# MarineRoboticsGroup/mac

Hardware: AMD Instinct MI355X
Metric: frank_wolfe_iters_per_sec (higher is better)
Workload: dtype f64; 1 GPU; configs[3]: ER N=100000 ~2M candidates, chain fixed, K=10%; N=100000, m_candidates=2001737, K=200173, fixed_edges=99999, fw_iters=209, parallelism=single GPU

## Files before the change

### include/machip.h

```cpp
#ifndef MACHIP_H
#define MACHIP_H

#include <stdint.h>

#ifdef __cplusplus
extern "C" {
#endif

#define MACHIP_ABI_VERSION 11

typedef enum machip_status {
    MACHIP_OK = 0,
    MACHIP_NOT_CONVERGED = 1,
    MACHIP_DISCONNECTED = 2,
    MACHIP_BAD_ARG = 3,
    MACHIP_HIP_ERROR = 4,
    MACHIP_RCCL_ERROR = 5,
    MACHIP_NO_DEVICE = 6
} machip_status;

typedef struct machip_problem machip_problem;

typedef struct machip_solve_stats {
    int64_t lanczos_steps;
    int64_t spmv_total;
    int64_t vec_passes;
    int64_t restarts;
    int64_t nnz;
    int64_t support;
    double residual;
    double lnorm;
    double gpu_ms;
    double step_ms;
    int64_t steps_timed;
    int64_t steps_lowp;
    double drift;
} machip_solve_stats;

int machip_version(void);
int machip_sizeof_stats(void);
int machip_device_count(void);
const char* machip_last_error(void);

int machip_create(int device, int64_t n,
                  int64_t n_fixed, const int32_t* fi, const int32_t* fj, const double* fw,
                  int64_t m, const int32_t* ci, const int32_t* cj, const double* cw,
                  double min_selection_weight_tol, machip_problem** out);
void machip_destroy(machip_problem* p);

int machip_set_x(machip_problem* p, const double* x);
int machip_get_x(machip_problem* p, double* x);

int machip_assemble(machip_problem* p, int64_t* nnz_out);
int machip_get_laplacian(machip_problem* p, int32_t* indptr, int32_t* indices, double* data);

int machip_fiedler(machip_problem* p, double tol, int max_steps, const double* x0, int warm_start,
                   double* lambda2, double* v_out, double* X_out, int q,
                   machip_solve_stats* stats);

int machip_set_start(machip_problem* p, const double* x0);

int machip_gradient(machip_problem* p, double* g_out);

int machip_lp_topk(machip_problem* p, int64_t k, double* s_out);

int machip_fw_step(machip_problem* p, int64_t k, int iter, double tol, int max_steps, int warm_start,
                   double* f, double* dual, double* gnorm, machip_solve_stats* stats);
int machip_fw_commit(machip_problem* p);
int machip_fw_run(machip_problem* p, int64_t k, int first_iter, int max_iters, double gap_tol, double grad_tol, double tol,
                  int max_steps, int warm_start, double* upper_inout, double* f_traj, double* dual_traj, double* gnorm_traj,
                  machip_solve_stats* stats, int* modes, int* iters_done);

int machip_round_nearest(machip_problem* p, int64_t k, int decimals, double* rounded_out);

int machip_fiedler_csr(int device, int64_t n, const int32_t* indptr, const int32_t* indices,
                       const double* data, double tol, int max_steps, const double* x0,
                       double* lambda2, double* v_out, double* X_out, int q,
                       machip_solve_stats* stats);

int machip_spmv(machip_problem* p, const double* v, double* y, int variant);

int machip_landscape(machip_problem* p, int sweeps, double* u_out);

int machip_profile_spmv(machip_problem* p, int reps, double* avg_us, double* bytes_per_launch);

int machip_comm_unique_id(void* id128);
int machip_comm_init(machip_problem* p, int rank, int nranks, const void* id128);
int machip_comm_init_local(machip_problem** handles, int nranks);
int machip_selftest_watchdog(int work_ms, int limit_ms);
int machip_peer_access(int device_a, int device_b);
int machip_ipc_blob_bytes(void);
int machip_ipc_export(machip_problem* p, void* blob, int blob_bytes);
int machip_comm_init_ipc(machip_problem* p, int rank, int nranks, const void* blobs, double timeout_s);
int machip_comm_close_ipc(machip_problem* p);
int machip_comm_drop_ipc(machip_problem* p);
int machip_comm_drop(machip_problem* p);
int machip_comm_timing(machip_problem* p, double* grad_us, double* exchange_us);
int machip_solve_mode(machip_problem* p, int64_t* closures);
int machip_comm_mode(machip_problem* p);
int machip_shard_plan(int64_t m, int nranks, int rank, int64_t* lo, int64_t* hi, int64_t* shard);

int machip_eval_batch(machip_problem* p, int B, const double* X, double tol, int max_steps, double* lambda2,
                      int* status);

int machip_fw_sweep(machip_problem* p, int B, const int64_t* ks, const double* X0, int max_iters, double gap_tol,
                    double grad_tol, double tol, int max_steps, int warm_start, int round_decimals, double* X_out,
                    double* R_out, double* upper, double* f_traj, int* iters, int* status);

int machip_set_solver(machip_problem* p, int mode);

int machip_set_precision(machip_problem* p, int precision);

#define MACHIP_OPTION_AUTO INT64_MIN
int machip_set_option(machip_problem* p, const char* name, int64_t value);
int machip_get_option(machip_problem* p, const char* name, int64_t* value);
const char* machip_option_name(int i);

int machip_synchronize(machip_problem* p);

int machip_membench(int device, int64_t bytes, int reps, double* read_gbs, double* triad_gbs);
int machip_panel_plan(int64_t n, int64_t nnz, int maxlen, int* out12);
void machip_release_cache(void);
int machip_host_tridiag_smallest(const double* a, const double* b, int J, double* theta, double* s);
int machip_host_follow_records(const double* tri3, int J, int n, double e_target, double tiny_l, int jcap, int* points, int cap,
                               int* npoints, int* jeff, double* est);

typedef struct machip_esp machip_esp;
#define MACHIP_ESP_DENSE_INVERSE 1
#define MACHIP_ESP_MATRIX_FREE 2
#define MACHIP_ESP_SPANNING_TREE 8
int machip_esp_create(int device, int64_t n, int64_t n_fixed, const int32_t* fi, const int32_t* fj, const double* fw,
                      int64_t m, const int32_t* ci, const int32_t* cj, const double* cw, int fold, int flags, machip_esp** out);
void machip_esp_destroy(machip_esp* h);
int machip_esp_select(machip_esp* h, int nb, const int64_t* ks, int32_t* order_out, double* gain_out, double* t_ms_out);
int machip_esp_weighted_resistances(machip_esp* h, double* r_out);
int machip_esp_info(machip_esp* h, int32_t* info4, double* beta);
int machip_esp_tree_plan(int64_t n, int64_t n_fixed, const int32_t* fi, const int32_t* fj, const double* fw, int32_t* parent,
                         double* R, int32_t* pre, int32_t* end, int64_t* n_seeds, int32_t* su, int32_t* sv, double* sw);
int machip_esp_seeds(machip_esp* h, int64_t* seeds_out);

int machip_esp_relax_eval(machip_esp* h, const double* x, double* F_out, double* grad_out);
int machip_esp_relax_run(machip_esp* h, int64_t k, int max_iters, double gap_tol, double grad_tol, double* x_inout,
                         double* f_traj, double* dual_traj, double* gnorm_traj, int* iters_out, double* upper_out);
int machip_esp_relax_inner(machip_esp* h, const double* a, const double* b, double* out);

typedef struct machip_eig machip_eig;
int machip_eig_create(int device, int64_t n, int64_t n_fixed, const int32_t* fi, const int32_t* fj, const double* fw,
                      int64_t m, const int32_t* ci, const int32_t* cj, const double* cw, int fold, int batch, int flags, machip_eig** out);
void machip_eig_destroy(machip_eig* h);
int machip_eig_select(machip_eig* h, int64_t k, int32_t* order_out, double* lambda2_out, double* t_ms_out);
int machip_eig_candidate_lambda2(machip_eig* h, double* out);
int machip_eig_candidate_bounds(machip_eig* h, double* out);
int machip_eig_info(machip_eig* h, int32_t* info6, double* beta_lambda2, int64_t cap, int32_t* solved_out, int32_t* applies_out);

#ifdef __cplusplus
}
#endif
#endif
```

### mac_amd/_lib.py

```python
from __future__ import annotations

import ctypes as C
import os

import numpy as np

_HERE = os.path.dirname(os.path.abspath(__file__))
LIB_PATH = os.environ.get("MACHIP_LIB") or os.path.join(_HERE, "libmachip.so")

OK, NOT_CONVERGED, DISCONNECTED, BAD_ARG, HIP_ERROR, RCCL_ERROR, NO_DEVICE = range(7)
STATUS_NAMES = ["OK", "NOT_CONVERGED", "DISCONNECTED", "BAD_ARG", "HIP_ERROR", "RCCL_ERROR", "NO_DEVICE"]


class MachipError(RuntimeError):
    def __init__(self, status, msg):
        super().__init__(f"libmachip: {STATUS_NAMES[status] if 0 <= status < 7 else status}: {msg}")
        self.status = status


class NotConverged(MachipError):
    pass


class Disconnected(MachipError):
    """lambda_2 ~ 0 (the reference fails with SuperLU 'Factor is exactly singular')."""


class SolveStats(C.Structure):
    _fields_ = [("lanczos_steps", C.c_int64), ("spmv_total", C.c_int64), ("vec_passes", C.c_int64),
                ("restarts", C.c_int64), ("nnz", C.c_int64), ("support", C.c_int64),
                ("residual", C.c_double), ("lnorm", C.c_double), ("gpu_ms", C.c_double),
                ("step_ms", C.c_double), ("steps_timed", C.c_int64), ("steps_lowp", C.c_int64), ("drift", C.c_double)]

    def asdict(self):
        return {k: getattr(self, k) for k, _ in self._fields_}


_i32p = C.POINTER(C.c_int32)
_f64p = C.POINTER(C.c_double)
_lib = None

SIGNATURES = {
    "machip_version": (C.c_int, []),
    "machip_sizeof_stats": (C.c_int, []),
    "machip_device_count": (C.c_int, []),
    "machip_last_error": (C.c_char_p, []),
    "machip_create": (C.c_int, [C.c_int, C.c_int64, C.c_int64, _i32p, _i32p, _f64p, C.c_int64, _i32p, _i32p,
                                _f64p, C.c_double, C.POINTER(C.c_void_p)]),
    "machip_destroy": (None, [C.c_void_p]),
    "machip_set_x": (C.c_int, [C.c_void_p, _f64p]),
    "machip_get_x": (C.c_int, [C.c_void_p, _f64p]),
    "machip_assemble": (C.c_int, [C.c_void_p, C.POINTER(C.c_int64)]),
    "machip_get_laplacian": (C.c_int, [C.c_void_p, _i32p, _i32p, _f64p]),
    "machip_fiedler": (C.c_int, [C.c_void_p, C.c_double, C.c_int, _f64p, C.c_int, _f64p, _f64p, _f64p, C.c_int,
                                 C.POINTER(SolveStats)]),
    "machip_set_start": (C.c_int, [C.c_void_p, _f64p]),
    "machip_gradient": (C.c_int, [C.c_void_p, _f64p]),
    "machip_lp_topk": (C.c_int, [C.c_void_p, C.c_int64, _f64p]),
    "machip_fw_step": (C.c_int, [C.c_void_p, C.c_int64, C.c_int, C.c_double, C.c_int, C.c_int, _f64p, _f64p,
                                 _f64p, C.POINTER(SolveStats)]),
    "machip_fw_commit": (C.c_int, [C.c_void_p]),
    "machip_fw_run": (C.c_int, [C.c_void_p, C.c_int64, C.c_int, C.c_int, C.c_double, C.c_double, C.c_double, C.c_int, C.c_int, _f64p, _f64p,
                                _f64p, _f64p, C.POINTER(SolveStats), C.POINTER(C.c_int), C.POINTER(C.c_int)]),
    "machip_round_nearest": (C.c_int, [C.c_void_p, C.c_int64, C.c_int, _f64p]),
    "machip_fiedler_csr": (C.c_int, [C.c_int, C.c_int64, _i32p, _i32p, _f64p, C.c_double, C.c_int, _f64p, _f64p,
                                     _f64p, _f64p, C.c_int, C.POINTER(SolveStats)]),
    "machip_spmv": (C.c_int, [C.c_void_p, _f64p, _f64p, C.c_int]),
    "machip_landscape": (C.c_int, [C.c_void_p, C.c_int, _f64p]),
    "machip_profile_spmv": (C.c_int, [C.c_void_p, C.c_int, _f64p, _f64p]),
    "machip_comm_unique_id": (C.c_int, [C.c_void_p]),
    "machip_comm_init": (C.c_int, [C.c_void_p, C.c_int, C.c_int, C.c_void_p]),
    "machip_comm_init_local": (C.c_int, [C.POINTER(C.c_void_p), C.c_int]),
    "machip_selftest_watchdog": (C.c_int, [C.c_int, C.c_int]),
    "machip_peer_access": (C.c_int, [C.c_int, C.c_int]),
    "machip_ipc_blob_bytes": (C.c_int, []),
    "machip_ipc_export": (C.c_int, [C.c_void_p, C.c_void_p, C.c_int]),
    "machip_comm_init_ipc": (C.c_int, [C.c_void_p, C.c_int, C.c_int, C.c_void_p, C.c_double]),
    "machip_comm_close_ipc": (C.c_int, [C.c_void_p]),
    "machip_comm_mode": (C.c_int, [C.c_void_p]),
    "machip_shard_plan": (C.c_int, [C.c_int64, C.c_int, C.c_int, C.POINTER(C.c_int64), C.POINTER(C.c_int64), C.POINTER(C.c_int64)]),
    "machip_eval_batch": (C.c_int, [C.c_void_p, C.c_int, _f64p, C.c_double, C.c_int, _f64p, C.POINTER(C.c_int)]),
    "machip_fw_sweep": (C.c_int, [C.c_void_p, C.c_int, C.POINTER(C.c_int64), _f64p, C.c_int, C.c_double, C.c_double, C.c_double,
                                  C.c_int, C.c_int, C.c_int, _f64p, _f64p, _f64p, _f64p, C.POINTER(C.c_int), C.POINTER(C.c_int)]),
    "machip_set_solver": (C.c_int, [C.c_void_p, C.c_int]),
    "machip_set_option": (C.c_int, [C.c_void_p, C.c_char_p, C.c_int64]),
    "machip_get_option": (C.c_int, [C.c_void_p, C.c_char_p, C.POINTER(C.c_int64)]),
    "machip_option_name": (C.c_char_p, [C.c_int]),
    "machip_comm_drop_ipc": (C.c_int, [C.c_void_p]),
    "machip_comm_drop": (C.c_int, [C.c_void_p]),
    "machip_comm_timing": (C.c_int, [C.c_void_p, _f64p, _f64p]),
    "machip_solve_mode": (C.c_int, [C.c_void_p, C.POINTER(C.c_int64)]),
    "machip_set_precision": (C.c_int, [C.c_void_p, C.c_int]),
    "machip_synchronize": (C.c_int, [C.c_void_p]),
    "machip_membench": (C.c_int, [C.c_int, C.c_int64, C.c_int, _f64p, _f64p]),
    "machip_host_tridiag_smallest": (C.c_int, [_f64p, _f64p, C.c_int, _f64p, _f64p]),
    "machip_host_follow_records": (C.c_int, [_f64p, C.c_int, C.c_int, C.c_double, C.c_double, C.c_int, C.POINTER(C.c_int), C.c_int,
                                             C.POINTER(C.c_int), C.POINTER(C.c_int), C.POINTER(C.c_double)]),
    "machip_release_cache": (None, []),
    "machip_panel_plan": (C.c_int, [C.c_int64, C.c_int64, C.c_int, C.POINTER(C.c_int)]),
    "machip_esp_create": (C.c_int, [C.c_int, C.c_int64, C.c_int64, _i32p, _i32p, _f64p, C.c_int64, _i32p, _i32p, _f64p,
                                    C.c_int, C.c_int, C.POINTER(C.c_void_p)]),
    "machip_esp_destroy": (None, [C.c_void_p]),
    "machip_esp_select": (C.c_int, [C.c_void_p, C.c_int, C.POINTER(C.c_int64), _i32p, _f64p, _f64p]),
    "machip_esp_weighted_resistances": (C.c_int, [C.c_void_p, _f64p]),
    "machip_esp_info": (C.c_int, [C.c_void_p, _i32p, C.POINTER(C.c_double)]),
    "machip_esp_tree_plan": (C.c_int, [C.c_int64, C.c_int64, _i32p, _i32p, _f64p, _i32p, _f64p, _i32p, _i32p, C.POINTER(C.c_int64),
                                       _i32p, _i32p, _f64p]),
    "machip_esp_seeds": (C.c_int, [C.c_void_p, C.POINTER(C.c_int64)]),
    "machip_esp_relax_eval": (C.c_int, [C.c_void_p, _f64p, C.POINTER(C.c_double), _f64p]),
    "machip_esp_relax_run": (C.c_int, [C.c_void_p, C.c_int64, C.c_int, C.c_double, C.c_double, _f64p, _f64p, _f64p, _f64p,
                                       C.POINTER(C.c_int), C.POINTER(C.c_double)]),
    "machip_esp_relax_inner": (C.c_int, [C.c_void_p, _f64p, _f64p, C.POINTER(C.c_double)]),
    "machip_eig_create": (C.c_int, [C.c_int, C.c_int64, C.c_int64, _i32p, _i32p, _f64p, C.c_int64, _i32p, _i32p, _f64p,
                                    C.c_int, C.c_int, C.c_int, C.POINTER(C.c_void_p)]),
    "machip_eig_destroy": (None, [C.c_void_p]),
    "machip_eig_select": (C.c_int, [C.c_void_p, C.c_int64, _i32p, _f64p, _f64p]),
    "machip_eig_candidate_lambda2": (C.c_int, [C.c_void_p, _f64p]),
    "machip_eig_candidate_bounds": (C.c_int, [C.c_void_p, _f64p]),
    "machip_eig_info": (C.c_int, [C.c_void_p, _i32p, _f64p, C.c_int64, _i32p, _i32p]),
}


def load():
    global _lib
    if _lib is not None:
        return _lib
    if not os.path.exists(LIB_PATH):
        raise ImportError(f"{LIB_PATH} is missing: build it with `python __graft_entry__.py` "
                          "(hipcc --offload-arch=gfx950); mac_amd has no CPU fallback")
    lib = C.CDLL(LIB_PATH, mode=C.RTLD_GLOBAL)
    for name, (res, args) in SIGNATURES.items():
        fn = getattr(lib, name)
        fn.restype = res
        fn.argtypes = args
    _lib = lib
    import atexit
    atexit.register(lib.machip_release_cache)
    return lib


OPTION_AUTO = -(1 << 63)
CREATION_OPTIONS = frozenset({"asm_g", "asm_maxgrid", "vbudget_mb", "vcap"})


def option_names():
    lib, out, i = load(), [], 0
    while True:
        nm = lib.machip_option_name(i)
        if nm is None:
            return out
        out.append(nm.decode())
        i += 1


def set_default_option(name, value=None):
    check(load().machip_set_option(None, name.encode(), OPTION_AUTO if value is None else int(value)))


class default_options:

    def __init__(self, **opts):
        self.opts = opts

    def __enter__(self):
        lib = load()
        self.old = {}
        for k, v in self.opts.items():
            cur = C.c_int64(0)
            check(lib.machip_get_option(None, k.encode(), C.byref(cur)))
            self.old[k] = cur.value
            set_default_option(k, v)
        return self

    def __exit__(self, *exc):
# ... 130 lines not shown

    def gradient(self, want=True):
        g = np.empty(self.m) if want else None
        check(self._lib.machip_gradient(self._h, p_f64(g)))
        return g

    def lp_topk(self, k, want=True):
        s = np.empty(self.m) if want else None
        check(self._lib.machip_lp_topk(self._h, int(k), p_f64(s)))
        return s

    def fw_step(self, k, it, tol=1e-8, max_steps=0, warm_start=False):
        f, d, gn = C.c_double(), C.c_double(), C.c_double()
        check(self._lib.machip_fw_step(self._h, int(k), int(it), float(tol), int(max_steps),
                                       int(bool(warm_start)), C.byref(f), C.byref(d), C.byref(gn),
                                       C.byref(self.stats)))
        return f.value, d.value, gn.value

    def fw_commit(self):
        check(self._lib.machip_fw_commit(self._h))

    def fw_run(self, k, max_iters, first_iter=0, gap_tol=0.0, grad_tol=0.0, tol=1e-8, max_steps=0, warm_start=False, upper=float("inf")):
        n = max(1, int(max_iters))
        f = np.zeros(n); d = np.zeros(n); gn = np.zeros(n)
        st = (SolveStats * n)()
        modes = (C.c_int * (2 * n))()
        up = C.c_double(float(upper)); done = C.c_int(0)
        status = self._lib.machip_fw_run(self._h, int(k), int(first_iter), int(max_iters), float(gap_tol), float(grad_tol), float(tol),
                                         int(max_steps), int(bool(warm_start)), C.byref(up), p_f64(f), p_f64(d), p_f64(gn), st, modes, C.byref(done))
        it = int(done.value)
        if it:
            C.memmove(C.byref(self.stats), C.byref(st[it - 1]), C.sizeof(SolveStats))
        check(status)
        return dict(f=f[:it], dual=d[:it], gnorm=gn[:it], upper=up.value, iters=it, stats=[st[i] for i in range(it)],
                    modes=[(int(modes[2 * i]), int(modes[2 * i + 1])) for i in range(it)])

    def round_nearest(self, k, decimals=10):
        out = np.empty(self.m)
        check(self._lib.machip_round_nearest(self._h, int(k), -1 if decimals is None else int(decimals), p_f64(out)))
        return out

    def profile_spmv(self, reps=200):
        us, by = C.c_double(), C.c_double()
        check(self._lib.machip_profile_spmv(self._h, int(reps), C.byref(us), C.byref(by)))
        return us.value, by.value

    def comm_init(self, rank, nranks, unique_id: bytes):
        _single_node_bootstrap()
        buf = C.create_string_buffer(unique_id, 128)
        with _stdout_to_stderr():
            st = self._lib.machip_comm_init(self._h, int(rank), int(nranks), buf)
        check(st)

    def ipc_export(self) -> bytes:
        nb = self._lib.machip_ipc_blob_bytes()
        buf = C.create_string_buffer(nb)
        check(self._lib.machip_ipc_export(self._h, buf, nb))
        return buf.raw

    def comm_init_ipc(self, rank, nranks, blobs, timeout_s=10.0):
        nb = self._lib.machip_ipc_blob_bytes()
        assert len(blobs) == nranks and all(len(b) == nb for b in blobs)
        buf = C.create_string_buffer(b"".join(blobs), nb * nranks)
        check(self._lib.machip_comm_init_ipc(self._h, int(rank), int(nranks), buf, float(timeout_s)))

    def comm_close_ipc(self):
        check(self._lib.machip_comm_close_ipc(self._h))

    def comm_drop_ipc(self):
        check(self._lib.machip_comm_drop_ipc(self._h))

    def comm_drop(self):
        check(self._lib.machip_comm_drop(self._h))

    def comm_timing(self):
        a, b = C.c_double(0.0), C.c_double(0.0)
        check(self._lib.machip_comm_timing(self._h, C.byref(a), C.byref(b)))
        return a.value, b.value

    def solve_mode(self):
        c = C.c_int64(0)
        return int(self._lib.machip_solve_mode(self._h, C.byref(c))), int(c.value)

    def set_option(self, name, value=None):
        if value is not None and name in CREATION_OPTIONS:
            raise ValueError(f"option {name!r} is read when the handle is created: set it with mac_amd._lib.default_options({name}=...) around the constructor")
        check(self._lib.machip_set_option(self._h, name.encode(), OPTION_AUTO if value is None else int(value)))

    def set_options(self, **opts):
        for k, v in opts.items():
            self.set_option(k, v)

    def get_option(self, name):
        v = C.c_int64(0)
        check(self._lib.machip_get_option(self._h, name.encode(), C.byref(v)))
        return None if v.value == OPTION_AUTO else v.value

    def set_solver(self, mode):
        check(self._lib.machip_set_solver(self._h, int(mode)))

    def eval_batch(self, X, tol=1e-8, max_steps=0):
        X = np.ascontiguousarray(X, dtype=np.float64)
        assert X.ndim == 2 and X.shape[1] == self.m
        B = X.shape[0]
        lam = np.zeros(B)
        st = np.zeros(B, dtype=np.int32)
        check(self._lib.machip_eval_batch(self._h, B, p_f64(X), float(tol), int(max_steps), p_f64(lam),
                                          st.ctypes.data_as(C.POINTER(C.c_int))))
        return lam, st

    def fw_sweep(self, ks, X0, max_iters=5, gap_tol=1e-4, grad_tol=1e-8, tol=1e-8, max_steps=0, warm_start=False,
                 round_decimals=10, want_rounded=True):
        X0 = np.ascontiguousarray(X0, dtype=np.float64)
        ks = np.ascontiguousarray(ks, dtype=np.int64)
        assert X0.ndim == 2 and X0.shape == (len(ks), self.m)
        B = len(ks)
        X = np.empty((B, self.m)); R = np.empty((B, self.m)) if want_rounded else None
        up = np.zeros(B); ft = np.full((B, max(1, max_iters)), np.nan)
        it = np.zeros(B, dtype=np.int32); st = np.zeros(B, dtype=np.int32)
        check(self._lib.machip_fw_sweep(self._h, B, ks.ctypes.data_as(C.POINTER(C.c_int64)), p_f64(X0), int(max_iters),
                                        float(gap_tol), float(grad_tol), float(tol), int(max_steps), int(bool(warm_start)),
                                        int(round_decimals), p_f64(X), p_f64(R), p_f64(up), p_f64(ft),
                                        it.ctypes.data_as(C.POINTER(C.c_int)), st.ctypes.data_as(C.POINTER(C.c_int))))
        return dict(x=X, rounded=R, upper=up, f_traj=ft[:, :max_iters], iters=it, status=st)

    def set_precision(self, precision):
        check(self._lib.machip_set_precision(self._h, int(precision)))

    def synchronize(self):
        check(self._lib.machip_synchronize(self._h))


ESP_DENSE_INVERSE = 1
ESP_MATRIX_FREE = 2
ESP_SPANNING_TREE = 8


def host_esp_tree(n, fi, fj, fw):
    fi, fj, fw = i32(fi), i32(fj), f64(fw)
    n, nf = int(n), len(fw)
    parent, pre, end = (np.zeros(max(n, 1), dtype=np.int32) for _ in range(3))
    R = np.zeros(max(n, 1))
    su, sv, sw = np.zeros(max(nf, 1), dtype=np.int32), np.zeros(max(nf, 1), dtype=np.int32), np.zeros(max(nf, 1))
    r = C.c_int64(0)
    check(load().machip_esp_tree_plan(n, nf, p_i32(fi), p_i32(fj), p_f64(fw), p_i32(parent), p_f64(R), p_i32(pre), p_i32(end),
                                      C.byref(r), p_i32(su), p_i32(sv), p_f64(sw)))
    r = r.value
    return dict(parent=parent[:n], R=R[:n], pre=pre[:n], end=end[:n], seeds=(su[:r].copy(), sv[:r].copy(), sw[:r].copy()))


class Esp:

    def __init__(self, n, fi, fj, fw, ci, cj, cw, fold=64, dense_inverse=False, device=0, *, matrix_free=False):
        if not isinstance(matrix_free, (bool, np.bool_)) and matrix_free != "tree":
            raise ValueError(f'matrix_free must be False, True or "tree", not {matrix_free!r}')
        lib = load()
        require_device()
        self.n = int(n)
        fi, fj, fw = i32(fi), i32(fj), f64(fw)
        ci, cj, cw = i32(ci), i32(cj), f64(cw)
        self.m = int(len(cw))
        h = C.c_void_p()
        flags = (ESP_DENSE_INVERSE if dense_inverse else 0) | (ESP_MATRIX_FREE if matrix_free else 0)
        if isinstance(matrix_free, str):
            flags |= ESP_SPANNING_TREE
        check(lib.machip_esp_create(int(device), self.n, len(fw), p_i32(fi), p_i32(fj), p_f64(fw), self.m,
# ... 198 lines not shown
```

### mac_amd/csrc/kernels.h

```cpp
#pragma once
#include "common.h"

namespace machip {

template <typename T>
struct CsrViewT {
    int n;
    const int* rowptr;
    const int* col;
    const T* val;
};
using CsrView = CsrViewT<double>;

struct PatternView {
    int n;
    const int* prow;
    const int* pcol;
    const int* pk;
    const double* pw;
};

struct LanState {
    int jA;
    int jB;
// ... 3 lines not shown

struct LanView {
    int n;
    LanState* st;
    double* u;
    double* w;
    double* V;
    double* alpha;
    double* beta;
    double* l1;
    double* part_u;
    int P_u;
    double* part_a;
    int P_a;
};

constexpr int kAsmGrid = 4096;
__global__ __launch_bounds__(kBlock) void k_x_bits(const double* __restrict__ x, long m, double tol, unsigned long long* __restrict__ bits) {
    for (long i = (long)blockIdx.x * kBlock + threadIdx.x; i < m; i += (long)gridDim.x * kBlock) {
        const unsigned long long bal = __ballot(x[i] > tol);
        if ((threadIdx.x & 63) == 0) bits[i >> 6] = bal;
    }
}
__device__ __forceinline__ bool x_bit(const unsigned int* __restrict__ bits32, int k) { return (bits32[k >> 5] >> (k & 31)) & 1u; }

template <int G>
__global__ __launch_bounds__(kBlock) void k_asm_count(PatternView P, const unsigned int* __restrict__ xbits,
                                                      int rows_per_block,
                                                      int* __restrict__ cnt, int* __restrict__ blk_sum,
                                                      int* __restrict__ hsum = nullptr) {
    __shared__ int sm[4];
    constexpr int GPB = kBlock / G;
    const int lane = threadIdx.x % G, g = threadIdx.x / G;
    const int r0 = blockIdx.x * rows_per_block;
    const int r1 = min(P.n, r0 + rows_per_block);
    int local = 0, supp = 0, mx = 0;
    for (int r = r0 + g; r < r1; r += GPB) {
        const int b = P.prow[r], e = P.prow[r + 1];
        int c = 0, sc = 0;
        for (int p = b + lane; p < e; p += G) {
            const int k = P.pk[p];
            const bool cand = k >= 0;
            const bool act = cand ? x_bit(xbits, k) : true;
            c += act;
            sc += (cand && act);
        }
        c = group_sum_i<G>(c);
        sc = group_sum_i<G>(sc);
        if (lane == 0) {
            cnt[r] = c + 1;
            local += c + 1;
            supp += sc;
            mx = max(mx, c + 1);
        }
    }
    const int tot = block_sum_i(local, sm);
    const int stot = block_sum_i(supp, sm);
#pragma unroll
    for (int o = 32; o > 0; o >>= 1) mx = max(mx, __shfl_xor(mx, o, kWave));
    __syncthreads();
    if ((threadIdx.x & 63) == 0) sm[threadIdx.x >> 6] = mx;
    __syncthreads();
    if (threadIdx.x == 0) {
        blk_sum[blockIdx.x] = tot;
        blk_sum[kAsmGrid + blockIdx.x] = stot;
        const int longest = max(max(sm[0], sm[1]), max(sm[2], sm[3]));
        blk_sum[2 * kAsmGrid + blockIdx.x] = longest;
        if (hsum) {
            hsum[blockIdx.x] = tot; hsum[kAsmGrid + blockIdx.x] = stot; hsum[2 * kAsmGrid + blockIdx.x] = longest;
        }
    }
}

struct PanSpec {
    int NP = 0;
    int C = 1;
    int band = 0;
    int* ps = nullptr;
    double* bd = nullptr;
    int* bpk = nullptr;
    int* ovf = nullptr;
};

template <int G>
__global__ __launch_bounds__(kBlock) void k_asm_fill(PatternView P, const unsigned int* __restrict__ xbits, const double* __restrict__ x,
                                                     int rows_per_block,
                                                     const int* __restrict__ cnt,
                                                     const int* __restrict__ blk_sum,
                                                     int* __restrict__ rowptr, int* __restrict__ col,
                                                     double* __restrict__ val,
                                                     double* __restrict__ blk_lnorm, PanSpec S = PanSpec()) {
    extern __shared__ __attribute__((aligned(16))) char smem_raw[];
    int* s_off = reinterpret_cast<int*>(smem_raw);
    __shared__ int sm_i[4];
    __shared__ double sm_d[4];
    __shared__ int s_chunk[kBlock];
    constexpr int GPB = kBlock / G;
    const int tid = threadIdx.x;
    const int lane = tid % G, g = tid / G;
    const int r0 = blockIdx.x * rows_per_block;
    const int r1 = min(P.n, r0 + rows_per_block);
    const int nr = max(0, r1 - r0);

    int acc = 0;
    for (int b = tid; b < (int)blockIdx.x; b += kBlock) acc += blk_sum[b];
    const int base = block_sum_i(acc, sm_i);

    const int per = (nr + kBlock - 1) / kBlock;
    int csum = 0;
    for (int i = 0; i < per; ++i) {
        const int idx = tid * per + i;
        if (idx < nr) csum += cnt[r0 + idx];
    }
    {
        const int ln = tid & 63, wv = tid >> 6;
        int x = csum;
        for (int o = 1; o < 64; o <<= 1) { const int y = __shfl_up(x, o, kWave); if (ln >= o) x += y; }
        if (ln == 63) s_chunk[wv] = x;
        __syncthreads();
        int before = 0;
        for (int q = 0; q < wv; ++q) before += s_chunk[q];
        int run = before + x - csum;
        if (tid == kBlock - 1) s_off[nr] = before + x;
        for (int i = 0; i < per; ++i) {
            const int idx = tid * per + i;
            if (idx < nr) { s_off[idx] = run; run += cnt[r0 + idx]; }
        }
    }
    __syncthreads();

    double lmax = 0.0;
    for (int r = r0 + g; r < r1; r += GPB) {
        const int b = P.prow[r], e = P.prow[r + 1];
        const int out = base + s_off[r - r0];
        int pos = out + 1;
        double dsum = 0.0, asum = 0.0;
        int lastpid = 0;
        int hb = 0x7fffffff, hn = 0;
        double vl = 0.0, vu = 0.0;
        const int gbase = ((tid & 63) / G) * G;
        for (int p0 = b; p0 < e; p0 += G) {
            const int p = p0 + lane;
            const bool in = p < e;
            const int kc = in ? P.pk[p] : -1;
            const double wgt = in ? P.pw[p] : 0.0;
            const double xk = kc >= 0 ? x[kc] : 1.0;
            const bool act = in && (kc < 0 || x_bit(xbits, kc));
            const double v = act ? xk * wgt : 0.0;
            const unsigned long long bal = __ballot(act);
            unsigned long long gm;
            if (G == 64) gm = bal;
            else gm = (bal >> gbase) & ((1ull << (G & 63)) - 1ull);
            const unsigned long long below = gm & ((1ull << lane) - 1ull);
            const int before = __popcll(below);
            const int c = act ? P.pcol[p] : 0;
            if (act) { col[pos + before] = c; val[pos + before] = -v; }
            if (S.NP) {
                const int pid = act ? c / S.C : 0;
                const int src = below ? 63 - __builtin_clzll(below) : 0;
                const int got = __shfl(pid, gbase + src, kWave);
                const int ppid = below ? got : lastpid;
                if (act) {
                    const int q = pos + before;
                    for (int pp = ppid + 1; pp <= pid; ++pp) S.ps[(size_t)r * (S.NP + 1) + pp] = q;
                    if (S.band && (c == r - 1 || c == r + 1)) {
                        hb = min(hb, q); hn += 1;
                        if (c == r - 1) vl += -v; else vu += -v;
                    }
                }
                if (gm) lastpid = __shfl(pid, gbase + 63 - __builtin_clzll(gm), kWave);
            }
            pos += __popcll(gm);
            dsum += v;
            asum += fabs(v);
        }
        dsum = group_sum<G>(dsum);
        asum = group_sum<G>(asum);
        if (S.NP) {
            if (lane == 0) S.ps[(size_t)r * (S.NP + 1)] = out + 1;
            for (int pp = lastpid + 1 + lane; pp <= S.NP; pp += G) S.ps[(size_t)r * (S.NP + 1) + pp] = pos;
            if (S.band) {
                hn = group_sum_i<G>(hn);
                vl = group_sum<G>(vl); vu = group_sum<G>(vu);
#pragma unroll
                for (int o = G / 2; o > 0; o >>= 1) hb = min(hb, __shfl_xor(hb, o, kWave));
                if (lane == 0) {
                    S.bpk[r] = ((hn ? hb : pos) << 3) | min(hn, 7);
                    if (hn > 7) *S.ovf = 1;
                    S.bd[r] = dsum; S.bd[(size_t)P.n + r] = vl; S.bd[2 * (size_t)P.n + r] = vu;
                }
            }
        }
        if (lane == 0) {
            rowptr[r] = out;
            col[out] = r;
            val[out] = dsum;
            lmax = fmax(lmax, fabs(dsum) + asum);
        }
    }
    lmax = block_max(lmax, sm_d);
    if (tid == 0) {
        blk_lnorm[blockIdx.x] = lmax;
        if (blockIdx.x == gridDim.x - 1) rowptr[P.n] = base + s_off[nr];
    }
}

template <int G, class Op>
__device__ __forceinline__ void spmv_rows_vec(const CsrView& A, const double* __restrict__ x, Op& op) {
    constexpr int GPB = kBlock / G;
    const int lane = threadIdx.x % G, g = threadIdx.x / G;
    const int stride = gridDim.x * GPB;
    for (int r = blockIdx.x * GPB + g; r < A.n; r += 2 * stride) {
        const int r2 = r + stride;
        const bool two = r2 < A.n;
        const int b = A.rowptr[r], e = A.rowptr[r + 1];
        const int b2 = two ? A.rowptr[r2] : 0, e2 = two ? A.rowptr[r2 + 1] : 0;
        double acc = 0.0, acc2 = 0.0;
        int p = b + lane, q = b2 + lane;
        while (p < e || q < e2) {
            double v1 = 0.0, x1 = 0.0, v2 = 0.0, x2 = 0.0;
            if (p < e) { v1 = A.val[p]; x1 = op.gather(x, A.col[p]); }
            if (q < e2) { v2 = A.val[q]; x2 = op.gather(x, A.col[q]); }
            if (p < e) acc += v1 * x1;
            if (q < e2) acc2 += v2 * x2;
            p += G; q += G;
        }
        acc = group_sum<G>(acc);
        acc2 = group_sum<G>(acc2);
        if (lane == 0) { op.row(r, acc); if (two) op.row(r2, acc2); }
    }
}

constexpr int kStreamTile = 2048;

template <int TPR, class Op>
__device__ __forceinline__ void spmv_rows_stream(const CsrView& A, const double* __restrict__ x, Op& op,
                                                 double* prod, int* sptr) {
    constexpr int R = kBlock / TPR;
    const int tid = threadIdx.x;
    const int row = tid / TPR, sub = tid % TPR;
    for (int tile = blockIdx.x; tile * R < A.n; tile += gridDim.x) {
        const int r0 = tile * R;
        const int nr = min(R, A.n - r0);
        for (int i = tid; i <= nr; i += kBlock) sptr[i] = A.rowptr[r0 + i];
        __syncthreads();
        const int p0 = sptr[0], p1 = sptr[nr];
        double acc = 0.0;
        for (int base = p0; base < p1; base += kStreamTile) {
            const int cnt = min(kStreamTile, p1 - base);
            for (int i = tid; i < cnt; i += kBlock) prod[i] = A.val[base + i] * op.gather(x, A.col[base + i]);
            __syncthreads();
            if (row < nr) {
                const int lo = max(sptr[row], base), hi = min(sptr[row + 1], base + cnt);
                for (int q = lo + sub; q < hi; q += TPR) acc += prod[q - base];
            }
            __syncthreads();
        }
        acc = group_sum<TPR>(acc);
        if (row < nr && sub == 0) op.row(r0 + row, acc);
        __syncthreads();
    }
}

struct OpPlain {
    double* y;
    __device__ __forceinline__ void begin(double*) {}
    __device__ __forceinline__ double gather(const double* __restrict__ x, int c) const { return x[c]; }
    __device__ __forceinline__ void row(int r, double acc) { y[r] = acc; }
    __device__ __forceinline__ void end(double*) {}
};

struct OpLanczos {
    LanView L;
    int j;
    double mu, beta, inv, ap;
    const double* vprev;
    double* vj;
    __device__ __forceinline__ void begin(double* sm) {
        j = L.st->jA;
        const double s1 = reduce_partials(L.part_u, L.P_u, sm);
        const double s2 = reduce_partials(L.part_u + kMaxGrid, L.P_u, sm);
        const double s3 = reduce_partials(L.part_u + 2 * kMaxGrid, L.P_u, sm);
        mu = s1 / (double)L.n;
        const double nrm2 = s2 - (double)L.n * mu * mu;
        beta = nrm2 > 0.0 ? sqrt(nrm2) : 0.0;
        inv = beta > 1e-290 ? 1.0 / beta : 0.0;
        ap = 0.0;
        vj = L.V + (size_t)j * (size_t)L.n;
        vprev = j > 0 ? vj - L.n : nullptr;
        if (blockIdx.x == 0 && threadIdx.x == 0) {
            L.beta[j] = beta;
            L.l1[j] = s3 * inv;
            L.st->jB = j;
        }
    }
    __device__ __forceinline__ double gather(const double* __restrict__ x, int c) const { return x[c]; }
    __device__ __forceinline__ void row(int r, double acc) {
        const double wr = acc * inv;
        const double v = (L.u[r] - mu) * inv;
        vj[r] = v;
        L.w[r] = wr;
        const double t = vprev ? wr - beta * vprev[r] : wr;
        ap += v * t;
    }
    __device__ __forceinline__ void end(double* sm) {
        const double tot = block_sum(ap, sm);
        if (threadIdx.x == 0) L.part_a[blockIdx.x] = tot;
    }
};

template <int G, class Op>
__global__ __launch_bounds__(kBlock) void k_spmv_vec(CsrView A, const double* __restrict__ x, Op op) {
    __shared__ double sm[4];
    op.begin(sm);
    spmv_rows_vec<G>(A, x, op);
    op.end(sm);
}

template <int TPR, class Op>
__global__ __launch_bounds__(kBlock) void k_spmv_stream(CsrView A, const double* __restrict__ x, Op op) {
    __shared__ double sm[4];
    __shared__ double prod[kStreamTile];
    __shared__ int sptr[kBlock / TPR + 1];
    op.begin(sm);
    spmv_rows_stream<TPR>(A, x, op, prod, sptr);
    op.end(sm);
}

__global__ __launch_bounds__(kBlock) void k_land_init(CsrView A, double* __restrict__ dg, double* __restrict__ u) {
    for (int r = blockIdx.x * kBlock + threadIdx.x; r < A.n; r += gridDim.x * kBlock) {
        double d = 0.0;
        for (int p = A.rowptr[r], e = A.rowptr[r + 1]; p < e; ++p)
            if (A.col[p] == r) { d = A.val[p]; break; }
        dg[r] = d;
        u[r] = d > 0.0 ? 1.0 / d : 0.0;
    }
}
struct OpLand {
    const double* uin;
    double* uout;
    const double* dg;
    double* pmax;
    double mx;
    __device__ __forceinline__ void begin(double*) { mx = 0.0; }
    __device__ __forceinline__ double gather(const double* __restrict__ x, int c) const { return x[c]; }
    __device__ __forceinline__ void row(int r, double acc) {
        const double d = dg[r];
        double v = d > 0.0 ? uin[r] + (1.0 - acc) / d : 0.0;
        v = v > 0.0 && v < 1e300 ? v : 0.0;
        uout[r] = v;
        mx = fmax(mx, v);
    }
    __device__ __forceinline__ void end(double* sm) {
        const double m = block_max(mx, sm);
        if (threadIdx.x == 0) pmax[blockIdx.x] = m;
    }
};
__global__ __launch_bounds__(kBlock) void k_land_weight(const double* __restrict__ u, const double* __restrict__ pmax, int npart,
                                                        double* __restrict__ z, int n, double p, double floor_w) {
    __shared__ double sm[4];
    double m = 0.0;
    for (int i = threadIdx.x; i < npart; i += kBlock) m = fmax(m, pmax[i]);
    m = block_max(m, sm);
    if (!(m > 0.0)) return;
    const double inv = 1.0 / m;
    for (int r = blockIdx.x * kBlock + threadIdx.x; r < n; r += gridDim.x * kBlock) {
        const double q = u[r] * inv;
        z[r] *= fmax(q > 0.0 ? exp(p * log(q)) : 0.0, floor_w);
    }
}

__global__ __launch_bounds__(kBlock) void k_lan_update(LanView L) {
    __shared__ double sm[4];
    const int j = L.st->jB;
    const double alpha = reduce_partials(L.part_a, L.P_a, sm);
    const double beta = L.beta[j];
    const double* vj = L.V + (size_t)j * (size_t)L.n;
    const double* vp = j > 0 ? vj - L.n : nullptr;
    double s1 = 0.0, s2 = 0.0, s3 = 0.0;
    for (int r = blockIdx.x * kBlock + threadIdx.x; r < L.n; r += gridDim.x * kBlock) {
        double t = L.w[r] - alpha * vj[r];
        if (vp) t -= beta * vp[r];
        L.u[r] = t;
        s1 += t;
        s2 += t * t;
        s3 += fabs(t);
    }
    s1 = block_sum(s1, sm);
    s2 = block_sum(s2, sm);
    s3 = block_sum(s3, sm);
    if (threadIdx.x == 0) {
        L.part_u[blockIdx.x] = s1;
        L.part_u[kMaxGrid + blockIdx.x] = s2;
        L.part_u[2 * kMaxGrid + blockIdx.x] = s3;
        if (blockIdx.x == 0) {
            L.alpha[j] = alpha;
            L.st->jA = j + 1;
        }
    }
}

__global__ __launch_bounds__(kBlock) void k_lan_tail(LanView L) {
    __shared__ double sm[4];
    const int j = L.st->jA;
    const double s1 = reduce_partials(L.part_u, L.P_u, sm);
    const double s2 = reduce_partials(L.part_u + kMaxGrid, L.P_u, sm);
    const double s3 = reduce_partials(L.part_u + 2 * kMaxGrid, L.P_u, sm);
    if (threadIdx.x == 0) {
        const double mu = s1 / (double)L.n;
        const double nrm2 = s2 - (double)L.n * mu * mu;
        const double beta = nrm2 > 0.0 ? sqrt(nrm2) : 0.0;
        L.beta[j] = beta;
        L.l1[j] = beta > 1e-290 ? s3 / beta : 0.0;
    }
}

// ... 965 lines not shown
```

### mac_amd/csrc/machip.hip

```cpp
#include <rccl/rccl.h>
#include <unistd.h>

#include <algorithm>
#include <atomic>
#include <cmath>
#include <chrono>
#include <condition_variable>
#include <functional>
#include <future>
#include <memory>
#include <mutex>
#include <numeric>
#include <thread>
#include <vector>

#include "solver.h"
#include "esp.h"
#include "esp_free.h"
#include "esp_tree.h"
#include "esp_relax.h"
#include "eig.h"

namespace machip {
thread_local std::string g_err;
}
using namespace machip;

#define NCCL_TRY(expr)                                                                       \
    do {                                                                                     \
        ncclResult_t r__ = (expr);                                                           \
        if (r__ != ncclSuccess)                                                              \
            return fail(MACHIP_RCCL_ERROR, std::string(#expr) + ": " + ncclGetErrorString(r__)); \
    } while (0)

static int run_with_watchdog(const std::function<int()>& fn, double limit_s, const std::string& what) {
    auto state = std::make_shared<std::promise<int>>();
    std::future<int> fut = state->get_future();
    std::thread([state, fn] { int r = MACHIP_HIP_ERROR; try { r = fn(); } catch (...) {} state->set_value(r); }).detach();
    if (fut.wait_for(std::chrono::duration<double>(limit_s)) != std::future_status::ready)
        return fail(MACHIP_RCCL_ERROR, what + " did not return within " + std::to_string((int)limit_s) + " s (a peer rank is missing, or the fabric / bootstrap interface is not reachable; MACHIP_RCCL_TIMEOUT_S raises the limit)");
    return fut.get();
}
static double rccl_timeout_s() { const Options& opt = default_options(); const int t = OPT(rccl_timeout_s, 600); return t > 0 ? (double)t : 600.0; }

struct machip_problem;
struct LocalGroup {
    int nranks = 0;
    std::vector<double*> g;
    std::vector<machip_problem*> members;
    ShardGroup sg;
    bool shard_eig = false;
    int lead_status = MACHIP_OK;
    double lead_lam = 0.0;
    machip_solve_stats lead_stats{};
    std::string lead_err;
    ~LocalGroup() {
        for (ShardRank& r : sg.rk) for (hipEvent_t e : r.ev) if (e) (void)hipEventDestroy(e);
        if (sg.fork) (void)hipEventDestroy(sg.fork);
    }
    std::mutex mu;
    std::condition_variable cv;
    int waiting = 0;
    unsigned long generation = 0;
    bool broken = false;
    bool barrier() {
        std::unique_lock<std::mutex> lk(mu);
        if (broken) return false;
        const unsigned long gen = generation;
        if (++waiting == nranks) { waiting = 0; ++generation; cv.notify_all(); return true; }
        cv.wait(lk, [&] { return generation != gen || broken; });
        return !broken;
    }
    void abort() {
        std::lock_guard<std::mutex> lk(mu);
        broken = true;
        cv.notify_all();
    }
};

struct machip_problem {
    int device = 0;
    hipStream_t stream = nullptr;
    int n = 0;
    long m = 0, m_pad = 0;
    double tol_sel = 1e-10;
    int *prow = nullptr, *pcol = nullptr, *pk = nullptr;
    double* pw = nullptr;
    long P = 0;
    int asm_G = 16, asm_rpb = 1, asm_grid = 1;
    int *ci = nullptr, *cj = nullptr;
    double* cw = nullptr;
    double *x = nullptr, *x_next = nullptr, *g = nullptr, *s = nullptr, *scratch_m = nullptr;
    int *cnt = nullptr, *blk_sum = nullptr, *rowptr = nullptr, *col = nullptr;
    double *val = nullptr, *blk_lnorm = nullptr;
    unsigned long long *xb = nullptr, *xb_next = nullptr;
    bool xb_valid = false, xb_next_valid = false;
    long nnz = 0, support = 0;
    int maxlen = 0;
    double lnorm = 0.0;
    bool assembled = false, have_vec = false, csr_only = false;
    bool band_dups_ok = true;
    unsigned int* hist = nullptr;
    SelState* sel = nullptr;
    double* part_fw = nullptr;
    int* h_int = nullptr;
    double* h_dbl = nullptr;
    int* d_hint = nullptr;
    double* d_hdbl = nullptr;
    Solver sol;
    ncclComm_t comm = nullptr;
    std::shared_ptr<LocalGroup> lgroup;
    bool first_collective_pending = false;
    hipEvent_t ev_g0 = nullptr, ev_g1 = nullptr, ev_g2 = nullptr;
    bool ev_g_valid = false;
    std::unique_ptr<IpcGroup> ipcg;
    int rank = 0, nranks = 1;
    bool is_lane = false, lane_fw_ready = false;
    std::vector<machip_problem*> lanes;
    unsigned long start_version = 0;
    unsigned long seen_start_version = ~0ul;

    CsrView csr() const { return CsrView{n, rowptr, col, val}; }
    PatternView pattern() const { return PatternView{n, prow, pcol, pk, pw}; }
};

static int create_lane_stream(const Options& opt, int device, hipStream_t* out) {
    if (OPT(lane_queues, 0) == 0) {
        hipDeviceProp_t prop;
        if (hipGetDeviceProperties(&prop, device) == hipSuccess && prop.multiProcessorCount > 0) {
            const int words = (prop.multiProcessorCount + 31) / 32;
            std::vector<uint32_t> mask((size_t)words, 0xffffffffu);
            if (prop.multiProcessorCount % 32) mask.back() = (1u << (prop.multiProcessorCount % 32)) - 1u;
            if (hipExtStreamCreateWithCUMask(out, (uint32_t)words, mask.data()) == hipSuccess) return MACHIP_OK;
            (void)hipGetLastError();
        }
    }
    HIP_TRY(hipStreamCreateWithFlags(out, hipStreamNonBlocking));
    return MACHIP_OK;
}

namespace {

std::mutex g_csr_mu;
machip_problem* g_csr_cache = nullptr;

struct Slot {
    int col;
    int k;
    double w;
};

int build_pattern(machip_problem* p, int64_t nf, const int32_t* fi, const int32_t* fj, const double* fw,
                  int64_t m, const int32_t* ci, const int32_t* cj, const double* cw) {
    const Options& opt = p->sol.opt;
    const int n = p->n;
    std::vector<long> deg((size_t)n + 1, 0);
    auto chk = [&](int a, int b) { return a >= 0 && a < n && b >= 0 && b < n; };
    for (int64_t e = 0; e < nf; ++e) {
        if (!chk(fi[e], fj[e])) return fail(MACHIP_BAD_ARG, "fixed edge endpoint out of range");
        if (fi[e] != fj[e]) { deg[(size_t)fi[e]]++; deg[(size_t)fj[e]]++; }
    }
    for (int64_t e = 0; e < m; ++e) {
        if (!chk(ci[e], cj[e])) return fail(MACHIP_BAD_ARG, "candidate edge endpoint out of range");
        if (ci[e] != cj[e]) { deg[(size_t)ci[e]]++; deg[(size_t)cj[e]]++; }
    }
    std::vector<long> off((size_t)n + 1, 0);
    for (int r = 0; r < n; ++r) off[(size_t)r + 1] = off[(size_t)r] + deg[(size_t)r];
    std::vector<Slot> slots((size_t)off[(size_t)n]);
    std::vector<long> cur(off.begin(), off.end() - 1);
    for (int64_t e = 0; e < nf; ++e) {
        const int a = fi[e], b = fj[e];
        if (a == b) continue;
        slots[(size_t)cur[(size_t)a]++] = Slot{b, -1, fw[e]};
        slots[(size_t)cur[(size_t)b]++] = Slot{a, -1, fw[e]};
    }
    for (int64_t e = 0; e < m; ++e) {
        const int a = ci[e], b = cj[e];
        if (a == b) continue;
        slots[(size_t)cur[(size_t)a]++] = Slot{b, (int)e, cw[e]};
        slots[(size_t)cur[(size_t)b]++] = Slot{a, (int)e, cw[e]};
    }
    std::vector<int> prow((size_t)n + 1, 0);
    std::vector<int> pcol, pk;
    std::vector<double> pw;
    pcol.reserve(slots.size()); pk.reserve(slots.size()); pw.reserve(slots.size());
    for (int r = 0; r < n; ++r) {
        Slot* b = slots.data() + off[(size_t)r];
        Slot* e = slots.data() + off[(size_t)r + 1];
        std::sort(b, e, [](const Slot& x, const Slot& y) {
            if (x.col != y.col) return x.col < y.col;
            return x.k < y.k;
        });
        for (Slot* q = b; q < e; ++q) {
            if (q->k < 0 && !pcol.empty() && (long)pcol.size() > prow[(size_t)r] && pcol.back() == q->col &&
                pk.back() < 0) {
                pw.back() += q->w;
            } else {
                pcol.push_back(q->col); pk.push_back(q->k); pw.push_back(q->w);
            }
        }
        if (pcol.size() > 2000000000ull) return fail(MACHIP_BAD_ARG, "pattern exceeds int32 indexing");
        {
            int band_slots = 0;
            for (size_t q = (size_t)prow[(size_t)r]; q < pcol.size(); ++q) band_slots += (pcol[q] == r - 1 || pcol[q] == r + 1);
            if (band_slots > 7) p->band_dups_ok = false;
        }
        prow[(size_t)r + 1] = (int)pcol.size();
    }
    p->P = (long)pcol.size();
    ST_TRY(dev_alloc(&p->prow, (size_t)n + 1));
    ST_TRY(dev_alloc(&p->pcol, (size_t)p->P)); ST_TRY(dev_alloc(&p->pk, (size_t)p->P)); ST_TRY(dev_alloc(&p->pw, (size_t)p->P));
    HIP_TRY(hipMemcpyAsync(p->prow, prow.data(), sizeof(int) * ((size_t)n + 1), hipMemcpyHostToDevice, p->stream));
    if (p->P) {
        HIP_TRY(hipMemcpyAsync(p->pcol, pcol.data(), sizeof(int) * (size_t)p->P, hipMemcpyHostToDevice, p->stream));
        HIP_TRY(hipMemcpyAsync(p->pk, pk.data(), sizeof(int) * (size_t)p->P, hipMemcpyHostToDevice, p->stream));
        HIP_TRY(hipMemcpyAsync(p->pw, pw.data(), sizeof(double) * (size_t)p->P, hipMemcpyHostToDevice, p->stream));
    }
    HIP_TRY(hipStreamSynchronize(p->stream));
    const double mean = n ? (double)p->P / n : 1.0;
    int G = 4;
    while (G < 64 && G < mean * 0.75) G <<= 1;
    p->asm_G = OPT(asm_g, G);
    const int gpb = kBlock / p->asm_G;
    long nblk = std::min<long>(std::min(kAsmGrid, std::max(1, OPT(asm_maxgrid, kAsmGrid))), ((long)n + gpb - 1) / gpb);
    if (nblk < 1) nblk = 1;
    long rpb = ((long)n + nblk - 1) / nblk;
    rpb = (rpb + gpb - 1) / gpb * gpb;
    p->asm_rpb = (int)rpb;
    p->asm_grid = (int)(((long)n + rpb - 1) / rpb);
    if (p->asm_grid < 1) p->asm_grid = 1;
    if ((rpb + 1) * (long)sizeof(int) > 64 * 1024)
        return fail(MACHIP_BAD_ARG, "num_nodes above the supported 16.7 million (row-offset scan of the assembly kernel)");
    return MACHIP_OK;
}

template <int G>
void launch_asm(machip_problem* p, const PanSpec& S) {
    const PatternView P = p->pattern();
    const unsigned int* xb32 = reinterpret_cast<const unsigned int*>(p->xb);
    k_asm_count<G><<<p->asm_grid, kBlock, 0, p->stream>>>(P, xb32, p->asm_rpb, p->cnt, p->blk_sum, p->d_hint);
    const size_t lds = sizeof(int) * ((size_t)p->asm_rpb + 1);
    k_asm_fill<G><<<p->asm_grid, kBlock, lds, p->stream>>>(P, xb32, p->x, p->asm_rpb, p->cnt, p->blk_sum,
                                                           p->rowptr, p->col, p->val, p->d_hdbl, S);
}

int assemble(machip_problem* p) {
    if (p->csr_only) return fail(MACHIP_BAD_ARG, "handle wraps a caller CSR; nothing to assemble");
    PanSpec S;
    ST_TRY(p->sol.pan_spec_prepare(&S));
    if (!p->xb_valid) {
        const int grid = std::max(1, (int)std::min<long>(kMaxGrid, (p->m + kBlock - 1) / kBlock));
        k_x_bits<<<grid, kBlock, 0, p->stream>>>(p->x, p->m, p->tol_sel, p->xb);
        p->xb_valid = true;
    }
    switch (p->asm_G) {
        case 4: launch_asm<4>(p, S); break;
        case 8: launch_asm<8>(p, S); break;
        case 16: launch_asm<16>(p, S); break;
        case 32: launch_asm<32>(p, S); break;
        default: launch_asm<64>(p, S); break;
    }
    HIP_TRY(hipGetLastError());
    const int gb = p->asm_grid;
    HIP_TRY(hipStreamSynchronize(p->stream));
    long nnz = 0, supp = 0;
    int maxlen = 0;
    double ln = 0.0;
    for (int b = 0; b < gb; ++b) {
        nnz += p->h_int[b]; supp += p->h_int[kAsmGrid + b]; maxlen = std::max(maxlen, p->h_int[2 * kAsmGrid + b]);
        ln = std::max(ln, p->h_dbl[b]);
    }
    p->nnz = nnz; p->support = supp / 2; p->lnorm = ln; p->maxlen = maxlen;
    p->assembled = true;
    return MACHIP_OK;
}

int alloc_common(machip_problem* p, int vbudget_mb = 0) {
    ST_TRY(p->sol.init(p->n, p->stream, vbudget_mb));
    HIP_TRY(hipHostMalloc((void**)&p->h_int, sizeof(int) * 3 * kAsmGrid, hipHostMallocMapped));
    HIP_TRY(hipHostMalloc((void**)&p->h_dbl, sizeof(double) * std::max(4 * kMaxGrid, kAsmGrid), hipHostMallocMapped));
    HIP_TRY(hipHostGetDevicePointer((void**)&p->d_hint, p->h_int, 0));
    HIP_TRY(hipHostGetDevicePointer((void**)&p->d_hdbl, p->h_dbl, 0));
    return MACHIP_OK;
}

int select_on(machip_problem* p, const double* keys, long k, SelState* st, int prefer_high, bool hist0_done = false) {
    const Options& opt = p->sol.opt;
    const long m = p->m;
    if (k < 0) k = 0;
    if (k > m) k = m;
    if (m <= kSelSmallMax && OPT(sel_small, 1)) {
        k_sel_small<<<1, 1024, 0, p->stream>>>(keys, m, (long long)k, st, prefer_high);
        HIP_TRY(hipGetLastError());
        return MACHIP_OK;
    }
    if (!hist0_done) k_sel_init<<<1, 1024, 0, p->stream>>>(st, (long long)k, p->hist, 6 * kBins);
    if (k > 0) {
        constexpr int B = 1024, U = 4;
        const int grid = (int)std::max<long>(1, std::min<long>(128, (m + (long)B * U - 1) / ((long)B * U)));
        if (hist0_done) k_sel_close0<<<1, 1024, 0, p->stream>>>(p->hist, st);
        for (int pass = hist0_done ? 1 : 0; pass < 6; ++pass) k_sel_pass<U, B><<<grid, B, 0, p->stream>>>(keys, m, pass, p->hist, st);
    }
    k_sel_ties<<<1, 1024, 0, p->stream>>>(keys, m, st, prefer_high);
    HIP_TRY(hipGetLastError());
    return MACHIP_OK;
}

int select_topk(machip_problem* p, long k, bool hist0_done = false) { return select_on(p, p->g, k, p->sel, 0, hist0_done); }

void shard_plan(long m, int nranks, int rank, long* lo, long* hi, long* shard) {
    const long sh = nranks > 0 ? (m + nranks - 1) / nranks : m;
    *shard = sh;
    *lo = std::min(m, sh * rank);
    *hi = std::min(m, *lo + sh);
}

int local_allgather(machip_problem* p, long shard) {
    LocalGroup& G = *p->lgroup;
    HIP_TRY(hipStreamSynchronize(p->stream));
    if (!G.barrier()) return fail(MACHIP_RCCL_ERROR, "in-process communicator was shut down by another rank");
    for (int r = 0; r < G.nranks; ++r)
        if (r != p->rank)
            HIP_TRY(hipMemcpyAsync(p->g + shard * r, G.g[(size_t)r] + shard * r, sizeof(double) * (size_t)shard,
                                   hipMemcpyDeviceToDevice, p->stream));
    HIP_TRY(hipStreamSynchronize(p->stream));
    if (!G.barrier()) return fail(MACHIP_RCCL_ERROR, "in-process communicator was shut down by another rank");
    return MACHIP_OK;
}

int compute_gradient(machip_problem* p, bool have_vec_now = false, long fuse_k = -1, bool* fused = nullptr) {
    const Options& opt = p->sol.opt;
    if (!p->have_vec && !have_vec_now) return fail(MACHIP_BAD_ARG, "no Fiedler vector on the device: call machip_fiedler first");
    const long m = p->m;
    long lo = 0, hi = m, shard = m;
    if (p->nranks > 1) shard_plan(m, p->nranks, p->rank, &lo, &hi, &shard);
    const bool ipc_gather = p->nranks > 1 && !p->comm && p->ipcg;
    if (ipc_gather) {
        k_ipc_pubwait<<<1, 64, 0, p->stream>>>(p->ipcg->view, 3);
    }
    const bool timed = p->nranks > 1;
    if (timed) {
        if (!p->ev_g0) { HIP_TRY(hipEventCreate(&p->ev_g0)); HIP_TRY(hipEventCreate(&p->ev_g1)); HIP_TRY(hipEventCreate(&p->ev_g2)); }
        p->ev_g_valid = false;
        HIP_TRY(hipEventRecord(p->ev_g0, p->stream));
    }
    if (hi > lo) {
        const int grid = (int)std::min<long>(kMaxGrid * 4, (hi - lo + kBlock - 1) / kBlock);
        PeerVecs all;
        if (ipc_gather) { all.n = p->ipcg->nranks; for (int q = 0; q < all.n; ++q) all.v[q] = p->ipcg->g[q]; }
        const bool fuse = fuse_k > 0 && p->nranks <= 1 && m > kSelSmallMax && OPT(sel_fuse, 1) != 0;
        if (fused) *fused = fuse;
        if (fuse) {
            k_sel_init<<<1, 1024, 0, p->stream>>>(p->sel, (long long)std::min(fuse_k, m), p->hist, (6 + kSelRep) * kBins);
            k_grad<true><<<grid, kBlock, 0, p->stream>>>(p->ci, p->cj, p->cw, p->sol.yvec, lo, hi, p->g, all, p->hist + 6 * kBins);
        } else k_grad<false><<<grid, kBlock, 0, p->stream>>>(p->ci, p->cj, p->cw, p->sol.yvec, lo, hi, p->g, all);
        HIP_TRY(hipGetLastError());
    }
    if (timed) HIP_TRY(hipEventRecord(p->ev_g1, p->stream));
    if (ipc_gather) {
        k_ipc_pubwait<<<1, 64, 0, p->stream>>>(p->ipcg->view, 2);
        HIP_TRY(hipGetLastError());
        HIP_TRY(hipEventRecord(p->ev_g2, p->stream));
        p->ev_g_valid = true;
        return MACHIP_OK;
    }
    if (p->nranks > 1) {
        if (p->comm) {
            NCCL_TRY(ncclAllGather(p->g + shard * p->rank, p->g, (size_t)shard, ncclDouble, p->comm, p->stream));
            if (p->first_collective_pending) {
                p->first_collective_pending = false;
                const auto t0 = std::chrono::steady_clock::now();
                const double lim = rccl_timeout_s();
                for (;;) {
                    const hipError_t q = hipStreamQuery(p->stream);
                    if (q == hipSuccess) break;
                    if (q != hipErrorNotReady) return fail(MACHIP_HIP_ERROR, std::string("first ncclAllGather: ") + hipGetErrorString(q));
                    ncclResult_t ar = ncclSuccess;
                    if (ncclCommGetAsyncError(p->comm, &ar) == ncclSuccess && ar != ncclSuccess && ar != ncclInProgress)
                        return fail(MACHIP_RCCL_ERROR, std::string("first ncclAllGather failed asynchronously: ") + ncclGetErrorString(ar));
                    if (std::chrono::duration<double>(std::chrono::steady_clock::now() - t0).count() > lim) {
                        (void)ncclCommAbort(p->comm);
                        p->comm = nullptr;
                        return fail(MACHIP_RCCL_ERROR, "first ncclAllGather of rank " + std::to_string(p->rank) + " of " + std::to_string(p->nranks) +
                                    " did not complete within " + std::to_string((int)lim) + " s: communicator aborted");
                    }
                    std::this_thread::sleep_for(std::chrono::microseconds(200));
                }
            }
        }
        else if (p->lgroup) { const int st = local_allgather(p, shard); if (st != MACHIP_OK) { p->lgroup->abort(); return st; } }
        else return fail(MACHIP_BAD_ARG, "nranks > 1 without a communicator");
        HIP_TRY(hipEventRecord(p->ev_g2, p->stream));
        p->ev_g_valid = true;
    }
    return MACHIP_OK;
}

int run_fiedler(machip_problem* p, double tol, int max_steps, const double* x0, int warm_start,
                double* lambda2, machip_solve_stats* stats) {
    if (!p->assembled) ST_TRY(assemble(p));
    if (x0) {
        HIP_TRY(hipMemcpyAsync(p->sol.start, x0, sizeof(double) * (size_t)p->n, hipMemcpyHostToDevice, p->stream));
        HIP_TRY(hipStreamSynchronize(p->stream));
        p->sol.have_start = true;
        ++p->start_version;
    }
    machip_solve_stats local;
    memset(&local, 0, sizeof(local));
    p->sol.maxlen_hint = p->maxlen;
    p->sol.support_hint = (p->csr_only && !p->sol.chain_like) ? -1 : p->support;
    p->sol.start_guess = x0 != nullptr;
    const int st = p->sol.solve(p->csr(), p->nnz, p->lnorm, tol, max_steps, (x0 == nullptr && warm_start) ? 1 : 0,
                                kAuto, lambda2, &local);
    p->sol.start_guess = false;
    local.support = p->support;
    if (stats) *stats = local;
    p->have_vec = (st == MACHIP_OK || st == MACHIP_NOT_CONVERGED || st == MACHIP_DISCONNECTED);
    return st;
}

int group_fiedler(machip_problem* p, double tol, int max_steps, int warm_start, double* lambda2, machip_solve_stats* stats) {
    LocalGroup& G = *p->lgroup;
    if (!G.barrier()) return fail(MACHIP_RCCL_ERROR, "in-process communicator was shut down by another rank");
    if (p->rank == 0) {
        for (int r = 0; r < G.nranks; ++r) {
            machip_problem* q = G.members[(size_t)r];
            ShardRank& k = G.sg.rk[(size_t)r];
            k.device = q->device; k.stream = q->stream; k.Z0 = q->sol.Z0; k.Z1 = q->sol.Z1; k.part = q->sol.part; k.V = q->sol.V;
            k.ypart = q->sol.ypart; k.sdev = q->sol.sdev; k.yvec = q->sol.yvec; k.A = q->csr();
        }
        machip_solve_stats local;
        memset(&local, 0, sizeof(local));
        p->sol.shard = &G.sg;
        int st = run_fiedler(p, tol, max_steps, nullptr, warm_start, &G.lead_lam, &local);
        p->sol.shard = nullptr;
        if (st == MACHIP_OK || st == MACHIP_NOT_CONVERGED || st == MACHIP_DISCONNECTED) {
            const std::string keep = g_err;
            for (int r = 1; r < G.nranks && (st == MACHIP_OK || st == MACHIP_NOT_CONVERGED || st == MACHIP_DISCONNECTED); ++r)
                if (hipMemcpyAsync(G.sg.rk[(size_t)r].yvec, p->sol.yvec, sizeof(double) * (size_t)p->n, hipMemcpyDeviceToDevice, p->stream) != hipSuccess)
                    st = fail(MACHIP_HIP_ERROR, "copy of the Fiedler vector to a peer failed");
            if (hipStreamSynchronize(p->stream) != hipSuccess) st = fail(MACHIP_HIP_ERROR, "stream error after the row-partitioned solve");
            else g_err = keep;
        }
        G.lead_status = st; G.lead_stats = local; G.lead_err = g_err;
    }
    if (!G.barrier()) return fail(MACHIP_RCCL_ERROR, "in-process communicator was shut down by another rank");
    const int st = G.lead_status;
    *lambda2 = G.lead_lam;
    if (stats) { *stats = G.lead_stats; stats->support = p->support; }
    if (p->rank != 0) {
        g_err = G.lead_err;
        p->have_vec = (st == MACHIP_OK || st == MACHIP_NOT_CONVERGED || st == MACHIP_DISCONNECTED);
    }
    return st;
}

}

extern "C" {

int machip_version(void) { return MACHIP_ABI_VERSION; }
int machip_sizeof_stats(void) { return (int)sizeof(machip_solve_stats); }

int machip_device_count(void) {
    int c = 0;
    if (hipGetDeviceCount(&c) != hipSuccess) return 0;
    return c;
}

const char* machip_last_error(void) { return g_err.c_str(); }

int machip_create(int device, int64_t n, int64_t n_fixed, const int32_t* fi, const int32_t* fj, const double* fw,
                  int64_t m, const int32_t* ci, const int32_t* cj, const double* cw, double min_sel_tol,
                  machip_problem** out) {
    if (!out) return fail(MACHIP_BAD_ARG, "out is NULL");
    *out = nullptr;
    if (n < 2 || n > 2000000000ll) return fail(MACHIP_BAD_ARG, "num_nodes must be in [2, 2e9]");
    if (n_fixed < 0 || m < 0 || m > 2000000000ll) return fail(MACHIP_BAD_ARG, "bad edge counts");
    if ((n_fixed && (!fi || !fj || !fw)) || (m && (!ci || !cj || !cw))) return fail(MACHIP_BAD_ARG, "NULL edge array");
    if (n_fixed + m < n - 1) return fail(MACHIP_BAD_ARG, "fewer than n-1 edges: no spanning tree possible");
    if ((double)(n_fixed + m) > 0.5 * (double)n * (double)(n - 1)) return fail(MACHIP_BAD_ARG, "more edges than the complete graph");
    if (machip_device_count() <= 0) return fail(MACHIP_NO_DEVICE, "no HIP device visible");
    HIP_TRY(hipSetDevice(device));
// ... 22 lines not shown
        ST_TRY(dev_alloc(&p->cnt, (size_t)n + 1)); ST_TRY(dev_alloc(&p->blk_sum, 3 * kAsmGrid));
        ST_TRY(dev_alloc(&p->rowptr, (size_t)n + 1)); ST_TRY(dev_alloc(&p->col, cap)); ST_TRY(dev_alloc(&p->val, cap));
        ST_TRY(dev_alloc(&p->blk_lnorm, kAsmGrid));
        ST_TRY(dev_alloc(&p->xb, (size_t)m / 64 + 2)); ST_TRY(dev_alloc(&p->xb_next, (size_t)m / 64 + 2));
        ST_TRY(dev_alloc(&p->hist, (6 + kSelRep) * kBins)); ST_TRY(dev_alloc(&p->sel, 2)); ST_TRY(dev_alloc(&p->part_fw, 2 * kMaxGrid));
        ST_TRY(alloc_common(p));
        p->sol.csr_cap = cap;
        p->sol.pat = p->pattern();
        p->sol.pan_allowed = p->band_dups_ok;
        {
            std::vector<char> has((size_t)n, 0);
            for (int64_t e = 0; e < n_fixed; ++e) {
                const int a = std::min(fi[e], fj[e]), b = std::max(fi[e], fj[e]);
                if (a >= 0 && b < n && b == a + 1 && fw[e] > 0.0) has[(size_t)a] = 1;
            }
            long cnt = 0;
            for (int64_t i = 0; i + 1 < n; ++i) cnt += has[(size_t)i];
            p->sol.chain_like = cnt >= (long)(0.98 * (double)(n - 1));
            p->sol.chain_edges = cnt;
        }
        return MACHIP_OK;
    };
    st = body();
    if (st != MACHIP_OK) { machip_destroy(p); return st; }
    *out = p;
    return MACHIP_OK;
}

void machip_destroy(machip_problem* p) {
    if (!p) return;
    for (machip_problem* q : p->lanes) machip_destroy(q);
    p->lanes.clear();
    (void)hipSetDevice(p->device);
    if (p->stream) (void)hipStreamSynchronize(p->stream);
    if (p->is_lane) { p->prow = p->pcol = p->pk = nullptr; p->pw = nullptr; p->ci = p->cj = nullptr; p->cw = nullptr; }
    if (p->comm) (void)ncclCommDestroy(p->comm);
    if (p->lgroup) p->lgroup->abort();
    if (p->ipcg) {
        IpcGroup& G = *p->ipcg;
        if (!G.clean_exit) { k_ipc_abort<<<1, 64, 0, p->stream>>>(G.view); (void)hipStreamSynchronize(p->stream); }
        p->sol.ipc = nullptr;
        p->ipcg.reset();
    }
    p->sol.destroy();
    void* ptrs[] = {p->prow, p->pcol, p->pk, p->pw, p->ci, p->cj, p->cw, p->x, p->x_next, p->g, p->s, p->scratch_m, p->cnt,
                    p->blk_sum, p->rowptr, p->col, p->val, p->blk_lnorm, p->xb, p->xb_next, p->hist, p->sel, p->part_fw};
    for (void* q : ptrs) if (q) (void)hipFree(q);
    for (hipEvent_t e : {p->ev_g0, p->ev_g1, p->ev_g2}) if (e) (void)hipEventDestroy(e);
    if (p->h_int) (void)hipHostFree(p->h_int);
    if (p->h_dbl) (void)hipHostFree(p->h_dbl);
    if (p->stream) (void)hipStreamDestroy(p->stream);
    delete p;
}

int machip_set_x(machip_problem* p, const double* x) {
    if (!p || !x || p->csr_only) return fail(MACHIP_BAD_ARG, "machip_set_x: bad handle or NULL x");
    HIP_TRY(hipSetDevice(p->device));
    HIP_TRY(hipMemcpyAsync(p->x, x, sizeof(double) * (size_t)p->m, hipMemcpyHostToDevice, p->stream));
    HIP_TRY(hipStreamSynchronize(p->stream));
    p->assembled = false; p->xb_valid = false;
    return MACHIP_OK;
}

int machip_get_x(machip_problem* p, double* x) {
    if (!p || !x || p->csr_only) return fail(MACHIP_BAD_ARG, "machip_get_x: bad handle or NULL x");
    HIP_TRY(hipSetDevice(p->device));
    HIP_TRY(hipMemcpyAsync(x, p->x, sizeof(double) * (size_t)p->m, hipMemcpyDeviceToHost, p->stream));
    HIP_TRY(hipStreamSynchronize(p->stream));
    return MACHIP_OK;
}

int machip_assemble(machip_problem* p, int64_t* nnz_out) {
    if (!p) return fail(MACHIP_BAD_ARG, "NULL handle");
    HIP_TRY(hipSetDevice(p->device));
    ST_TRY(assemble(p));
    if (nnz_out) *nnz_out = p->nnz;
    return MACHIP_OK;
}

int machip_get_laplacian(machip_problem* p, int32_t* indptr, int32_t* indices, double* data) {
    if (!p || !indptr || !indices || !data) return fail(MACHIP_BAD_ARG, "NULL argument");
    HIP_TRY(hipSetDevice(p->device));
    if (!p->assembled) ST_TRY(assemble(p));
    HIP_TRY(hipMemcpyAsync(indptr, p->rowptr, sizeof(int) * ((size_t)p->n + 1), hipMemcpyDeviceToHost, p->stream));
    HIP_TRY(hipMemcpyAsync(indices, p->col, sizeof(int) * (size_t)p->nnz, hipMemcpyDeviceToHost, p->stream));
    HIP_TRY(hipMemcpyAsync(data, p->val, sizeof(double) * (size_t)p->nnz, hipMemcpyDeviceToHost, p->stream));
    HIP_TRY(hipStreamSynchronize(p->stream));
    return MACHIP_OK;
}

int machip_fiedler(machip_problem* p, double tol, int max_steps, const double* x0, int warm_start,
                   double* lambda2, double* v_out, double* X_out, int q, machip_solve_stats* stats) {
    if (!p || !lambda2) return fail(MACHIP_BAD_ARG, "NULL argument");
    if (X_out && (q < 1 || q > 4)) return fail(MACHIP_BAD_ARG, "q must be in [1,4]");
    HIP_TRY(hipSetDevice(p->device));
    const int st = run_fiedler(p, tol, max_steps, x0, warm_start, lambda2, stats);
    if (st != MACHIP_OK && st != MACHIP_NOT_CONVERGED && st != MACHIP_DISCONNECTED) return st;
    const std::string keep = g_err;
    if (v_out) {
        HIP_TRY(hipMemcpyAsync(v_out, p->sol.yvec, sizeof(double) * (size_t)p->n, hipMemcpyDeviceToHost, p->stream));
        HIP_TRY(hipStreamSynchronize(p->stream));
    }
    if (X_out) ST_TRY(p->sol.ritz_block(q, X_out));
    g_err = keep;
    return st;
}

int machip_set_start(machip_problem* p, const double* x0) {
    if (!p || !x0) return fail(MACHIP_BAD_ARG, "NULL argument");
    HIP_TRY(hipSetDevice(p->device));
    HIP_TRY(hipMemcpyAsync(p->sol.start, x0, sizeof(double) * (size_t)p->n, hipMemcpyHostToDevice, p->stream));
    HIP_TRY(hipStreamSynchronize(p->stream));
    p->sol.have_start = true;
    ++p->start_version;
    return MACHIP_OK;
}

namespace {
struct GroupGuard {
    machip_problem* p;
    bool ok = false;
    ~GroupGuard() {
        if (!ok && p && p->lgroup) p->lgroup->abort();
        if (!ok && p && p->ipcg) { k_ipc_abort<<<1, 64, 0, p->stream>>>(p->ipcg->view); (void)hipStreamSynchronize(p->stream); }
    }
};
}

int machip_gradient(machip_problem* p, double* g_out) {
    if (!p || p->csr_only) return fail(MACHIP_BAD_ARG, "bad handle");
    GroupGuard guard{p};
    HIP_TRY(hipSetDevice(p->device));
    if (!p->have_vec) { guard.ok = true; return fail(MACHIP_BAD_ARG, "no Fiedler vector on the device: call machip_fiedler first"); }
    ST_TRY(compute_gradient(p));
    if (g_out) HIP_TRY(hipMemcpyAsync(g_out, p->g, sizeof(double) * (size_t)p->m, hipMemcpyDeviceToHost, p->stream));
    HIP_TRY(hipStreamSynchronize(p->stream));
    guard.ok = true;
    return MACHIP_OK;
}

int machip_lp_topk(machip_problem* p, int64_t k, double* s_out) {
    if (!p || p->csr_only) return fail(MACHIP_BAD_ARG, "bad handle");
    HIP_TRY(hipSetDevice(p->device));
    ST_TRY(select_topk(p, (long)k));
    const int grid = (int)std::min<long>(kMaxGrid, (p->m + kBlock - 1) / kBlock);
    k_fw_final<<<std::max(grid, 1), kBlock, 0, p->stream>>>(p->g, nullptr, p->m, p->sel, 0.0, nullptr, p->s, p->part_fw);
    if (s_out) HIP_TRY(hipMemcpyAsync(s_out, p->s, sizeof(double) * (size_t)p->m, hipMemcpyDeviceToHost, p->stream));
    HIP_TRY(hipStreamSynchronize(p->stream));
    return MACHIP_OK;
}

int machip_fw_step(machip_problem* p, int64_t k, int iter, double tol, int max_steps, int warm_start,
                   double* f, double* dual, double* gnorm, machip_solve_stats* stats) {
    if (!p || p->csr_only || !f || !dual || !gnorm) return fail(MACHIP_BAD_ARG, "bad argument");
    GroupGuard guard{p};
    HIP_TRY(hipSetDevice(p->device));
    ST_TRY(assemble(p));
    double lam = 0.0;
    const int grid = std::max(1, (int)std::min<long>(kMaxGrid, (p->m + kBlock - 1) / kBlock));
    const double gamma = 2.0 / ((double)iter + 2.0);
    int epi_status = MACHIP_OK;
    auto epilogue = [&](bool speculative) {
        bool fused = false;
        int st = compute_gradient(p, speculative, (long)k, &fused);
        if (st == MACHIP_OK) st = select_topk(p, (long)k, fused);
        if (st == MACHIP_OK) {
            k_fw_final<<<grid, kBlock, 0, p->stream>>>(p->g, p->x, p->m, p->sel, gamma, p->x_next, nullptr, p->d_hdbl, p->tol_sel, p->xb_next);
            p->xb_next_valid = true;
            if (hipGetLastError() != hipSuccess) st = fail(MACHIP_HIP_ERROR, "k_fw_final launch failed");
        }
        epi_status = st;
    };
    bool done = false;
    auto soft = [](int st) { return st == MACHIP_NOT_CONVERGED || st == MACHIP_DISCONNECTED; };
    if (p->lgroup && p->lgroup->shard_eig) {
        const int st = group_fiedler(p, tol, max_steps, warm_start, &lam, stats);
        if (st != MACHIP_OK) { guard.ok = soft(st); return st; }
    } else {
        const bool spec = p->nranks <= 1 && p->sol.opt.get(kOpt_spec_epilogue, 1) != 0;
        if (spec) p->sol.after_check = [&] { epilogue(true); };
        const int st = run_fiedler(p, tol, max_steps, nullptr, warm_start, &lam, stats);
        p->sol.after_check = nullptr;
        if (st != MACHIP_OK) { guard.ok = soft(st); return st; }
        done = spec && p->sol.hook_seq == p->sol.final_check_seq && epi_status == MACHIP_OK;
    }
    if (!done) {
        epilogue(false);
        if (epi_status != MACHIP_OK) return epi_status;
        HIP_TRY(hipStreamSynchronize(p->stream));
    }
    if (p->ipcg) ST_TRY(p->sol.ipc_check_err("gradient exchange"));
    double d = 0.0, q2 = 0.0;
    for (int b = 0; b < grid; ++b) { d += p->h_dbl[b]; q2 += p->h_dbl[kMaxGrid + b]; }
    *f = lam;
    *dual = lam + d;
    *gnorm = std::sqrt(q2);
    guard.ok = true;
    return MACHIP_OK;
}

int machip_fw_run(machip_problem* p, int64_t k, int first_iter, int max_iters, double gap_tol, double grad_tol, double tol, int max_steps,
                  int warm_start, double* upper_inout, double* f_traj, double* dual_traj, double* gnorm_traj, machip_solve_stats* stats,
                  int* modes, int* iters_done) {
    if (!p || p->csr_only || max_iters < 0 || first_iter < 0 || !upper_inout || !iters_done) return fail(MACHIP_BAD_ARG, "machip_fw_run: bad argument");
    double u = *upper_inout;
    int done = 0;
    *iters_done = 0;
    for (int i = 0; i < max_iters; ++i) {
        double f = 0.0, dual = 0.0, gn = 0.0;
        machip_solve_stats st;
        memset(&st, 0, sizeof(st));
        const int rc = machip_fw_step(p, k, first_iter + i, tol, max_steps, (warm_start && (first_iter + i) > 0) ? 1 : 0, &f, &dual, &gn, &st);
        if (rc != MACHIP_OK) { *upper_inout = u; *iters_done = done; return rc; }
        u = std::min(u, dual);
        if (f_traj) f_traj[i] = f;
        if (dual_traj) dual_traj[i] = dual;
        if (gnorm_traj) gnorm_traj[i] = gn;
        if (stats) stats[i] = st;
        if (modes) { modes[2 * i] = p->sol.last_mode; modes[2 * i + 1] = (int)p->sol.last_wb_s; }
        done = i + 1;
        if (gn < grad_tol) break;
        if ((u - f) < gap_tol * std::fabs(f)) break;
        ST_TRY(machip_fw_commit(p));
    }
    *upper_inout = u; *iters_done = done;
    return MACHIP_OK;
}

int machip_round_nearest(machip_problem* p, int64_t k, int decimals, double* rounded_out) {
    if (!p || p->csr_only || !rounded_out) return fail(MACHIP_BAD_ARG, "bad argument");
    if (decimals > 15) return fail(MACHIP_BAD_ARG, "decimals must be <= 15");
    HIP_TRY(hipSetDevice(p->device));
    const long m = p->m;
    if (m == 0) return MACHIP_OK;
    if (!p->scratch_m) ST_TRY(dev_alloc(&p->scratch_m, (size_t)m + 64));
    const int grid = std::max(1, (int)std::min<long>(kMaxGrid, (m + kBlock - 1) / kBlock));
    double* r = p->s;
    const bool tb = decimals >= 0;
    if (tb) k_round_keys<<<grid, kBlock, 0, p->stream>>>(p->x, m, std::pow(10.0, decimals), r);
    else HIP_TRY(hipMemcpyAsync(r, p->x, sizeof(double) * (size_t)m, hipMemcpyDeviceToDevice, p->stream));
// ... 26 lines not shown

int machip_fiedler_csr(int device, int64_t n, const int32_t* indptr, const int32_t* indices, const double* data,
                       double tol, int max_steps, const double* x0, double* lambda2, double* v_out, double* X_out,
                       int q, machip_solve_stats* stats) {
    if (!indptr || !indices || !data || !lambda2) return fail(MACHIP_BAD_ARG, "NULL argument");
    if (n < 2 || n > 2000000000ll) return fail(MACHIP_BAD_ARG, "n must be in [2, 2e9]");
    if (X_out && (q < 1 || q > 4)) return fail(MACHIP_BAD_ARG, "q must be in [1,4]");
    const long nnz = indptr[n];
    if (indptr[0] != 0 || nnz < 0) return fail(MACHIP_BAD_ARG, "bad indptr: indptr[0] must be 0 and indptr[n] >= 0 (int32 row pointers: nnz < 2^31)");
    for (int64_t r = 0; r < n; ++r)
        if (indptr[r + 1] < indptr[r]) return fail(MACHIP_BAD_ARG, "indptr not monotone");
    double lnorm = 0.0;
    int maxlen_csr = 0;
    long chain_cnt = 0;
    for (int64_t r = 0; r < n; ++r) {
        double s = 0.0;
        for (long pp = indptr[r]; pp < (long)indptr[r + 1]; ++pp) {
            if (indices[pp] < 0 || indices[pp] >= n) return fail(MACHIP_BAD_ARG, "column index out of range");
            s += std::fabs(data[pp]);
            if (indices[pp] == r + 1 && data[pp] != 0.0) ++chain_cnt;
        }
        lnorm = std::max(lnorm, s);
        maxlen_csr = std::max(maxlen_csr, (int)(indptr[r + 1] - indptr[r]));
    }
    if (machip_device_count() <= 0) return fail(MACHIP_NO_DEVICE, "no HIP device visible");
    HIP_TRY(hipSetDevice(device));
    std::unique_lock<std::mutex> lk(g_csr_mu, std::try_to_lock);
    machip_problem* p = nullptr;
    bool cached = false;
    if (lk.owns_lock() && g_csr_cache && g_csr_cache->device == device && g_csr_cache->n == (int)n && (long)g_csr_cache->sol.csr_cap >= nnz) {
        p = g_csr_cache;
        cached = true;
    } else {
        if (lk.owns_lock() && g_csr_cache) { machip_destroy(g_csr_cache); g_csr_cache = nullptr; }
        p = new machip_problem();
        p->device = device; p->n = (int)n; p->csr_only = true;
    }
    auto body = [&]() -> int {
        if (!cached) {
            const size_t cap = (size_t)nnz + (size_t)nnz / 4 + 64;
            HIP_TRY(hipStreamCreateWithFlags(&p->stream, hipStreamNonBlocking));
            ST_TRY(dev_alloc(&p->rowptr, (size_t)n + 1)); ST_TRY(dev_alloc(&p->col, cap)); ST_TRY(dev_alloc(&p->val, cap));
            ST_TRY(alloc_common(p));
            p->sol.csr_cap = cap;
        }
        HIP_TRY(hipMemcpyAsync(p->rowptr, indptr, sizeof(int) * ((size_t)n + 1), hipMemcpyHostToDevice, p->stream));
        if (nnz) {
            HIP_TRY(hipMemcpyAsync(p->col, indices, sizeof(int) * (size_t)nnz, hipMemcpyHostToDevice, p->stream));
            HIP_TRY(hipMemcpyAsync(p->val, data, sizeof(double) * (size_t)nnz, hipMemcpyHostToDevice, p->stream));
        }
        HIP_TRY(hipStreamSynchronize(p->stream));
        p->nnz = nnz; p->lnorm = lnorm; p->maxlen = maxlen_csr; p->assembled = true; p->have_vec = false;
        Solver& S = p->sol;
        S.have_prev = false; S.warm_skip = 0; S.warm_fails = 0; S.last_pr = 0.0; S.have_start = false; S.hist_lan_steps = -1; S.hist_lob_iters = -1; S.hist_exact_iters = -1; S.last_steps = 0;
        S.last_steps_lowp = 0; S.J_last = 0; S.last_was_lob = false; S.last_seq_f32 = false; S.solver_mode = 0; S.precision = 0;
        S.opt = default_options();
        p->sol.chain_like = chain_cnt >= (long)(0.98 * (double)(n - 1));
        p->sol.chain_edges = chain_cnt;
        p->support = std::max<long>(0, (nnz - n) / 2 - chain_cnt);
        return MACHIP_OK;
    };
    int st = body();
    if (st == MACHIP_OK) st = machip_fiedler(p, tol, max_steps, x0, 0, lambda2, v_out, X_out, q, stats);
    const std::string keep = g_err;
    const bool hard = st != MACHIP_OK && st != MACHIP_NOT_CONVERGED && st != MACHIP_DISCONNECTED;
    if (lk.owns_lock() && !hard) g_csr_cache = p;
    else {
        if (cached) g_csr_cache = nullptr;
        machip_destroy(p);
    }
    g_err = keep;
    return st;
}

void machip_release_cache(void) {
    std::lock_guard<std::mutex> lk(g_csr_mu);
    if (g_csr_cache) { machip_destroy(g_csr_cache); g_csr_cache = nullptr; }
}

int machip_spmv(machip_problem* p, const double* v, double* y, int variant) {
    if (!p || !v || !y) return fail(MACHIP_BAD_ARG, "NULL argument");
    HIP_TRY(hipSetDevice(p->device));
    if (!p->assembled) ST_TRY(assemble(p));
    HIP_TRY(hipMemcpyAsync(p->sol.y_raw, v, sizeof(double) * (size_t)p->n, hipMemcpyHostToDevice, p->stream));
    const SpmvPlan pl = plan_spmv(p->sol.opt, p->n, p->nnz, variant);
    OpPlain op{p->sol.w2};
    launch_spmv(pl, p->stream, p->csr(), p->sol.y_raw, op);
    HIP_TRY(hipMemcpyAsync(y, p->sol.w2, sizeof(double) * (size_t)p->n, hipMemcpyDeviceToHost, p->stream));
    HIP_TRY(hipStreamSynchronize(p->stream));
    return MACHIP_OK;
}

int machip_landscape(machip_problem* p, int sweeps, double* u_out) {
    if (!p || !u_out || sweeps < 0 || sweeps > 16) return fail(MACHIP_BAD_ARG, "bad argument (0 <= sweeps <= 16)");
    HIP_TRY(hipSetDevice(p->device));
    if (!p->assembled) ST_TRY(assemble(p));
    const SpmvPlan pl = p->sol.landscape_plan(p->nnz);
    const double* f = p->sol.landscape_field(p->csr(), pl, sweeps);
    HIP_TRY(hipGetLastError());
    HIP_TRY(hipMemcpyAsync(u_out, f, sizeof(double) * (size_t)p->n, hipMemcpyDeviceToHost, p->stream));
    HIP_TRY(hipStreamSynchronize(p->stream));
    return MACHIP_OK;
}

int machip_profile_spmv(machip_problem* p, int reps, double* avg_us, double* bytes_per_launch) {
    if (!p || !avg_us || reps < 1) return fail(MACHIP_BAD_ARG, "bad argument");
    HIP_TRY(hipSetDevice(p->device));
    if (!p->assembled) ST_TRY(assemble(p));
    Solver& S = p->sol;
    const SpmvPlan pl = plan_pipe(p->sol.opt, p->n, p->nnz, p->maxlen);
    k_fill_start<<<S.vgrid(), kBlock, 0, p->stream>>>(S.u, p->n, 77ull);
    const PipeView L = S.pview(pl);
    k_pipe_init<<<pl.grid, kBlock, 0, p->stream>>>(L, S.u, (int)(++S.epoch));
    launch_pipe(pl, p->stream, p->csr(), L, 0);
    launch_pipe(pl, p->stream, p->csr(), L, 1);
    k_pipe_tail<<<1, 64, 0, p->stream>>>(L, 2);
    for (int i = 0; i < 3; ++i) launch_pipe(pl, p->stream, p->csr(), L, 0);
    HIP_TRY(hipEventRecord(S.ev0, p->stream));
    for (int i = 0; i < reps; ++i) launch_pipe(pl, p->stream, p->csr(), L, 0);
    HIP_TRY(hipEventRecord(S.ev1, p->stream));
    HIP_TRY(hipEventSynchronize(S.ev1));
    float ms = 0.f;
    HIP_TRY(hipEventElapsedTime(&ms, S.ev0, S.ev1));
    *avg_us = 1e3 * (double)ms / reps;
    if (bytes_per_launch) {
        *bytes_per_launch = (double)p->nnz * 12.0 + ((double)p->n + 1.0) * 4.0 + (double)p->n * 56.0;
    }
    return MACHIP_OK;
}

int machip_comm_unique_id(void* id128) {
    if (!id128) return fail(MACHIP_BAD_ARG, "NULL id buffer");
    static_assert(sizeof(ncclUniqueId) == 128, "ncclUniqueId is expected to be 128 bytes");
    ncclUniqueId id;
    NCCL_TRY(ncclGetUniqueId(&id));
    memcpy(id128, &id, sizeof(id));
    return MACHIP_OK;
}

int machip_comm_init(machip_problem* p, int rank, int nranks, const void* id128) {
    if (!p || p->csr_only || !id128 || nranks < 1 || rank < 0 || rank >= nranks) return fail(MACHIP_BAD_ARG, "bad argument");
    if (nranks > 64) return fail(MACHIP_BAD_ARG, "at most 64 ranks");
    if (p->comm || p->lgroup) return fail(MACHIP_BAD_ARG, "machip_comm_init: handle already belongs to a communicator");
    HIP_TRY(hipSetDevice(p->device));
    ncclUniqueId id;
    memcpy(&id, id128, sizeof(id));
    {
        const int dev = p->device;
        auto comm_out = std::make_shared<ncclComm_t>(nullptr);
        auto err_out = std::make_shared<std::string>();
        const int st = run_with_watchdog([=]() -> int {
            if (hipSetDevice(dev) != hipSuccess) { *err_out = "hipSetDevice failed"; return MACHIP_HIP_ERROR; }
            const ncclResult_t r = ncclCommInitRank(comm_out.get(), nranks, id, rank);
            if (r != ncclSuccess) { *err_out = std::string("ncclCommInitRank: ") + ncclGetErrorString(r); return MACHIP_RCCL_ERROR; }
            return MACHIP_OK;
        }, rccl_timeout_s(), "ncclCommInitRank (rank " + std::to_string(rank) + " of " + std::to_string(nranks) + ")");
        if (st != MACHIP_OK) return err_out->empty() ? st : fail((machip_status)st, *err_out);
        p->comm = *comm_out;
    }
    p->rank = rank; p->nranks = nranks;
    p->first_collective_pending = true;
    long lo, hi, shard;
    shard_plan(p->m, nranks, rank, &lo, &hi, &shard);
    p->m_pad = shard * nranks;
    return MACHIP_OK;
}

namespace {
struct IpcBlob {
    unsigned long long magic;
    int n; long m; int pid; int device;
    hipIpcMemHandle_t Z0, Z1, part, yraw, g, flags;
};
constexpr unsigned long long kIpcMagic = 0x6d61636869706331ull;
constexpr size_t kIpcFlagWords = (size_t)kIpcChannels * kMaxPeers + kIpcChannels + 8;
}

int machip_ipc_blob_bytes(void) { return (int)sizeof(IpcBlob); }

int machip_ipc_export(machip_problem* p, void* blob, int blob_bytes) {
    if (!p || p->csr_only || !blob || blob_bytes < (int)sizeof(IpcBlob)) return fail(MACHIP_BAD_ARG, "machip_ipc_export: bad argument");
    if (p->lgroup || p->ipcg) return fail(MACHIP_BAD_ARG, "machip_ipc_export: handle already belongs to a communicator");
    HIP_TRY(hipSetDevice(p->device));
    auto G = std::make_unique<IpcGroup>();
    ST_TRY(dev_alloc(&G->flags_mem, kIpcFlagWords));
    HIP_TRY(hipMemsetAsync(G->flags_mem, 0, sizeof(unsigned long long) * kIpcFlagWords, p->stream));
    HIP_TRY(hipStreamSynchronize(p->stream));
    HIP_TRY(hipHostMalloc((void**)&G->h_err, 64, hipHostMallocMapped));
    *G->h_err = 0;
    IpcBlob b;
    memset(&b, 0, sizeof(b));
// ... 173 lines not shown
        q->sol.opt = opt;
        ST_TRY(alloc_common(q, std::max(16, OPT(lane_vbudget_mb, std::max(16, OPT(vbudget_mb, 4096) / 8)))));
        q->sol.csr_cap = cap;
        q->sol.pat = q->pattern();
        q->sol.pan_allowed = p->sol.pan_allowed;
        q->sol.chain_like = p->sol.chain_like; q->sol.chain_edges = p->sol.chain_edges;
        return MACHIP_OK;
    };
    const int st = body();
    if (st != MACHIP_OK) { machip_destroy(q); return st; }
    *out = q;
    return MACHIP_OK;
}

int ensure_lane_fw(machip_problem* q) {
    if (q->lane_fw_ready) return MACHIP_OK;
    const size_t mp = (size_t)q->m + 64 * 8;
    if (!q->x_next) ST_TRY(dev_alloc(&q->x_next, mp));
    if (!q->g) ST_TRY(dev_alloc(&q->g, mp));
    if (!q->s) ST_TRY(dev_alloc(&q->s, mp));
    if (!q->hist) ST_TRY(dev_alloc(&q->hist, (6 + kSelRep) * kBins));
    if (!q->sel) ST_TRY(dev_alloc(&q->sel, 2));
    if (!q->part_fw) ST_TRY(dev_alloc(&q->part_fw, 2 * kMaxGrid));
    HIP_TRY(hipMemsetAsync(q->g, 0, sizeof(double) * mp, q->stream));
    HIP_TRY(hipStreamSynchronize(q->stream));
    q->lane_fw_ready = true;
    return MACHIP_OK;
}

int prepare_lanes(machip_problem* p, int B, bool fw, int* nl_out) {
    const bool small = p->sol.chain_like && persist_fits(p->n, std::max(0l, (long)p->P - 2 * p->sol.chain_edges));
    const Options& opt = p->sol.opt;
    int nl = std::max(1, std::min(B, std::min(16, OPT(lanes, small ? 16 : 4))));
    while ((int)p->lanes.size() < nl) {
        machip_problem* q = nullptr;
        const int st = make_lane(p, &q);
        if (st != MACHIP_OK) {
            if (p->lanes.empty()) return st;
            (void)hipGetLastError();
            nl = (int)p->lanes.size();
            break;
        }
        p->lanes.push_back(q);
    }
    HIP_TRY(hipStreamSynchronize(p->stream));
    for (int l = 0; l < nl; ++l) {
        machip_problem* q = p->lanes[(size_t)l];
        q->sol.solver_mode = p->sol.solver_mode; q->sol.precision = p->sol.precision;
        q->sol.opt = p->sol.opt;
        q->sol.throughput_lane = true;
        if (p->sol.have_start && q->seen_start_version != p->start_version) {
            HIP_TRY(hipMemcpyAsync(q->sol.start, p->sol.start, sizeof(double) * (size_t)p->n, hipMemcpyDeviceToDevice, q->stream));
            HIP_TRY(hipStreamSynchronize(q->stream));
            q->sol.have_start = true;
            q->seen_start_version = p->start_version;
        }
    }
    if (fw) for (int l = 0; l < nl; ++l) ST_TRY(ensure_lane_fw(p->lanes[(size_t)l]));
    *nl_out = nl;
    return MACHIP_OK;
}
}

int machip_eval_batch(machip_problem* p, int B, const double* X, double tol, int max_steps, double* lambda2, int* status) {
    if (!p || p->csr_only || p->is_lane || B < 0 || (B && (!X || !lambda2))) return fail(MACHIP_BAD_ARG, "machip_eval_batch: bad argument");
    if (B == 0) return MACHIP_OK;
    HIP_TRY(hipSetDevice(p->device));
    int nl = 0;
    ST_TRY(prepare_lanes(p, B, false, &nl));
    std::atomic<int> next{0};
    std::vector<int> lane_status((size_t)nl, MACHIP_OK);
    std::vector<std::string> lane_err((size_t)nl);
    auto work = [&](int l) {
        machip_problem* q = p->lanes[(size_t)l];
        if (hipSetDevice(q->device) != hipSuccess) { lane_status[(size_t)l] = MACHIP_HIP_ERROR; lane_err[(size_t)l] = "hipSetDevice failed"; return; }
        for (int b = next.fetch_add(1); b < B; b = next.fetch_add(1)) {
            int st = MACHIP_OK;
            double lam = 0.0;
            if (hipMemcpyAsync(q->x, X + (size_t)b * (size_t)q->m, sizeof(double) * (size_t)q->m, hipMemcpyHostToDevice, q->stream) != hipSuccess ||
                hipStreamSynchronize(q->stream) != hipSuccess) {
                st = fail(MACHIP_HIP_ERROR, "machip_eval_batch: copy of x failed");
            } else {
                q->assembled = false; q->xb_valid = false;
                st = assemble(q);
                q->sol.have_prev = false; q->sol.warm_skip = 0; q->sol.warm_fails = 0; q->sol.last_pr = 0.0; q->sol.hist_lan_steps = -1; q->sol.hist_lob_iters = -1; q->sol.hist_exact_iters = -1; q->sol.last_steps = 0; q->sol.last_steps_lowp = 0;
                if (st == MACHIP_OK) st = run_fiedler(q, tol, max_steps, nullptr, 0, &lam, nullptr);
            }
            lambda2[b] = lam;
            if (status) status[b] = st;
            if (st != MACHIP_OK && st != MACHIP_NOT_CONVERGED && st != MACHIP_DISCONNECTED) {
                lane_status[(size_t)l] = st; lane_err[(size_t)l] = g_err;
                return;
            }
        }
    };
    std::vector<std::thread> th;
    for (int l = 1; l < nl; ++l) th.emplace_back(work, l);
    work(0);
    for (auto& t : th) t.join();
    for (int l = 0; l < nl; ++l)
        if (lane_status[(size_t)l] != MACHIP_OK) return fail((machip_status)lane_status[(size_t)l], lane_err[(size_t)l]);
    return MACHIP_OK;
}

int machip_fw_sweep(machip_problem* p, int B, const int64_t* ks, const double* X0, int max_iters, double gap_tol,
                    double grad_tol, double tol, int max_steps, int warm_start, int round_decimals, double* X_out,
                    double* R_out, double* upper, double* f_traj, int* iters, int* status) {
    if (!p || p->csr_only || p->is_lane || B < 0 || max_iters < 0 || (B && (!ks || !X0 || !X_out || !upper || !iters || !status)))
        return fail(MACHIP_BAD_ARG, "machip_fw_sweep: bad argument");
    if (p->nranks > 1) return fail(MACHIP_BAD_ARG, "machip_fw_sweep: not on a handle that belongs to a communicator");
    if (B == 0) return MACHIP_OK;
    HIP_TRY(hipSetDevice(p->device));
    int nl = 0;
    ST_TRY(prepare_lanes(p, B, true, &nl));
    const size_t m = (size_t)p->m;
    std::atomic<int> next{0};
    std::vector<int> lane_status((size_t)nl, MACHIP_OK);
    std::vector<std::string> lane_err((size_t)nl);
    auto work = [&](int l) {
        machip_problem* q = p->lanes[(size_t)l];
        for (int b = next.fetch_add(1); b < B; b = next.fetch_add(1)) {
            Solver& S = q->sol;
            S.have_prev = false; S.warm_skip = 0; S.warm_fails = 0; S.last_pr = 0.0; S.hist_lan_steps = -1; S.hist_lob_iters = -1; S.hist_exact_iters = -1; S.last_steps = 0; S.last_steps_lowp = 0;
            int st = machip_set_x(q, X0 + (size_t)b * m);
            double u = std::numeric_limits<double>::infinity();
            int done = 0;
            for (int i = 0; i < max_iters && st == MACHIP_OK; ++i) {
                double f = 0.0, dual = 0.0, gn = 0.0;
                st = machip_fw_step(q, ks[b], i, tol, max_steps, warm_start && i > 0, &f, &dual, &gn, nullptr);
                if (st != MACHIP_OK) break;
                u = std::min(u, dual);
                if (f_traj) f_traj[(size_t)b * (size_t)max_iters + (size_t)i] = f;
                done = i + 1;
                if (gn < grad_tol) break;
                if ((u - f) < gap_tol * std::fabs(f)) break;
                st = machip_fw_commit(q);
            }
            if (st == MACHIP_OK) st = machip_get_x(q, X_out + (size_t)b * m);
            if (st == MACHIP_OK && R_out) st = machip_round_nearest(q, ks[b], round_decimals, R_out + (size_t)b * m);
            upper[b] = u; iters[b] = done; status[b] = st;
            if (st != MACHIP_OK && st != MACHIP_NOT_CONVERGED && st != MACHIP_DISCONNECTED) {
                lane_status[(size_t)l] = st; lane_err[(size_t)l] = g_err;
                return;
            }
        }
    };
    std::vector<std::thread> th;
    for (int l = 1; l < nl; ++l) th.emplace_back(work, l);
    work(0);
    for (auto& t : th) t.join();
    for (int l = 0; l < nl; ++l)
        if (lane_status[(size_t)l] != MACHIP_OK) return fail((machip_status)lane_status[(size_t)l], lane_err[(size_t)l]);
    return MACHIP_OK;
}

int machip_set_option(machip_problem* p, const char* name, int64_t value) {
    const int id = option_id(name);
    if (id < 0) return fail(MACHIP_BAD_ARG, std::string("machip_set_option: unknown option '") + (name ? name : "(null)") + "'");
    const long v = value == INT64_MIN ? kOptAuto : (long)value;
    if (!p) { default_options().v[id] = v; return MACHIP_OK; }
    p->sol.opt.v[id] = v;
    for (machip_problem* q : p->lanes) q->sol.opt.v[id] = v;
    return MACHIP_OK;
}

int machip_get_option(machip_problem* p, const char* name, int64_t* value) {
    const int id = option_id(name);
    if (id < 0 || !value) return fail(MACHIP_BAD_ARG, "machip_get_option: unknown option or NULL output");
    const long v = p ? p->sol.opt.v[id] : default_options().v[id];
    *value = v == kOptAuto ? INT64_MIN : (int64_t)v;
    return MACHIP_OK;
}

const char* machip_option_name(int i) { return (i >= 0 && i < kNumOpts) ? option_names()[i] : nullptr; }

int machip_comm_timing(machip_problem* p, double* grad_us, double* exchange_us) {
    if (!p || !grad_us || !exchange_us) return fail(MACHIP_BAD_ARG, "machip_comm_timing: NULL argument");
    *grad_us = 0.0; *exchange_us = 0.0;
    if (!p->ev_g_valid) return fail(MACHIP_BAD_ARG, "machip_comm_timing: no sharded gradient has been computed on this handle");
    HIP_TRY(hipSetDevice(p->device));
    HIP_TRY(hipEventSynchronize(p->ev_g2));
    float a = 0.f, b = 0.f;
    HIP_TRY(hipEventElapsedTime(&a, p->ev_g0, p->ev_g1));
    HIP_TRY(hipEventElapsedTime(&b, p->ev_g1, p->ev_g2));
    *grad_us = 1e3 * (double)a; *exchange_us = 1e3 * (double)b;
    return MACHIP_OK;
}

int machip_solve_mode(machip_problem* p, int64_t* closures) {
    if (!p) return -1;
    if (closures) *closures = p->sol.last_wb_s;
    return p->sol.last_mode;
}

int machip_comm_drop(machip_problem* p) {
    if (!p) return fail(MACHIP_BAD_ARG, "machip_comm_drop: NULL handle");
    if (p->lgroup) return fail(MACHIP_BAD_ARG, "machip_comm_drop: in-process communicators end with their handles");
    HIP_TRY(hipSetDevice(p->device));
    (void)hipStreamSynchronize(p->stream);
    if (p->ipcg) { p->sol.ipc = nullptr; p->ipcg.reset(); }
    if (p->comm) { (void)ncclCommAbort(p->comm); p->comm = nullptr; }
    p->first_collective_pending = false; p->ev_g_valid = false;
    p->rank = 0; p->nranks = 1; p->m_pad = p->m;
    return MACHIP_OK;
}

int machip_comm_drop_ipc(machip_problem* p) {
    if (!p || !p->ipcg) return fail(MACHIP_BAD_ARG, "machip_comm_drop_ipc: no inter-process communicator");
    HIP_TRY(hipSetDevice(p->device));
    HIP_TRY(hipStreamSynchronize(p->stream));
    p->sol.ipc = nullptr;
    p->ipcg.reset();
    if (!p->comm) { p->rank = 0; p->nranks = 1; p->m_pad = p->m; }
    return MACHIP_OK;
}

int machip_set_solver(machip_problem* p, int mode) {
    if (!p || mode < 0 || mode > 2) return fail(MACHIP_BAD_ARG, "machip_set_solver: mode must be 0 (auto), 1 (Lanczos) or 2 (preconditioned)");
    p->sol.solver_mode = mode;
    return MACHIP_OK;
}

int machip_set_precision(machip_problem* p, int precision) {
    if (!p || precision < 0 || precision > 1) return fail(MACHIP_BAD_ARG, "machip_set_precision: 0 (f64) or 1 (f32 iterate + f64 refinement)");
    p->sol.precision = precision;
    return MACHIP_OK;
}

int machip_synchronize(machip_problem* p) {
    if (!p) return fail(MACHIP_BAD_ARG, "NULL handle");
    HIP_TRY(hipSetDevice(p->device));
    HIP_TRY(hipStreamSynchronize(p->stream));
    return MACHIP_OK;
}

int machip_membench(int device, int64_t bytes, int reps, double* read_gbs, double* triad_gbs) {
    if (bytes < (1 << 20) || reps < 1 || !read_gbs || !triad_gbs) return fail(MACHIP_BAD_ARG, "machip_membench: bytes >= 1 MiB, reps >= 1, non-NULL outputs");
    if (machip_device_count() <= 0) return fail(MACHIP_NO_DEVICE, "no HIP device visible");
    HIP_TRY(hipSetDevice(device));
    const long cnt2 = (long)(bytes / 16);
    double2 *a = nullptr, *b = nullptr, *c = nullptr;
    double* out = nullptr;
    hipEvent_t e0 = nullptr, e1 = nullptr;
    hipStream_t ms_ = nullptr;
    auto body = [&]() -> int {
        HIP_TRY(hipStreamCreateWithFlags(&ms_, hipStreamNonBlocking));
        ST_TRY(dev_alloc(&a, (size_t)cnt2)); ST_TRY(dev_alloc(&b, (size_t)cnt2)); ST_TRY(dev_alloc(&c, (size_t)cnt2)); ST_TRY(dev_alloc(&out, 8));
        HIP_TRY(hipMemsetAsync(a, 0, (size_t)cnt2 * 16, ms_)); HIP_TRY(hipMemsetAsync(b, 0, (size_t)cnt2 * 16, ms_)); HIP_TRY(hipMemsetAsync(c, 0, (size_t)cnt2 * 16, ms_));
        HIP_TRY(hipEventCreate(&e0)); HIP_TRY(hipEventCreate(&e1));
        const int grid = 256 * 16;
        float ms = 0.f;
        k_mb_read<<<grid, kBlock, 0, ms_>>>(a, cnt2, out);
        HIP_TRY(hipEventRecord(e0, ms_));
        for (int r = 0; r < reps; ++r) k_mb_read<<<grid, kBlock, 0, ms_>>>(r & 1 ? b : a, cnt2, out);
        HIP_TRY(hipEventRecord(e1, ms_)); HIP_TRY(hipEventSynchronize(e1));
        HIP_TRY(hipEventElapsedTime(&ms, e0, e1));
        *read_gbs = (double)cnt2 * 16.0 * reps / (ms * 1e-3) / 1e9;
        k_mb_triad<<<grid, kBlock, 0, ms_>>>(a, b, c, 3.0, cnt2);
        HIP_TRY(hipEventRecord(e0, ms_));
        for (int r = 0; r < reps; ++r) k_mb_triad<<<grid, kBlock, 0, ms_>>>(a, b, c, 3.0, cnt2);
        HIP_TRY(hipEventRecord(e1, ms_)); HIP_TRY(hipEventSynchronize(e1));
        HIP_TRY(hipEventElapsedTime(&ms, e0, e1));
        *triad_gbs = (double)cnt2 * 48.0 * reps / (ms * 1e-3) / 1e9;
        HIP_TRY(hipGetLastError());
        return MACHIP_OK;
    };
    const int st = body();
    const std::string keep = g_err;
// ... 484 lines not shown
```

### mac_amd/csrc/options.h

```cpp
#pragma once
#include <climits>
#include <cstdlib>
#include <cstring>
#include <mutex>
#include <string>

namespace machip {

#define MACHIP_OPTION_LIST(X)                                                                                                      \
                                                                                                          \
    X(solver) X(graph) X(debug) X(chunk) X(chunk_near) X(sched) X(near_x10) X(trigger_pct) X(classic_n) X(persist) X(pchunk)      \
    X(spec_epilogue) X(spec_slack_pct) X(f32_switch_e9) X(tailless) X(stream) X(stream_trigger_pct) X(stream_retry_pct) X(stream_look) X(stream_margin) X(stream_window) X(stream_far) X(start_land) X(start_pow) X(start_floor_e6) X(start_land_pr_permille) X(start_land_min_mean10)                                                                \
                                                                        \
    X(spmv) X(g) X(unroll) X(block) X(maxgrid) X(defer) X(tpr) X(ell)                                                              \
                                                                                                            \
    X(panel) X(panel_min_n) X(panel_min_mean10) X(panel_multi_min_mean10) X(panel_np) X(panel_nb) X(panel_b2) X(panel_g2)         \
    X(panel_cells) X(panel_maxcells) X(panel_band) X(panel_u) X(panel_u_amp) X(pan32) X(pan32_switch_e9) X(panel_ops) X(panel_rev)                                                                               \
                                                                                                 \
    X(woodbury) X(wb_max) X(wb_hard) X(wb_lane_max) X(exact_big) X(exact_switch) X(gj_look_min) X(lob_density_pct) X(lob_chunk)   \
    X(lob_patience) X(lob_small_s) X(lob_fuse)                                                                                     \
     \
    X(sel_small) X(sel_fuse) X(asm_g) X(asm_maxgrid) X(vbudget_mb) X(vcap) X(lanes) X(lane_vbudget_mb) X(lane_queues) X(shard_eig) X(ipc_panel) \
    X(rccl_timeout_s)                                                                                                              \
               \
    X(esp_free_split)

enum OptId {
#define X(n) kOpt_##n,
    MACHIP_OPTION_LIST(X)
#undef X
    kNumOpts
};

constexpr long kOptAuto = LONG_MIN;

inline const char* const* option_names() {
    static const char* const names[] = {
#define X(n) #n,
        MACHIP_OPTION_LIST(X)
#undef X
        nullptr};
    return names;
}
inline int option_id(const char* name) {
    if (!name) return -1;
    const char* const* nm = option_names();
    for (int i = 0; i < kNumOpts; ++i) if (!strcmp(nm[i], name)) return i;
    return -1;
}

struct Options {
    long v[kNumOpts];
    int get(OptId id, int dflt) const { return v[id] == kOptAuto ? dflt : (int)v[id]; }
    bool is_set(OptId id) const { return v[id] != kOptAuto; }
};

inline long option_parse(int id, const char* s) {
    if (id == kOpt_solver) {
        if (!strcmp(s, "auto")) return 0;
        if (!strcmp(s, "lanczos")) return 1;
        if (!strcmp(s, "lobpcg")) return 2;
    }
    if (id == kOpt_spmv) {
        if (!strcmp(s, "stream")) return 1;
        if (!strcmp(s, "vec")) return 2;
    }
    if (id == kOpt_lane_queues) {
        if (!strcmp(s, "shared")) return 1;
        if (!strcmp(s, "cumask")) return 0;
    }
    return atol(s);
}

inline Options& default_options() {
    static Options D;
    static std::once_flag once;
    std::call_once(once, [] {
        const char* const* nm = option_names();
        for (int i = 0; i < kNumOpts; ++i) {
            D.v[i] = kOptAuto;
            std::string e = "MACHIP_";
            for (const char* c = nm[i]; *c; ++c) e += (char)(*c >= 'a' && *c <= 'z' ? *c - 32 : *c);
            const char* s = getenv(e.c_str());
            if (s && *s) D.v[i] = option_parse(i, s);
        }
    });
    return D;
}

#define OPT(name, dflt) (opt.get(kOpt_##name, (dflt)))

}
```

### mac_amd/csrc/solver.h

```cpp
#pragma once
#include <functional>
#include <dlfcn.h>

#include <array>
#include <deque>
#include <limits>
#include <map>
#include <mutex>
#include <tuple>
#include <vector>

#include "kernels.h"
#include "persist.h"
#include "precond.h"
#include "woodbury.h"
#include "panel.h"
#include "plan.h"
#include "tridiag.h"
#include "follow.h"

namespace machip {


struct IpcGroup {
    int nranks = 0, rank = 0;
    IpcView view;
    void* Z0[kMaxPeers] = {};
    void* Z1[kMaxPeers] = {};
    double* part[kMaxPeers] = {};
    double* yraw[kMaxPeers] = {};
    double* g[kMaxPeers] = {};
    std::vector<void*> opened;
    unsigned long long* flags_mem = nullptr;
    int* h_err = nullptr;
    int g0 = 0, g1 = 0;
    bool clean_exit = false;
    ~IpcGroup() {
        for (void* q : opened) (void)hipIpcCloseMemHandle(q);
        if (flags_mem) (void)hipFree(flags_mem);
        if (h_err) (void)hipHostFree(h_err);
    }
};

struct Solver {
    Options opt = default_options();
    int n = 0;
    hipStream_t stream = nullptr;
    size_t vcap = 0;
    double *u = nullptr, *V = nullptr, *tri = nullptr, *part = nullptr;
    Z2 *Z0 = nullptr, *Z1 = nullptr;
    LanState* st = nullptr;
    double *y_raw = nullptr, *w2 = nullptr, *yvec = nullptr, *ypart = nullptr, *sdev = nullptr;
    double *part_c = nullptr, *part_a2 = nullptr, *part_r = nullptr, *scratch3 = nullptr, *rq_dev = nullptr;
    LanState* st2 = nullptr;
    double *wc = nullptr, *ctri = nullptr, *part_u = nullptr, *part_a = nullptr;
    LanState* stc = nullptr;
    float* valf = nullptr;
    size_t valf_cap = 0, csr_cap = 0;
    bool last_seq_f32 = false;
    long last_steps_lowp = 0;
    double* start = nullptr;
    bool have_start = false, have_prev = false;
    int ks_max = 16;
    double* h_tri = nullptr;
    double* d_htri = nullptr;
    double* d_hpin = nullptr;
    unsigned long long* h_flag = nullptr;
    unsigned long long* d_hflag = nullptr;
    unsigned int epoch = 0;
    double* h_pin = nullptr;
    hipEvent_t ev0 = nullptr, ev1 = nullptr, evs0 = nullptr, evs1 = nullptr;
    bool ev1_at_check = false;
    std::function<void()> after_check;
    long check_seq = 0, hook_seq = -1, final_check_seq = -2;
    bool spec_likely = true;
    std::vector<hipEvent_t> ev_pool;
    std::map<std::tuple<int, int, int, int, int>, std::array<hipGraphExec_t, 2>> graphs;
    unsigned graph_flip = 0;
    const void* graph_csr_key = nullptr;
    bool profiled = false;
    double launch_us_hist[8] = {0, 0, 0, 0, 0, 0, 0, 0};
    double cur_launch_us = 0.0;
    bool use_graph(double launch_us = 0.0) const {
        if (opt.is_set(kOpt_graph)) return OPT(graph, 1) != 0;
        if (profiled) return false;
        if (throughput_lane) return false;
        return launch_us > 0.0 && launch_us < 5.2;
    }
    std::vector<double> ha, hb, hl1;
    std::vector<double> wk, guess;
    tri::Smallest sm;
    int J_last = 0;
    long last_steps = 0;
    int maxlen_hint = 0;
    double *lx_x = nullptr, *lx_Lx = nullptr, *lx_p = nullptr, *lx_Lp = nullptr, *lx_Lw = nullptr;
    double *lx_rT = nullptr, *lx_wT = nullptr, *lx_tl = nullptr, *lx_tdinv = nullptr, *lx_tcu = nullptr;
    double *lx_ys = nullptr, *lx_pas = nullptr, *lx_as = nullptr, *lx_bs = nullptr;
    double* lx_maps = nullptr;
    double *lx_ba = nullptr, *lx_bd = nullptr, *lx_bu = nullptr;
    int *wb_ui = nullptr, *wb_uj = nullptr, *wb_counts = nullptr;
    double *wb_uc = nullptr, *wb_g = nullptr, *wb_h = nullptr, *wb_Zt = nullptr, *wb_Cm = nullptr;
    size_t wb_Zt_cap = 0, wb_pas_cap = 0;
    double *wb_pas = nullptr, *wb_maps = nullptr;
    double* wb_Cm2 = nullptr;
    double* wb_piv = nullptr;
    WbView wb_active{};
    double *lx_part = nullptr, *lx_partR = nullptr;
    int *lx_colT = nullptr, *lx_bad = nullptr;
    PersistPack ppack{};
    int* ell_col = nullptr;
    double* ell_val = nullptr;
    CsrView ell_view{};
    size_t lx_colT_cap = 0;
    LobState* lx_st = nullptr;
    double *h_lrec = nullptr, *d_hlrec = nullptr;
    bool lob_ready = false, last_was_lob = false;
    int last_mode = 0;
    long last_wb_s = 0;
    int solver_mode = 0;
    bool throughput_lane = false;
    int precision = 0;
    bool chain_like = false;
    long chain_edges = 0;
    long support_hint = -1;
    long hist_lan_steps = -1, hist_lob_iters = -1;
    long hist_exact_iters = -1;
    static constexpr int kSwitchToExact = 1000;
    double switch_est_us = 0.0;
    double switch_to_go = 0.0;
    static constexpr int kLobCap = 100000;
    bool seq_sharded = false;
    bool seq_ipc = false;
    SpmvPlan seq_plan;
    ShardGroup* shard = nullptr;
    IpcGroup* ipc = nullptr;
    bool last_seq_sharded = false;
    bool pan_allowed = false;
    PanPlan pan;
    PanView panv{};
    bool pan_live = false;
    bool pan_u = false;
    PanU pu{};
    PeerSet* d_ps = nullptr; PeerSet h_ps{};
    double *pu_sig = nullptr, *pu_U0 = nullptr, *pu_U1 = nullptr;
    double last_amp = 0.0;
    bool pan32 = false;
    int pan32_from = INT_MAX;
    float* pan_bv32 = nullptr;
    size_t pan_bv32_cap = 0;
    size_t pan_cap = 0, pan_nt_cap = 0, pan_y_cap = 0, pan_band_cap = 0;
    std::array<int, 5> pan_shape_key{0, 0, 0, 0, 0};
    PatternView pat{};
    bool pan_rows_ready = false;
    int pan_rows_NP = 0, pan_rows_C = 0; bool pan_rows_band = false;

    int init(int n_, hipStream_t s, int budget_mb = 0) {
        n = n_;
        stream = s;
        size_t budget = (size_t)(budget_mb > 0 ? budget_mb : OPT(vbudget_mb, 4096)) * (size_t)(1 << 20);
        vcap = budget / (sizeof(double) * (size_t)std::max(n, 1));
        vcap = std::max<size_t>(std::min<size_t>(vcap, 16384), 64);
        vcap = std::min<size_t>(vcap, (size_t)n + 10);
        vcap = std::max<size_t>(vcap, 64);
        vcap = (size_t)OPT(vcap, (int)vcap);
        profiled = dlopen("librocprofiler-sdk.so", RTLD_NOLOAD | RTLD_LAZY) != nullptr ||
                   dlopen("librocprofiler-sdk.so.1", RTLD_NOLOAD | RTLD_LAZY) != nullptr;
        ST_TRY(dev_alloc(&u, n));
        ST_TRY(dev_alloc(&V, (size_t)n * vcap));
        ST_TRY(dev_alloc(&tri, 3 * (vcap + 2)));
        ST_TRY(dev_alloc(&part, 2 * kNP * kMaxGrid));
        ST_TRY(dev_alloc(&Z0, n)); ST_TRY(dev_alloc(&Z1, n));
        ST_TRY(dev_alloc(&st, 1)); ST_TRY(dev_alloc(&st2, 1));
        HIP_TRY(hipMemsetAsync(st2, 0, sizeof(LanState), stream));
        ST_TRY(dev_alloc(&y_raw, (size_t)n + 2)); ST_TRY(dev_alloc(&w2, (size_t)n + 2)); ST_TRY(dev_alloc(&yvec, n));
        ST_TRY(dev_alloc(&ypart, (size_t)n * ks_max)); ST_TRY(dev_alloc(&sdev, vcap + 2));
        ST_TRY(dev_alloc(&part_c, 3 * kMaxGrid)); ST_TRY(dev_alloc(&part_a2, kMaxGrid));
        ST_TRY(dev_alloc(&part_r, kMaxGrid)); ST_TRY(dev_alloc(&scratch3, 8)); ST_TRY(dev_alloc(&rq_dev, 1));
        ST_TRY(dev_alloc(&start, n));
        ST_TRY(dev_alloc(&wc, n)); ST_TRY(dev_alloc(&ctri, 3 * (vcap + 2)));
        ST_TRY(dev_alloc(&part_u, 3 * kMaxGrid)); ST_TRY(dev_alloc(&part_a, kMaxGrid)); ST_TRY(dev_alloc(&stc, 1));
        HIP_TRY(hipHostMalloc((void**)&h_tri, 3 * (vcap + 2) * sizeof(double), hipHostMallocMapped));
        HIP_TRY(hipHostGetDevicePointer((void**)&d_htri, h_tri, 0));
        HIP_TRY(hipHostMalloc((void**)&h_flag, 64, hipHostMallocMapped));
        HIP_TRY(hipHostGetDevicePointer((void**)&d_hflag, h_flag, 0));
        *h_flag = 0;
        HIP_TRY(hipHostMalloc((void**)&h_pin, (4 * (vcap + 2) + 2 * kMaxGrid + 64) * sizeof(double), hipHostMallocMapped));
        HIP_TRY(hipHostGetDevicePointer((void**)&d_hpin, h_pin, 0));
        HIP_TRY(hipEventCreate(&ev0)); HIP_TRY(hipEventCreate(&ev1));
        HIP_TRY(hipEventCreate(&evs0)); HIP_TRY(hipEventCreate(&evs1));
        return MACHIP_OK;
    }
    void destroy() {
        for (auto& kv : graphs) for (hipGraphExec_t ge : kv.second) if (ge) (void)hipGraphExecDestroy(ge);
        graphs.clear();
        void* ptrs[] = {u, V, tri, part, Z0, Z1, st, st2, y_raw, w2, yvec, ypart, sdev,
                        part_c, part_a2, part_r, scratch3, rq_dev, start, wc, ctri, part_u, part_a, stc,
                        lx_x, lx_Lx, lx_p, lx_Lp, lx_Lw, lx_rT, lx_wT, lx_tl, lx_tdinv, lx_tcu, lx_part, lx_partR,
                        lx_ys, lx_pas, lx_as, lx_bs, lx_maps, lx_ba, lx_bd, lx_bu, wb_ui, wb_uj, wb_counts, wb_uc, wb_g, wb_h, wb_Zt, wb_Cm, wb_Cm2, wb_piv, wb_pas, wb_maps,
                        lx_colT, lx_bad, lx_st, valf};
        {
            void* pb[] = {panv.tptr, panv.thead, panv.bval, panv.bcol, panv.ypart, panv.coef, panv.cbase, panv.ps, panv.tick, panv.claim, panv.ovf, panv.bd, panv.bpk};
            for (void* q : pb) if (q) (void)hipFree(q);
            void* pu_[] = {pu_U0, pu_U1, pu.W, pu_sig, pan_bv32, d_ps};
            for (void* q : pu_) if (q) (void)hipFree(q);
            void* pk[] = {ppack.band, ppack.cc, ppack.crow, ppack.ccol, ppack.cval, ell_col, ell_val};
            for (void* q : pk) if (q) (void)hipFree(q);
        }
        if (h_lrec) (void)hipHostFree(h_lrec);
        for (void* p : ptrs) if (p) (void)hipFree(p);
        if (h_tri) (void)hipHostFree(h_tri);
        if (h_flag) (void)hipHostFree(h_flag);
        if (h_pin) (void)hipHostFree(h_pin);
        if (ev0) (void)hipEventDestroy(ev0);
        if (ev1) (void)hipEventDestroy(ev1);
        if (evs0) (void)hipEventDestroy(evs0);
        if (evs1) (void)hipEventDestroy(evs1);
        for (hipEvent_t e : ev_pool) (void)hipEventDestroy(e);
    }

    bool start_guess = false;
    static constexpr int kWarmSkip = 7;
    int warm_skip = 0, warm_fails = 0;
    double last_pr = 0.0;
    SpmvPlan landscape_plan(long nnz) const { return plan_spmv(opt, n, nnz, kAuto, 3 * kMaxGrid); }
    const double* landscape_field(const CsrView& A, const SpmvPlan& pl, int sweeps, int* grid_out = nullptr) {
        k_land_init<<<vgrid(), kBlock, 0, stream>>>(A, wc, y_raw);
        double *src = y_raw, *dst = w2;
        const bool via_panel = pan_live && OPT(panel_ops, 1) != 0;
        for (int s = 0; s < sweeps; ++s) {
            OpLand op{src, dst, wc, part_c, 0.0};
            if (via_panel) panel_spmv(src, op, vgrid());
            else launch_spmv(pl, stream, A, src, op);
            std::swap(src, dst);
        }
        if (grid_out) *grid_out = via_panel ? vgrid() : pl.grid;
        return src;
    }
    template <class Op>
    void panel_spmv(const double* x, const Op& op, int grid) {
        const int g1 = pan.NB * pan.NP;
        const PipeView L = pview(SpmvPlan());
        switch (pan.LPT * 10 + pan.TWT) {
#define MACHIP_PANU_CASE(LP, TW) case LP * 10 + TW: k_pan_mul8<LP, TW, double><<<g1, kPanThreads, 0, stream>>>(x, panv.tptr, panv.thead, panv.bval, panv.bcol, panv.n, panv.C, panv.NP | (panv.TWW << 16), panv.NTB << 16, panv, L, -1); break;
#define MACHIP_PANU_ROW(LP) MACHIP_PANU_CASE(LP, 3) MACHIP_PANU_CASE(LP, 5) MACHIP_PANU_CASE(LP, 8)
            MACHIP_PANU_ROW(1) MACHIP_PANU_ROW(2) MACHIP_PANU_ROW(3) MACHIP_PANU_ROW(4) MACHIP_PANU_ROW(5) MACHIP_PANU_ROW(6)
            MACHIP_PANU_ROW(7) MACHIP_PANU_ROW(8) MACHIP_PANU_CASE(9, 3)
#undef MACHIP_PANU_ROW
#undef MACHIP_PANU_CASE
            default: break;
        }
        k_pan_rowop<Op><<<grid, kBlock, 0, stream>>>(panv, x, op);
    }
    int landscape_start(const CsrView& A, const SpmvPlan& pl) {
        const int sweeps = std::min(16, OPT(start_land, 3));
        if (sweeps <= 0) return MACHIP_OK;
        const double pw = (double)std::max(1, OPT(start_pow, 128));
        int gmax = pl.grid;
        const double* f = landscape_field(A, pl, sweeps, &gmax);
        const double floor_w = 1e-6 * (double)std::max(0, OPT(start_floor_e6, 1000));
        k_land_weight<<<vgrid(), kBlock, 0, stream>>>(f, part_c, gmax, u, n, pw, floor_w);
        HIP_TRY(hipGetLastError());
        return MACHIP_OK;
    }
    int vgrid() const { return (int)std::min<long>(kMaxGrid, ((long)n + kBlock - 1) / kBlock); }

    template <typename T = double>
    PipeViewT<T> pview(const SpmvPlan& pl) const {
        PipeViewT<T> L;
        L.n = n; L.st = st; L.Z0 = reinterpret_cast<ZRec<T>*>(Z0); L.Z1 = reinterpret_cast<ZRec<T>*>(Z1); L.V = reinterpret_cast<T*>(V); L.tri = tri; L.htri = d_htri; L.hflag = d_hflag; L.part = part; L.P = pl.grid; L.chunk = 0; L.pub = 0; L.pubstep = 0;
        L.sig = (pl.variant == kPanel && pan_u) ? pu_sig : nullptr;
        return L;
    }
    LanView check_view(const SpmvPlan& pl) const {
        LanView L;
        L.n = n; L.st = st2; L.u = y_raw; L.w = w2; L.V = yvec; L.alpha = scratch3; L.beta = scratch3 + 2;
        L.l1 = scratch3 + 4; L.part_u = part_c; L.P_u = vgrid(); L.part_a = part_a2; L.P_a = pl.grid;
        return L;
    }

    LanView classic_view(const SpmvPlan& pl) const {
        LanView L;
        L.n = n; L.st = stc; L.u = u; L.w = wc; L.V = V; L.alpha = ctri; L.beta = ctri + (vcap + 2);
        L.l1 = ctri + 2 * (vcap + 2); L.part_u = part_u; L.P_u = vgrid(); L.part_a = part_a; L.P_a = pl.grid;
        return L;
    }
    void enqueue_classic(const CsrView& A, const SpmvPlan& pl, int steps) {
        OpLanczos op;
        op.L = classic_view(pl);
        const int g2 = vgrid();
        for (int s = 0; s < steps; ++s) {
            launch_spmv(pl, stream, A, op.L.u, op);
            k_lan_update<<<g2, kBlock, 0, stream>>>(op.L);
        }
        k_lan_tail<<<1, kBlock, 0, stream>>>(op.L);
    }

    template <typename T = double>
    PersistViewT<T> persist_view() const {
        PersistViewT<T> L;
        L.n = n; L.st = st; L.u = u; L.vprev = wc; L.V = reinterpret_cast<T*>(V); L.tri = tri; L.htri = d_htri; L.hflag = d_hflag;
        return L;
    }
    int pack_persist(const CsrView& A) {
        if (!ppack.band) {
            ST_TRY(dev_alloc(&ppack.band, 5 * (size_t)kPersistPad)); ST_TRY(dev_alloc(&ppack.cc, 2 * (size_t)kPersistPad));
            ST_TRY(dev_alloc(&ppack.crow, (size_t)kPersistPad + 1));
            ST_TRY(dev_alloc(&ppack.ccol, kPersistPackEntries)); ST_TRY(dev_alloc(&ppack.cval, kPersistPackEntries));
        }
        k_persist_pack<<<1, 1024, 0, stream>>>(A, ppack);
        HIP_TRY(hipGetLastError());
        return MACHIP_OK;
    }
    template <typename T>
    void launch_persist_t(const CsrView& A, int steps) {
        const PersistViewT<T> L = persist_view<T>();
        switch ((n + kPersistThreads - 1) / kPersistThreads) {
            case 1: case 2: k_lan_persist<2, T><<<1, kPersistThreads, 0, stream>>>(ppack, L, steps); break;
            case 3: k_lan_persist<3, T><<<1, kPersistThreads, 0, stream>>>(ppack, L, steps); break;
            case 4: k_lan_persist<4, T><<<1, kPersistThreads, 0, stream>>>(ppack, L, steps); break;
            case 5: k_lan_persist<5, T><<<1, kPersistThreads, 0, stream>>>(ppack, L, steps); break;
            default: k_lan_persist<6, T><<<1, kPersistThreads, 0, stream>>>(ppack, L, steps); break;
        }
    }
    void launch_persist(const CsrView& A, int steps, bool f32 = false) {
        if (f32) launch_persist_t<float>(A, steps); else launch_persist_t<double>(A, steps);
    }

    int pan_spec_prepare(PanSpec* out) {
        *out = PanSpec();
        pan_rows_ready = false;
        if (!pan_allowed || !pat.prow) return MACHIP_OK;
        const PanPlan sh = plan_panel(opt, n, 0, 1, true, (long)csr_cap, true, OPT(stream, 1) != 0);
        if (!sh.on) return MACHIP_OK;
        ST_TRY(pan_row_buffers(sh, sh.band));
        HIP_TRY(hipMemsetAsync(panv.ovf, 0, sizeof(int), stream));
        out->NP = sh.NP; out->C = sh.C; out->band = sh.band ? 1 : 0;
        out->ps = panv.ps; out->bd = panv.bd; out->bpk = panv.bpk; out->ovf = panv.ovf;
        pan_rows_ready = true; pan_rows_NP = sh.NP; pan_rows_C = sh.C; pan_rows_band = sh.band;
        return MACHIP_OK;
    }
    template <class T>
    int pan_regrow(T** ptr, size_t count, bool* dropped) {
        if (*ptr) { if (!*dropped) { HIP_TRY(hipStreamSynchronize(stream)); drop_graphs(); *dropped = true; } (void)hipFree(*ptr); *ptr = nullptr; }
        return dev_alloc(ptr, count);
    }
    int pan_row_buffers(const PanPlan& pn, bool band) {
        bool dropped = false;
        if ((size_t)pn.NP * (size_t)n > pan_y_cap) {
            ST_TRY(pan_regrow(&panv.ypart, (size_t)pn.NP * ((size_t)n + 2), &dropped));
            ST_TRY(pan_regrow(&panv.ps, ((size_t)pn.NP + 1) * (size_t)n, &dropped));
            pan_y_cap = (size_t)pn.NP * (size_t)n;
            pan_rows_ready = false;
        }
        if (!panv.ovf) ST_TRY(dev_alloc(&panv.ovf, 1));
        if (band && (size_t)n > pan_band_cap) {
            ST_TRY(pan_regrow(&panv.bd, 3 * (size_t)n, &dropped)); ST_TRY(pan_regrow(&panv.bpk, (size_t)n, &dropped));
            pan_band_cap = (size_t)n;
            pan_rows_ready = false;
        }
        return MACHIP_OK;
    }
    int ensure_panel(const CsrView& A, long nnz, const PanPlan& pn, bool band, bool rows_ready) {
        const size_t cells = (size_t)pn.NB * pn.NP, NTP = (size_t)kPanWork * pn.TWW;
        const size_t NT = cells * NTP;
        bool dropped = false;
        if (NT > pan_nt_cap) {
            ST_TRY(pan_regrow(&panv.tptr, cells * (NTP + 1) + 1, &dropped)); ST_TRY(pan_regrow(&panv.thead, NT * 64, &dropped));
            pan_nt_cap = NT;
        }
        ST_TRY(pan_row_buffers(pn, band));
        if (!panv.coef) ST_TRY(dev_alloc(&panv.coef, 8));
        panv.band = band ? 1 : 0;
        panv.rev = OPT(panel_rev, 1) != 0 ? 1 : 0;
#ifdef PAN_CLOCKS
        if (!panv.clk) { ST_TRY(dev_alloc(&panv.clk, (size_t)16 * kMaxGrid)); HIP_TRY(hipMemsetAsync(panv.clk, 0, sizeof(long long) * 16 * kMaxGrid, stream)); }
#endif
        panv.n = n; panv.NP = pn.NP; panv.C = pn.C; panv.NB = pn.NB; panv.NTB = pn.NTB; panv.TWW = pn.TWW; panv.CELLS = pn.cells;
        const std::array<int, 5> key{pn.NP, pn.C, pn.NB, pn.NTB, pn.TWW};
        if (!panv.cbase || key != pan_shape_key) {
            HIP_TRY(hipStreamSynchronize(stream));
            if (!dropped) { drop_graphs(); dropped = true; }
            if (panv.cbase) { (void)hipFree(panv.cbase); panv.cbase = nullptr; }
            ST_TRY(dev_alloc(&panv.cbase, cells + 1));
            std::vector<int> cnt(cells + 1, 0);
            if (pat.prow) {
                HIP_TRY(hipMemsetAsync(panv.cbase, 0, sizeof(int) * (cells + 1), stream));
                k_pan_cellcap<<<(n + kBlock - 1) / kBlock, kBlock, 0, stream>>>(pat, 64 * pn.NTB, pn.C, pn.NP, panv.cbase);
                HIP_TRY(hipGetLastError());
                HIP_TRY(hipMemcpyAsync(cnt.data(), panv.cbase, sizeof(int) * cells, hipMemcpyDeviceToHost, stream));
                HIP_TRY(hipStreamSynchronize(stream));
            } else {
                return fail(MACHIP_BAD_ARG, "column-panel form without a pattern");
            }
            std::vector<int> base(cells + 1, 0);
            size_t run = 0;
            for (size_t c = 0; c < cells; ++c) {
                base[c] = (int)run;
                run += (((size_t)cnt[c] + (size_t)64 * pn.NTB + 63) / 64) * 64 + (size_t)64 * (kPanMaxLen + 1);
                if (run > 2000000000ull) return fail(MACHIP_BAD_ARG, "column-panel form exceeds int32 indexing");
            }
            base[cells] = (int)run;
            HIP_TRY(hipMemcpyAsync(panv.cbase, base.data(), sizeof(int) * (cells + 1), hipMemcpyHostToDevice, stream));
            HIP_TRY(hipStreamSynchronize(stream));
            if (run + kPanSlack > pan_cap) {
                ST_TRY(pan_regrow(&panv.bval, run + kPanSlack, &dropped)); ST_TRY(pan_regrow(&panv.bcol, run + kPanSlack, &dropped));
                pan_cap = run + kPanSlack;
            }
            pan_shape_key = key;
        }
        if (!rows_ready) {
            HIP_TRY(hipMemsetAsync(panv.ovf, 0, sizeof(int), stream));
            k_pan_rows<<<(n + kBlock - 1) / kBlock, kBlock, 0, stream>>>(A, panv);
            pan_rows_ready = true; pan_rows_NP = pn.NP; pan_rows_C = pn.C; pan_rows_band = band;
        }
        {
            const int g = pan_build_grid(pn.NB, pn.NP);
            switch ((64 * pn.NTB + kPanThreads - 1) / kPanThreads) {
                case 1: k_pan_build<1><<<g, kPanThreads, 0, stream>>>(A, panv); break;
                case 2: k_pan_build<2><<<g, kPanThreads, 0, stream>>>(A, panv); break;
                case 3: k_pan_build<3><<<g, kPanThreads, 0, stream>>>(A, panv); break;
                case 4: k_pan_build<4><<<g, kPanThreads, 0, stream>>>(A, panv); break;
                case 5: k_pan_build<5><<<g, kPanThreads, 0, stream>>>(A, panv); break;
                case 6: k_pan_build<6><<<g, kPanThreads, 0, stream>>>(A, panv); break;
                case 7: k_pan_build<7><<<g, kPanThreads, 0, stream>>>(A, panv); break;
                default: k_pan_build<8><<<g, kPanThreads, 0, stream>>>(A, panv); break;
            }
        }
        HIP_TRY(hipGetLastError());
        (void)nnz;
        return MACHIP_OK;
    }
#ifdef PAN_CLOCKS
#define MACHIP_FINU_CLK , (const PeerSet*)nullptr, 0, 0, panv.clk
#else
#define MACHIP_FINU_CLK
#endif
    void launch_pan_step(const PipeView& L, int s, int jhost = -1) {
        const int g1 = pan.NB * pan.NP;
        if (pan_u) {
            if (pan32 && jhost >= 0 && jhost >= pan32_from) {
                switch (pan.LPT) {
#define MACHIP_PANU32_CASE(LP) case LP: k_pan_mul8<LP, 3, float><<<g1, kPanThreads, 0, stream>>>(PAN_MUL8_ARGS(panv, pu, L, s), pan_bv32); break;
                    MACHIP_PANU32_CASE(1) MACHIP_PANU32_CASE(2) MACHIP_PANU32_CASE(3) MACHIP_PANU32_CASE(4) MACHIP_PANU32_CASE(5) MACHIP_PANU32_CASE(6)
                    MACHIP_PANU32_CASE(7) MACHIP_PANU32_CASE(8) MACHIP_PANU32_CASE(9)
#undef MACHIP_PANU32_CASE
                    default: break;
                }
            } else
            switch (pan.LPT * 10 + pan.TWT) {
#define MACHIP_PANU_CASE(LP, TW) case LP * 10 + TW: k_pan_mul8<LP, TW><<<g1, kPanThreads, 0, stream>>>(PAN_MUL8_ARGS(panv, pu, L, s)); break;
#define MACHIP_PANU_ROW(LP) MACHIP_PANU_CASE(LP, 3) MACHIP_PANU_CASE(LP, 5) MACHIP_PANU_CASE(LP, 8)
                MACHIP_PANU_ROW(1) MACHIP_PANU_ROW(2) MACHIP_PANU_ROW(3) MACHIP_PANU_ROW(4) MACHIP_PANU_ROW(5) MACHIP_PANU_ROW(6)
                MACHIP_PANU_ROW(7) MACHIP_PANU_ROW(8) MACHIP_PANU_CASE(9, 3)
#undef MACHIP_PANU_ROW
#undef MACHIP_PANU_CASE
                default: break;
            }
            const int npm = pan.NP <= 6 ? 6 : pan.NP <= 8 ? 8 : pan.NP <= 12 ? 12 : 16;
            switch (pan.block2 * 100 + npm) {
#define MACHIP_FINU_CASE(B, M) case B * 100 + M: k_pan_finu<B, M><<<pan.grid2, B, 0, stream>>>(PAN_FINU_ARGS(panv, pu, L, s, jhost) MACHIP_FINU_CLK); break;
#define MACHIP_FINU_ROW(B) MACHIP_FINU_CASE(B, 6) MACHIP_FINU_CASE(B, 8) MACHIP_FINU_CASE(B, 12) MACHIP_FINU_CASE(B, 16)
                MACHIP_FINU_ROW(256) MACHIP_FINU_ROW(512) MACHIP_FINU_ROW(1024)
#undef MACHIP_FINU_ROW
#undef MACHIP_FINU_CASE
                default: break;
            }
            return;
        }
        if (pan.cells > 1) {
            const int gm = pan.NP * ((pan.NB + pan.cells - 1) / pan.cells);
            switch (pan.RPT) {
#define MACHIP_PAN_CASE(R) case R: k_pan_mul_multi<R><<<gm, kPanThreads, 0, stream>>>(PAN_MUL_ARGS(panv, L, s)); break;
                MACHIP_PAN_CASE(1) MACHIP_PAN_CASE(2) MACHIP_PAN_CASE(3) MACHIP_PAN_CASE(4) MACHIP_PAN_CASE(5) MACHIP_PAN_CASE(6)
                MACHIP_PAN_CASE(7) MACHIP_PAN_CASE(8) MACHIP_PAN_CASE(9) MACHIP_PAN_CASE(10) MACHIP_PAN_CASE(11) MACHIP_PAN_CASE(12)
#undef MACHIP_PAN_CASE
                default: k_pan_mul_multi<13><<<gm, kPanThreads, 0, stream>>>(PAN_MUL_ARGS(panv, L, s)); break;
            }
        } else switch (pan.RPT) {
#define MACHIP_PAN_CASE(R) case R: k_pan_mul<R><<<g1, kPanThreads, 0, stream>>>(PAN_MUL_ARGS(panv, L, s)); break;
            MACHIP_PAN_CASE(1) MACHIP_PAN_CASE(2) MACHIP_PAN_CASE(3) MACHIP_PAN_CASE(4) MACHIP_PAN_CASE(5) MACHIP_PAN_CASE(6)
            MACHIP_PAN_CASE(7) MACHIP_PAN_CASE(8) MACHIP_PAN_CASE(9) MACHIP_PAN_CASE(10) MACHIP_PAN_CASE(11) MACHIP_PAN_CASE(12)
#undef MACHIP_PAN_CASE
            default: k_pan_mul<13><<<g1, kPanThreads, 0, stream>>>(PAN_MUL_ARGS(panv, L, s)); break;
        }
        if (pan.block2 == 1024) k_pan_fin<1024><<<pan.grid2, 1024, 0, stream>>>(PAN_FIN_ARGS(panv, L, s));
        else if (pan.block2 == 512) k_pan_fin<512><<<pan.grid2, 512, 0, stream>>>(PAN_FIN_ARGS(panv, L, s));
        else k_pan_fin<256><<<pan.grid2, 256, 0, stream>>>(PAN_FIN_ARGS(panv, L, s));
    }

    void shard_split(const SpmvPlan& pl) {
        const int R = (int)shard->rk.size();
        for (int r = 0; r < R; ++r) { shard->rk[(size_t)r].g0 = (int)((long)pl.grid * r / R); shard->rk[(size_t)r].g1 = (int)((long)pl.grid * (r + 1) / R); }
    }
    PeerSet shard_peers(const ShardRank& me, const SpmvPlan& pl) const {
        PeerSet PS;
        PS.n = (int)shard->rk.size(); PS.first = me.g0; PS.total = pl.grid;
        for (int q = 0; q < PS.n; ++q) { PS.Z0[q] = shard->rk[(size_t)q].Z0; PS.Z1[q] = shard->rk[(size_t)q].Z1; PS.part[q] = shard->rk[(size_t)q].part; }
        return PS;
    }
    void launch_chunk_sharded(const SpmvPlan& pl, int steps) {
        ShardGroup& G = *shard;
        const int R = (int)G.rk.size();
        shard_split(pl);
        (void)hipEventRecord(G.fork, stream);
        for (int q = 1; q < R; ++q) (void)hipStreamWaitEvent(G.rk[(size_t)q].stream, G.fork, 0);
        for (int s = 0; s < steps; ++s) {
            for (int r = 0; r < R; ++r) {
                ShardRank& me = G.rk[(size_t)r];
                if (s > 0) for (int q = 0; q < R; ++q) if (q != r) (void)hipStreamWaitEvent(me.stream, G.rk[(size_t)q].ev[(s - 1) & 1], 0);
                if (me.g1 > me.g0) {
                    if (!G.same_device) (void)hipSetDevice(me.device);
                    PipeView L = pview(pl);
                    L.Z0 = me.Z0; L.Z1 = me.Z1; L.V = me.V; L.part = me.part;
// ... 558 lines not shown
                if (est > 0.0) {
                    hist.emplace_back(jend, std::log(est));
                    while (hist.size() > 2 && hist[1].first <= jend - 48) hist.pop_front();
                    to_go = 1e18;
                    if (hist.front().first < jend) {
                        const double slope = (hist.front().second - hist.back().second) / (double)(jend - hist.front().first);
                        if (slope > 1e-7) to_go = std::max(0.0, (hist.back().second - ltarget) / slope);
                    }
                }
                if (bad || !(est == est) || est < tol * scale || jend >= cap || jend - best_it > patience) check = true;
                if (!wb && may_escalate && !check && ((jend >= 1500 && to_go > 3000.0) || jend >= 6000)) {
                    HIP_TRY(hipStreamSynchronize(stream));
                    *iters = it_enq; *restarts_out = restarts;
                    lob_escalate = true;
                    if (debug) fprintf(stderr, "[machip] lobpcg it=%d: escalating to the exact preconditioner (to_go %.0f)\n", jend, std::min(to_go, 1e9));
                    return MACHIP_NOT_CONVERGED;
                }
            }
            HIP_TRY(hipStreamSynchronize(stream));
            HIP_TRY(hipMemcpyAsync(y_raw, lx_x, sizeof(double) * (size_t)n, hipMemcpyDeviceToDevice, stream));
            k_vec_sums<<<g2, kBlock, 0, stream>>>(y_raw, n, part_c);
            ST_TRY(check_vector(A, pl, &rq, &r1));
            *spmvs += 1;
            *iters = it_enq;
            *restarts_out = restarts;
            if (debug) fprintf(stderr, "[machip]    lobpcg check it=%d rq=%.15g res=%.3e (tol %.1e)\n", it_enq, rq, r1 / scale, tol);
            if (!(rq == rq)) return MACHIP_NOT_CONVERGED;
            *lam = rq; *res = r1 / scale;
            if (*res < tol) return MACHIP_OK;
            if (it_enq >= cap || ++restarts > 12 || it_enq - best_it > patience) return MACHIP_NOT_CONVERGED;
        }
    }

    int solve(const CsrView& A, long nnz, double lnorm, double tol, int max_steps, int start_mode,
              int forced_variant, double* lambda2, machip_solve_stats* stats) {
        int mode = opt.is_set(kOpt_solver) ? OPT(solver, 0) : solver_mode;
        if (mode == 3) mode = 0;
        const bool eligible = n > 256 && n <= kTriBigMaxN;
        const bool small = n <= kPersistThreads * kPersistMaxRows;
        const long ratio = small ? 9 : 6;
        const bool sparse = (double)support_hint <= OPT(lob_density_pct, small ? 3 : 12) * 0.01 * (double)n;
        const bool chain_dominated = support_hint < 0 || support_hint <= 2 * (long)n;
        const bool stiff = hist_lan_steps > 2500 && (hist_lob_iters < 0 || hist_lob_iters * ratio < hist_lan_steps);
        const bool slow_lob = hist_lan_steps > 0 && hist_lob_iters > 0 && hist_lob_iters * ratio > 2 * hist_lan_steps;
        const long lob_it_guess = hist_lob_iters > 0 ? hist_lob_iters : 14;
        const double cost_lob = 60.0 + 2.7 * ((double)support_hint / 32.0) + 7.5 * (double)lob_it_guess;
        const bool exact_small = small && !throughput_lane && precision == 0 && support_hint >= 0 && support_hint <= OPT(lob_small_s, 700) &&
                                 support_hint <= wb_soft() && OPT(woodbury, 1) != 0 &&
                                 (hist_lan_steps <= 0 || cost_lob < 0.4 * (double)hist_lan_steps);
        bool exact_big = false;
        if (!small && n <= kTriMaxN && !throughput_lane && precision == 0 && support_hint > 0 && support_hint <= wb_soft() && hist_lan_steps > 0 &&
            OPT(woodbury, 1) != 0 && OPT(exact_big, 1) != 0) {
            const double sd = (double)support_hint, nd = (double)n, ldw = (double)((support_hint + kGjT - 1) / kGjT * kGjT);
            const double its = hist_exact_iters > 0 ? (double)hist_exact_iters : 14.0;
            const double est_exact = 120.0 + 4e-6 * nd * sd + 1.1e-5 * sd * sd + (ldw / kGjB) * (13.0 + 3.5e-6 * ldw * ldw) +
                                     its * (45.0 + 1.2e-6 * nd * sd + 2.5e-6 * sd * sd);
            exact_big = est_exact < 0.8 * (double)hist_lan_steps * (4.2 + 2e-6 * (double)nnz);
        }
        const bool want = chain_dominated &&
                          (mode == 2 || (mode == 0 && chain_like && support_hint >= 0 && ((sparse && !slow_lob) || stiff || exact_small || exact_big)));
        last_was_lob = false;
        final_check_seq = -2;
        bool after_switch = false;
        long pre_steps = 0;
        if (!(eligible && want) && mode == 0 && eligible && chain_dominated && chain_like && !small && n <= kTriMaxN && !throughput_lane &&
            precision == 0 && forced_variant == 0 && support_hint > 0 && support_hint <= wb_soft() &&
            OPT(woodbury, 1) != 0 && OPT(exact_big, 1) != 0 && OPT(exact_switch, 1) != 0) {
            const double sd = (double)support_hint, nd = (double)n, ldw = (double)((support_hint + kGjT - 1) / kGjT * kGjT);
            const double its = hist_exact_iters > 0 ? (double)hist_exact_iters : 14.0;
            switch_est_us = 120.0 + 4e-6 * nd * sd + 1.1e-5 * sd * sd + (ldw / kGjB) * (13.0 + 3.5e-6 * ldw * ldw) +
                            its * (45.0 + 1.2e-6 * nd * sd + 2.5e-6 * sd * sd);
            const int st = solve_lanczos(A, nnz, lnorm, tol, max_steps, start_mode, forced_variant, lambda2, stats);
            switch_est_us = 0.0;
            if (st != kSwitchToExact) {
                if (st == MACHIP_OK) hist_lan_steps = last_steps - (long)(0.35 * (double)last_steps_lowp);
                return st;
            }
            after_switch = true;
            pre_steps = last_steps;
            hist_lan_steps = last_steps + (long)std::min(switch_to_go, 1e6);
        }
        if ((eligible && want) || after_switch) {
            if (!after_switch) HIP_TRY(hipEventRecord(ev0, stream));
            double lam = 0.0, res = 0.0;
            long iters = 0, spmvs = 0, rst = 0;
            wb_limit_now = throughput_lane ? std::min(wb_soft(), OPT(wb_lane_max, 256)) : wb_soft();
            int st = solve_lob(A, nnz, lnorm, tol, max_steps, start_mode, &lam, &res, &iters, &spmvs, &rst);
            if (st == MACHIP_NOT_CONVERGED && lob_escalate) {
                long it1 = iters, sp1 = spmvs;
                wb_limit_now = wb_hard();
                st = solve_lob(A, nnz, lnorm, tol, max_steps, start_mode, &lam, &res, &iters, &spmvs, &rst);
                iters += it1; spmvs += sp1;
            }
            if (st == MACHIP_OK) {
                HIP_TRY(hipEventRecord(ev1, stream));
                HIP_TRY(hipEventSynchronize(ev1));
                float ms = 0.f;
                HIP_TRY(hipEventElapsedTime(&ms, ev0, ev1));
                last_mode = wb_active.s > 0 ? 7 : 6; last_wb_s = wb_active.s;
                have_prev = true; last_was_lob = true; last_steps = iters; J_last = 0;
                last_seq_sharded = false;
                hist_lob_iters = iters;
                if (wb_active.s > 0) hist_exact_iters = iters;
                *lambda2 = lam;
                if (stats) {
                    stats->lanczos_steps = iters + pre_steps; stats->spmv_total = spmvs + pre_steps; stats->vec_passes = iters * 16 + pre_steps * 7;
                    stats->restarts = rst; stats->nnz = nnz; stats->residual = res; stats->lnorm = lnorm; stats->gpu_ms = ms;
                    stats->step_ms = ms; stats->steps_timed = iters + pre_steps; stats->steps_lowp = 0;
                }
                if (lam < 1e-12 * (lnorm > 0 ? lnorm : 1.0))
                    return fail(MACHIP_DISCONNECTED, "lambda_2 ~ 0: the graph is not connected");
                return MACHIP_OK;
            }
            if (st != MACHIP_NOT_CONVERGED) return st;
        }
        const int st = solve_lanczos(A, nnz, lnorm, tol, max_steps, start_mode, forced_variant, lambda2, stats);
        if (st == MACHIP_OK) hist_lan_steps = last_steps - (long)(0.35 * (double)last_steps_lowp);
        return st;
    }

    int solve_lanczos(const CsrView& A, long nnz, double lnorm, double tol, int max_steps, int start_mode,
                      int forced_variant, double* lambda2, machip_solve_stats* stats) {
        const SpmvPlan pl = plan_spmv(opt, n, nnz, forced_variant, n > 32768 ? kMaxGrid : 0);
        SpmvPlan pp = plan_pipe(opt, n, nnz, maxlen_hint);
        const int g2 = vgrid();
        HIP_TRY(hipEventRecord(ev0, stream));
        ev1_at_check = false;
        if (max_steps <= 0) max_steps = 200000;
        long steps_total = 0, spmv_total = 0, restarts = 0;
        long steps_used = 0;
        double step_ms_acc = 0.0;
        long steps_timed_acc = 0;
        int status = MACHIP_NOT_CONVERGED;
        bool switch_out = false;
        double lam = 0.0, res = 0.0;
        const double tiny_l = (lnorm > 0 ? lnorm : 1.0);
        if (n < 2) { *lambda2 = 0.0; return fail(MACHIP_BAD_ARG, "graph with a single node has no Fiedler pair"); }

        const bool pmode_early = OPT(persist, 1) != 0 && chain_like && persist_fits(n, nnz - n - 2 * chain_edges);
        const double* begin_src = nullptr;
        const bool land_local = last_pr <= 0.0 || last_pr <= 0.001 * (double)std::max(1, OPT(start_land_pr_permille, 20)) * (double)n;
        const bool land_dense = 10.0 * (double)nnz >= (double)std::max(0, OPT(start_land_min_mean10, 60)) * (double)n;
        const bool land_ok = !start_guess && !pmode_early && n > OPT(classic_n, 256) && OPT(start_land, 3) > 0 && land_local && land_dense;
        bool warm = start_mode == 1 && have_prev;
        if (warm && land_ok && warm_skip > 0) { --warm_skip; warm = false; }
        const bool warm_probe = warm && land_ok;
        double start_overlap = -1.0;
        if (warm) {
            if (pmode_early) begin_src = yvec;
            else HIP_TRY(hipMemcpyAsync(u, yvec, sizeof(double) * (size_t)n, hipMemcpyDeviceToDevice, stream));
        } else if (have_start) {
            if (pmode_early) begin_src = start;
            else HIP_TRY(hipMemcpyAsync(u, start, sizeof(double) * (size_t)n, hipMemcpyDeviceToDevice, stream));
        } else {
            k_fill_start<<<g2, kBlock, 0, stream>>>(u, n, 0x1234567ull);
        }

        pan_live = false;

        const int chunk0 = std::min(kMaxChunk, std::max(2, OPT(chunk, 32) & ~1));
        const int chunk_near = std::min(chunk0, std::max(2, OPT(chunk_near, 8) & ~1));
        if (max_steps & 1) ++max_steps;
        const double trigger_slack = 0.01 * OPT(trigger_pct, 110);
        const double near_factor = 0.1 * OPT(near_x10, 20);
        std::deque<Pending> pend;
        bool done = false;

        bool classic = n <= OPT(classic_n, 256);
        const bool pmode = pmode_early;
        pan = plan_panel(opt, n, nnz, maxlen_hint, pan_allowed && !pmode && !classic && pp.variant == kVec && !shard, (long)csr_cap,
                         false, OPT(stream, 1) != 0);
        pan_u = false; last_amp = 0.0; pan32 = false; pan32_from = INT_MAX;
        if (ipc && !(pan.on && pan.u && precision == 0 && (long)pan.grid2 * pan.block2 >= (long)n && pan.grid2 >= ipc->nranks && OPT(ipc_panel, 1) != 0)) pan.on = false;
        if (precision == 1 && !(pan.on && pan.u && pan.TWT == 3 && OPT(pan32, 1) != 0)) pan.on = false;
        if (!pan.on && !pmode && !classic && !shard && !ipc && precision == 0 && pp.variant == kVec && pp.width == 4 && pp.defer < 3 &&
            maxlen_hint >= 1 && maxlen_hint <= 16 && OPT(ell, 1) != 0) {
            const int W = maxlen_hint <= 8 ? 8 : 16;
            if (!ell_col) { ST_TRY(dev_alloc(&ell_col, (size_t)n * 16)); ST_TRY(dev_alloc(&ell_val, (size_t)n * 16)); }
            k_ell_build<<<(int)std::min<long>(kMaxGrid, ((long)n * W + kBlock - 1) / kBlock), kBlock, 0, stream>>>(A, W, ell_col, ell_val);
            HIP_TRY(hipGetLastError());
            ell_view = CsrView{n, nullptr, ell_col, ell_val};
            pp.variant = kEll; pp.unroll = W / 4;
        }
        if (pan.on) {
            const bool rows_ready = pan_rows_ready && !pan.verify && pan_rows_NP == pan.NP && pan_rows_C == pan.C && pan_rows_band == pan.band;
            ST_TRY(ensure_panel(A, nnz, pan, pan.band, rows_ready));
            if (pan.verify) {
                int over = 0;
                HIP_TRY(hipMemcpyAsync(&over, panv.ovf, sizeof(int), hipMemcpyDeviceToHost, stream));
                HIP_TRY(hipStreamSynchronize(stream));
                if (over) pan.on = false;
            }
        }
        if (pan.on) {
            pp.variant = kPanel; pp.grid = pan.grid2; pp.block = pan.block2;
            pp.width = pan.NP * 100 + pan.RPT; pp.unroll = pan.TWW; pp.defer = pan.NB + 10000 * pan.cells + (pan.u ? 1000000 : 0);
            if (pan.u) {
                if (!pu_U0) {
                    ST_TRY(dev_alloc(&pu_U0, (size_t)n + 2)); ST_TRY(dev_alloc(&pu_U1, (size_t)n + 2)); ST_TRY(dev_alloc(&pu.W, (size_t)n));
                    ST_TRY(dev_alloc(&pu_sig, 2));
                    pu.sig = pu_sig;
                }
                pu.U0 = ipc ? reinterpret_cast<double*>(Z0) : pu_U0;
                pu.U1 = ipc ? reinterpret_cast<double*>(Z1) : pu_U1;
                pan_u = true;
                if (precision == 1 && !use_graph(launch_us_hist[kPanel] > 0.0 ? launch_us_hist[kPanel] : 8.0)) {
                    if (pan_bv32_cap < pan_cap) {
                        HIP_TRY(hipStreamSynchronize(stream));
                        if (pan_bv32) (void)hipFree(pan_bv32);
                        pan_bv32 = nullptr; pan_bv32_cap = 0;
                        ST_TRY(dev_alloc(&pan_bv32, pan_cap));
                        pan_bv32_cap = pan_cap;
                    }
                    k_to_f32<<<(int)std::min<long>(kMaxGrid, ((long)pan_cap + kBlock - 1) / kBlock), kBlock, 0, stream>>>(panv.bval, pan_bv32, (long)pan_cap);
                    pan32 = true;
                }
            }
        }
        pan_live = pan.on && pan_u;
        if (!warm && land_ok) ST_TRY(landscape_start(A, landscape_plan(nnz)));
        {
            const int vk = std::max(0, std::min(7, (int)pp.variant));
            cur_launch_us = launch_us_hist[vk] > 0.0 ? launch_us_hist[vk] : (pp.variant == kPanel ? 8.0 : 4.2 + 2e-6 * (double)nnz);
        }
        if (OPT(debug, 0)) fprintf(stderr, "[machip] fused steps: variant %d, %.2f us per launch (%s) -> %s\n", (int)pp.variant, cur_launch_us, launch_us_hist[std::max(0, std::min(7, (int)pp.variant))] > 0.0 ? "measured" : "model", use_graph(cur_launch_us) ? "captured chunks" : "eager launches");
        const PipeView L = pview(pp);
        const int pchunk0 = std::min(kPersistMaxSteps, std::max(2, OPT(pchunk, 64)));
        const bool debug = OPT(debug, 0) != 0;
        bool f32_seq = precision == 1 && !classic && pp.variant == kVec;
        const double f32_switch = std::max(std::max(tol, 1e-9 * (double)OPT(f32_switch_e9, 2000)),
                                           3e-7 * std::sqrt((double)n));
        long steps_lowp = 0;
        if (f32_seq && !pmode) {
            if (valf_cap < (size_t)nnz) {
                HIP_TRY(hipStreamSynchronize(stream));
                for (auto& kv : graphs) for (hipGraphExec_t ge : kv.second) if (ge) (void)hipGraphExecDestroy(ge);
                graphs.clear();
                if (valf) (void)hipFree(valf);
                valf = nullptr; valf_cap = 0;
                const size_t want = std::max<size_t>((size_t)nnz + (size_t)nnz / 2 + 1024, csr_cap);
                ST_TRY(dev_alloc(&valf, want));
                valf_cap = want;
            }
            k_to_f32<<<(int)std::min<long>(kMaxGrid, (nnz + kBlock - 1) / kBlock), kBlock, 0, stream>>>(A.val, valf, nnz);
        }
        if (pmode) ST_TRY(pack_persist(A));
        while (!done && steps_total < max_steps) {
            seq_sharded = false; seq_ipc = false;
            pan32_from = INT_MAX;
            if (pmode) {
                ++epoch;
                k_persist_begin<<<g2, kBlock, 0, stream>>>(persist_view(), (int)epoch, begin_src);
                begin_src = nullptr;
            } else if (classic) {
                k_vec_sums<<<g2, kBlock, 0, stream>>>(u, n, part_u);
                k_set_state<<<1, 64, 0, stream>>>(stc, 0);
            } else if (f32_seq) {
                ++epoch;
                k_pipe_init<<<pp.grid, kBlock, 0, stream>>>(pview<float>(pp), u, (int)epoch);
            } else {
                ++epoch;
                if (pan_u) k_pipe_init_u<<<pp.grid, kBlock, 0, stream>>>(L, pu, u, (int)epoch);
                else k_pipe_init<<<pp.grid, kBlock, 0, stream>>>(L, u, (int)epoch);
                if (shard && pp.variant == kVec) {
                    seq_sharded = true; seq_plan = pp;
                    ST_TRY(shard_broadcast_init());
                } else if (ipc && precision == 0 && ((pp.variant == kVec && pp.grid >= ipc->nranks) || (pp.variant == kPanel && pan_u))) {
                    seq_sharded = true; seq_ipc = true; seq_plan = pp;
                }
// ... 270 lines not shown
                        const size_t j = (size_t)(p.jstart + i);
                        h_tri[3 * j] = hp[i];
                        h_tri[3 * j + 1] = hp[(kMaxChunk + 2) + i];
                        h_tri[3 * j + 2] = hp[2 * (kMaxChunk + 2) + i];
                    }
                }
                const int Jold = (int)ha.size();
                const int J = p.jend;
                ha.resize((size_t)J); hb.resize((size_t)J + 1); hl1.resize((size_t)J + 1);
                for (int j = std::max(0, Jold - 1); j < J; ++j) {
                    ha[(size_t)j] = h_tri[3 * (size_t)j];
                    hl1[(size_t)j] = h_tri[3 * (size_t)j + 2];
                }
                for (int j = Jold; j <= J; ++j) hb[(size_t)j] = h_tri[3 * (size_t)j + 1];
                if (Jold == 0 && (hb[0] <= 0.0 || !(hb[0] == hb[0])))
                    return fail(MACHIP_BAD_ARG, "start vector is constant, zero or not finite");
                int Jeff = J;
                bool broke = false;
                for (int j = std::max(1, Jold); j <= J; ++j) {
                    if (!(hb[(size_t)j] > 1e-13 * tiny_l)) { Jeff = j; broke = true; break; }
                }
                tri::smallest_eigpair(ha.data(), hb.data(), Jeff, guess.data(), (int)guess.size(), theta_prev, sm, wk);
                guess = sm.s;
                theta_prev = sm.theta;
                const double rho = broke ? 0.0 : std::fabs(hb[(size_t)Jeff] * sm.s[(size_t)Jeff - 1]);
                const double l1v = hl1[(size_t)Jeff - 1] > 0 ? hl1[(size_t)Jeff - 1] : std::sqrt((double)n);
                const double est = rho * l1v;
                est_latest = est;
                if (!broke && est > 0.0) {
                    hist.emplace_back(J, std::log(est));
                    while (hist.size() > 2 && hist[1].first <= J - 64) hist.pop_front();
                    to_go = 1e18;
                    if (hist.front().first < J) {
                        const double slope = (hist.front().second - hist.back().second) / (double)(J - hist.front().first);
                        if (slope > 1e-7) to_go = std::max(0.0, (hist.back().second - ltarget) / slope);
                    }
                }
                const bool at_cap = (J >= jcap) || (steps_total >= max_steps && pend.empty());
                const bool trig = broke || est < trigger_slack * seq_tol * lnorm;
                if (switch_est_us > 0.0 && restarts == 0 && !f32_seq && !broke && !trig && !at_cap && J >= 128 && to_go < 1e17 &&
                    to_go * (4.2 + 2e-6 * (double)nnz) > 1.3 * switch_est_us) {
                    if (++switch_votes >= 2) {
                        if (debug) fprintf(stderr, "[machip]    J=%d: forecast %.0f steps to go -- handing over to the exact chain + closures mode (estimate %.0f us)\n", J, to_go, switch_est_us);
                        switch_to_go = to_go; switch_out = true; break;
                    }
                } else switch_votes = 0;

                if (debug) fprintf(stderr, "[machip] %s J=%d Jeff=%d theta=%.15g est=%.3e to_go=%.0f broke=%d pend=%zu passes=%d\n", pmode ? "persist" : (classic ? "classic" : "pipe"), J, Jeff, sm.theta, lnorm > 0 ? est / lnorm : est, std::min(to_go, 1e9), (int)broke, pend.size(), sm.passes);
                if ((trig && est < 0.5 * last_check_est) || broke || at_cap) {
                    double rq = 0.0, r1 = 0.0;
                    HIP_TRY(hipEventRecord(evs1, stream));
                    spec_likely = !f32_seq && est < 0.01 * OPT(spec_slack_pct, 105) * seq_tol * lnorm;
                    ST_TRY(explicit_check(A, pl, Jeff, sm.s.data(), &rq, &r1, f32_seq));
                    spec_likely = true;
                    {
                        float sms = 0.f;
                        HIP_TRY(hipEventElapsedTime(&sms, evs0, evs1));
                        step_ms_acc += sms; steps_timed_acc += J_enq - J_timed;
                        J_timed = J_enq;
                        HIP_TRY(hipEventRecord(evs0, stream));
                    }
                    spmv_total += 1;
                    J_last = Jeff;
                    last_check_est = std::max(est, 1e-300);
                    lam = rq;
                    res = lnorm > 0 ? r1 / lnorm : r1;
                    if (debug) fprintf(stderr, "[machip]    check J=%d rq=%.15g res=%.3e (tol %.1e)\n", Jeff, rq, res, tol);
                    if (res < tol) { converged = true; status = MACHIP_OK; final_check_seq = check_seq; break; }
                    if (broke || at_cap || f32_seq) { need_restart = true; break; }
                }
            }
            if (stream_mode && switch_out) HIP_TRY(hipStreamSynchronize(stream));
            for (const Pending& p : pend) {
                if (p.ev) { HIP_TRY(hipEventSynchronize(p.ev)); ev_pool.push_back(p.ev); }
            }
            if (!pend.empty()) HIP_TRY(hipStreamSynchronize(stream));
            pend.clear();
            last_seq_f32 = f32_seq;
            last_seq_sharded = seq_sharded;
            if (switch_out) break;
            if (converged) { done = true; break; }
            if (steps_total >= max_steps) break;
            HIP_TRY(hipMemcpyAsync(u, yvec, sizeof(double) * (size_t)n, hipMemcpyDeviceToDevice, stream));
            if (f32_seq) {
                f32_seq = false;
                if (res * tiny_l < 1e-4 * std::fabs(lam)) classic = true;
                continue;
            }
            ++restarts;
            classic = true;
            if (restarts > 64) break;
        }
        last_mode = steps_lowp > 0 ? 8 : pmode ? 4 : n <= OPT(classic_n, 256) ? 5 : pp.variant == kPanel ? 2 : pp.variant == kEll ? 3 : 1;
        if (switch_out) {
            last_steps = steps_used; last_steps_lowp = steps_lowp;
            return kSwitchToExact;
        }
        have_prev = true;
        last_steps = steps_used;
        last_steps_lowp = steps_lowp;
        if (warm_probe && start_overlap >= 0.0) {
            if (start_overlap < 2.0 / std::sqrt((double)n)) { warm_skip = std::min(63, kWarmSkip << std::min(warm_fails, 4)); ++warm_fails; }
            else warm_fails = 0;
        }
        if (OPT(debug, 0) && warm_probe) fprintf(stderr, "[machip] warm start: overlap of the previous vector with the result %.3f%s\n", start_overlap, warm_skip ? " -> the next warm requests start cold (landscape-weighted)" : "");
        if (!(ev1_at_check && status == MACHIP_OK)) {
            HIP_TRY(hipEventRecord(ev1, stream));
            HIP_TRY(hipEventSynchronize(ev1));
        }
        float ms = 0.f;
        HIP_TRY(hipEventElapsedTime(&ms, ev0, ev1));
        *lambda2 = lam;
        if (steps_timed_acc >= 16 && last_mode >= 1 && last_mode <= 3) {
            const int vk = std::max(0, std::min(7, (int)pp.variant));
            launch_us_hist[vk] = 1e3 * step_ms_acc / (double)steps_timed_acc / (pp.variant == kPanel ? 2.0 : 1.0);
        }
        if (stats) {
            stats->lanczos_steps = steps_used;
            stats->spmv_total = spmv_total;
            stats->vec_passes = steps_total * 7;
            stats->restarts = restarts;
            stats->nnz = nnz;
            stats->residual = res;
            stats->lnorm = lnorm;
            stats->gpu_ms = ms;
            stats->step_ms = step_ms_acc;
            stats->steps_timed = steps_timed_acc;
            stats->steps_lowp = steps_lowp;
            stats->drift = last_amp;
        }
        if (status == MACHIP_OK && lam < 1e-12 * tiny_l)
            return fail(MACHIP_DISCONNECTED, "lambda_2 ~ 0: the graph is not connected");
        if (status != MACHIP_OK)
            return fail(MACHIP_NOT_CONVERGED, "Lanczos hit the step cap before the residual test passed");
        return MACHIP_OK;
    }

    int ritz_block(int q, double* X_host) {
        const int Jeff = std::max(1, std::min(J_last, (int)ha.size()));
        const int ncand = std::min(Jeff, q + 6);
        std::vector<double> th, S;
        if (!last_was_lob && !last_seq_f32 && !last_seq_sharded) tri::smallest_block(ha.data(), hb.data(), Jeff, ncand, th, S, wk);
        const int g2 = vgrid();
        HIP_TRY(hipMemcpyAsync(X_host, yvec, sizeof(double) * (size_t)n, hipMemcpyDeviceToHost, stream));
        HIP_TRY(hipStreamSynchronize(stream));
        int acc = 1;
        std::vector<double> col((size_t)n);
        auto orth_accept = [&](double n0) -> bool {
            for (int pass = 0; pass < 2; ++pass)
                for (int p = 0; p < acc; ++p) {
                    const double* xp = X_host + (size_t)p * n;
                    double dot = 0.0;
                    for (int i = 0; i < n; ++i) dot += xp[i] * col[(size_t)i];
                    for (int i = 0; i < n; ++i) col[(size_t)i] -= dot * xp[i];
                }
            double n2 = 0.0;
            for (int i = 0; i < n; ++i) n2 += col[(size_t)i] * col[(size_t)i];
            if (!(n2 > 1e-6 * std::max(n0, 1e-300))) return false;
            const double inv = 1.0 / std::sqrt(n2);
            double* dst = X_host + (size_t)acc * n;
            for (int i = 0; i < n; ++i) dst[i] = col[(size_t)i] * inv;
            ++acc;
            return true;
        };
        for (int c = 1; c < (int)th.size() && acc < q; ++c) {
            memcpy(h_pin, S.data() + (size_t)c * Jeff, sizeof(double) * (size_t)Jeff);
// ... 36 lines not shown
```

Before: 130.3 iter/s.

## Add static panel layout over candidate union and skip per-iteration CSR assembly

Builds a fixed panel structure once from the union of all candidate edges plus the diagonal, then each Frank-Wolfe iteration only refreshes panel values from x through a source/weight map. Assembly can run in a rows-only mode that computes the diagonal, band terms and norm statistics without writing the CSR, and the CSR is filled lazily only when a path needs it. The aim is to remove the per-iteration CSR fill and panel rebuild. In exchange it adds a one-time setup with extra memory and a padded structure that holds inactive edges, so each SpMV may touch more entries.

```diff
diff --git a/include/machip.h b/include/machip.h
--- a/include/machip.h
+++ b/include/machip.h
@@ -97,6 +97,7 @@
 int machip_comm_drop(machip_problem* p);
 int machip_comm_timing(machip_problem* p, double* grad_us, double* exchange_us);
 int machip_solve_mode(machip_problem* p, int64_t* closures);
+int machip_panel_static_counts(machip_problem* p, int64_t* solves, int64_t* csr_fills);
 int machip_comm_mode(machip_problem* p);
 int machip_shard_plan(int64_t m, int nranks, int rank, int64_t* lo, int64_t* hi, int64_t* shard);
 
diff --git a/mac_amd/_lib.py b/mac_amd/_lib.py
--- a/mac_amd/_lib.py
+++ b/mac_amd/_lib.py
@@ -90,6 +90,7 @@
     "machip_comm_drop": (C.c_int, [C.c_void_p]),
     "machip_comm_timing": (C.c_int, [C.c_void_p, _f64p, _f64p]),
     "machip_solve_mode": (C.c_int, [C.c_void_p, C.POINTER(C.c_int64)]),
+    "machip_panel_static_counts": (C.c_int, [C.c_void_p, C.POINTER(C.c_int64), C.POINTER(C.c_int64)]),
     "machip_set_precision": (C.c_int, [C.c_void_p, C.c_int]),
     "machip_synchronize": (C.c_int, [C.c_void_p]),
     "machip_membench": (C.c_int, [C.c_int, C.c_int64, C.c_int, _f64p, _f64p]),
@@ -386,6 +387,11 @@
         c = C.c_int64(0)
         return int(self._lib.machip_solve_mode(self._h, C.byref(c))), int(c.value)
 
+    def panel_static_counts(self):
+        a, b = C.c_int64(0), C.c_int64(0)
+        check(self._lib.machip_panel_static_counts(self._h, C.byref(a), C.byref(b)))
+        return int(a.value), int(b.value)
+
     def set_option(self, name, value=None):
         if value is not None and name in CREATION_OPTIONS:
             raise ValueError(f"option {name!r} is read when the handle is created: set it with mac_amd._lib.default_options({name}=...) around the constructor")
diff --git a/mac_amd/csrc/kernels.h b/mac_amd/csrc/kernels.h
--- a/mac_amd/csrc/kernels.h
+++ b/mac_amd/csrc/kernels.h
@@ -109,14 +109,14 @@
     int* ovf = nullptr;
 };
 
-template <int G>
+template <int G, bool CSR = true>
 __global__ __launch_bounds__(kBlock) void k_asm_fill(PatternView P, const unsigned int* __restrict__ xbits, const double* __restrict__ x,
                                                      int rows_per_block,
                                                      const int* __restrict__ cnt,
                                                      const int* __restrict__ blk_sum,
                                                      int* __restrict__ rowptr, int* __restrict__ col,
                                                      double* __restrict__ val,
-                                                     double* __restrict__ blk_lnorm, PanSpec S = PanSpec()) {
+                                                     double* __restrict__ blk_lnorm, PanSpec S = PanSpec(), int* __restrict__ hsum = nullptr) {
     extern __shared__ __attribute__((aligned(16))) char smem_raw[];
     int* s_off = reinterpret_cast<int*>(smem_raw);
     __shared__ int sm_i[4];
@@ -129,9 +129,11 @@
     const int r1 = min(P.n, r0 + rows_per_block);
     const int nr = max(0, r1 - r0);
 
+    int base = 0;
+    if (CSR) {
     int acc = 0;
     for (int b = tid; b < (int)blockIdx.x; b += kBlock) acc += blk_sum[b];
-    const int base = block_sum_i(acc, sm_i);
+    base = block_sum_i(acc, sm_i);
 
     const int per = (nr + kBlock - 1) / kBlock;
     int csum = 0;
@@ -155,12 +157,14 @@
         }
     }
     __syncthreads();
+    }
 
     double lmax = 0.0;
+    int tot = 0, supp = 0, mx = 0;
     for (int r = r0 + g; r < r1; r += GPB) {
         const int b = P.prow[r], e = P.prow[r + 1];
-        const int out = base + s_off[r - r0];
-        int pos = out + 1;
+        const int out = CSR ? base + s_off[r - r0] : 0;
+        int pos = out + 1, sc = 0;
         double dsum = 0.0, asum = 0.0;
         int lastpid = 0;
         int hb = 0x7fffffff, hn = 0;
@@ -181,8 +185,11 @@
             const unsigned long long below = gm & ((1ull << lane) - 1ull);
             const int before = __popcll(below);
             const int c = act ? P.pcol[p] : 0;
-            if (act) { col[pos + before] = c; val[pos + before] = -v; }
-            if (S.NP) {
+            if (CSR && act) { col[pos + before] = c; val[pos + before] = -v; }
+            if (!CSR) {
+                sc += (act && kc >= 0);
+                if (act && S.band && (c == r - 1 || c == r + 1)) { if (c == r - 1) vl += -v; else vu += -v; }
+            } else if (S.NP) {
                 const int pid = act ? c / S.C : 0;
                 const int src = below ? 63 - __builtin_clzll(below) : 0;
                 const int got = __shfl(pid, gbase + src, kWave);
@@ -203,6 +210,15 @@
         }
         dsum = group_sum<G>(dsum);
         asum = group_sum<G>(asum);
+        if (!CSR) {
+            sc = group_sum_i<G>(sc);
+            if (S.band) {
+                vl = group_sum<G>(vl); vu = group_sum<G>(vu);
+                if (lane == 0) { S.bd[r] = dsum; S.bd[(size_t)P.n + r] = vl; S.bd[2 * (size_t)P.n + r] = vu; }
+            }
+            if (lane == 0) { tot += pos; supp += sc; mx = max(mx, pos); lmax = fmax(lmax, fabs(dsum) + asum); }
+            continue;
+        }
         if (S.NP) {
             if (lane == 0) S.ps[(size_t)r * (S.NP + 1)] = out + 1;
             for (int pp = lastpid + 1 + lane; pp <= S.NP; pp += G) S.ps[(size_t)r * (S.NP + 1) + pp] = pos;
@@ -226,6 +242,20 @@
         }
     }
     lmax = block_max(lmax, sm_d);
+    if (!CSR) {
+        tot = block_sum_i(tot, sm_i);
+        supp = block_sum_i(supp, sm_i);
+#pragma unroll
+        for (int o = 32; o > 0; o >>= 1) mx = max(mx, __shfl_xor(mx, o, kWave));
+        __syncthreads();
+        if ((tid & 63) == 0) sm_i[tid >> 6] = mx;
+        __syncthreads();
+        if (tid == 0) {
+            blk_lnorm[blockIdx.x] = lmax;
+            hsum[blockIdx.x] = tot; hsum[kAsmGrid + blockIdx.x] = supp; hsum[2 * kAsmGrid + blockIdx.x] = max(max(sm_i[0], sm_i[1]), max(sm_i[2], sm_i[3]));
+        }
+        return;
+    }
     if (tid == 0) {
         blk_lnorm[blockIdx.x] = lmax;
         if (blockIdx.x == gridDim.x - 1) rowptr[P.n] = base + s_off[nr];
@@ -359,6 +389,13 @@
         double d = 0.0;
         for (int p = A.rowptr[r], e = A.rowptr[r + 1]; p < e; ++p)
             if (A.col[p] == r) { d = A.val[p]; break; }
+        dg[r] = d;
+        u[r] = d > 0.0 ? 1.0 / d : 0.0;
+    }
+}
+__global__ __launch_bounds__(kBlock) void k_land_init_diag(const double* __restrict__ diag, int n, double* __restrict__ dg, double* __restrict__ u) {
+    for (int r = blockIdx.x * kBlock + threadIdx.x; r < n; r += gridDim.x * kBlock) {
+        const double d = diag[r];
         dg[r] = d;
         u[r] = d > 0.0 ? 1.0 / d : 0.0;
     }
diff --git a/mac_amd/csrc/machip.hip b/mac_amd/csrc/machip.hip
--- a/mac_amd/csrc/machip.hip
+++ b/mac_amd/csrc/machip.hip
@@ -99,6 +99,7 @@
     int maxlen = 0;
     double lnorm = 0.0;
     bool assembled = false, have_vec = false, csr_only = false;
+    bool csr_stale = false;
     bool band_dups_ok = true;
     unsigned int* hist = nullptr;
     SelState* sel = nullptr;
@@ -235,31 +236,56 @@
 }
 
 template <int G>
-void launch_asm(machip_problem* p, const PanSpec& S) {
+void launch_asm(machip_problem* p, const PanSpec& S, bool host_out = true, bool rows_only = false) {
     const PatternView P = p->pattern();
     const unsigned int* xb32 = reinterpret_cast<const unsigned int*>(p->xb);
-    k_asm_count<G><<<p->asm_grid, kBlock, 0, p->stream>>>(P, xb32, p->asm_rpb, p->cnt, p->blk_sum, p->d_hint);
     const size_t lds = sizeof(int) * ((size_t)p->asm_rpb + 1);
+    if (rows_only) {
+        k_asm_fill<G, false><<<p->asm_grid, kBlock, lds, p->stream>>>(P, xb32, p->x, p->asm_rpb, nullptr, nullptr, nullptr, nullptr, nullptr, p->d_hdbl, S, p->d_hint);
+        return;
+    }
+    k_asm_count<G><<<p->asm_grid, kBlock, 0, p->stream>>>(P, xb32, p->asm_rpb, p->cnt, p->blk_sum, host_out ? p->d_hint : nullptr);
     k_asm_fill<G><<<p->asm_grid, kBlock, lds, p->stream>>>(P, xb32, p->x, p->asm_rpb, p->cnt, p->blk_sum,
-                                                           p->rowptr, p->col, p->val, p->d_hdbl, S);
-}
-
-int assemble(machip_problem* p) {
-    if (p->csr_only) return fail(MACHIP_BAD_ARG, "handle wraps a caller CSR; nothing to assemble");
+                                                           p->rowptr, p->col, p->val, host_out ? p->d_hdbl : p->blk_lnorm, S);
+}
+void launch_asm_g(machip_problem* p, const PanSpec& S, bool host_out, bool rows_only) {
+    switch (p->asm_G) {
+        case 4: launch_asm<4>(p, S, host_out, rows_only); break;
+        case 8: launch_asm<8>(p, S, host_out, rows_only); break;
+        case 16: launch_asm<16>(p, S, host_out, rows_only); break;
+        case 32: launch_asm<32>(p, S, host_out, rows_only); break;
+        default: launch_asm<64>(p, S, host_out, rows_only); break;
+    }
+}
+
+int fill_csr(machip_problem* p) {
     PanSpec S;
     ST_TRY(p->sol.pan_spec_prepare(&S));
+    launch_asm_g(p, S, false, false);
+    HIP_TRY(hipGetLastError());
+    p->csr_stale = false; p->sol.csr_stale = false;
+    ++p->sol.pst_fills;
+    return MACHIP_OK;
+}
+
+int assemble(machip_problem* p, bool lazy = false) {
+    if (p->csr_only) return fail(MACHIP_BAD_ARG, "handle wraps a caller CSR; nothing to assemble");
+    bool rows_only = false;
+    if (lazy && p->nranks <= 1 && !p->lgroup && !p->ipcg && !p->comm) ST_TRY(p->sol.pst_prepare(&rows_only));
+    PanSpec S;
+    if (rows_only) {
+        S.band = 1; S.bd = p->sol.panv.bd;
+        p->sol.pan_rows_ready = false;
+    } else ST_TRY(p->sol.pan_spec_prepare(&S));
     if (!p->xb_valid) {
         const int grid = std::max(1, (int)std::min<long>(kMaxGrid, (p->m + kBlock - 1) / kBlock));
         k_x_bits<<<grid, kBlock, 0, p->stream>>>(p->x, p->m, p->tol_sel, p->xb);
         p->xb_valid = true;
     }
-    switch (p->asm_G) {
-        case 4: launch_asm<4>(p, S); break;
-        case 8: launch_asm<8>(p, S); break;
-        case 16: launch_asm<16>(p, S); break;
-        case 32: launch_asm<32>(p, S); break;
-        default: launch_asm<64>(p, S); break;
-    }
+    launch_asm_g(p, S, true, rows_only);
+    p->csr_stale = rows_only; p->sol.csr_stale = rows_only;
+    p->sol.pst_x = p->x; p->sol.pst_xb = reinterpret_cast<const unsigned int*>(p->xb);
+    if (rows_only && !p->sol.csr_fill) p->sol.csr_fill = [p] { return fill_csr(p); };
     HIP_TRY(hipGetLastError());
     const int gb = p->asm_grid;
     HIP_TRY(hipStreamSynchronize(p->stream));
@@ -398,7 +424,7 @@
 
 int run_fiedler(machip_problem* p, double tol, int max_steps, const double* x0, int warm_start,
                 double* lambda2, machip_solve_stats* stats) {
-    if (!p->assembled) ST_TRY(assemble(p));
+    if (!p->assembled) ST_TRY(assemble(p, true));
     if (x0) {
         HIP_TRY(hipMemcpyAsync(p->sol.start, x0, sizeof(double) * (size_t)p->n, hipMemcpyHostToDevice, p->stream));
         HIP_TRY(hipStreamSynchronize(p->stream));
@@ -587,6 +613,7 @@
     if (!p || !indptr || !indices || !data) return fail(MACHIP_BAD_ARG, "NULL argument");
     HIP_TRY(hipSetDevice(p->device));
     if (!p->assembled) ST_TRY(assemble(p));
+    if (p->csr_stale) ST_TRY(fill_csr(p));
     HIP_TRY(hipMemcpyAsync(indptr, p->rowptr, sizeof(int) * ((size_t)p->n + 1), hipMemcpyDeviceToHost, p->stream));
     HIP_TRY(hipMemcpyAsync(indices, p->col, sizeof(int) * (size_t)p->nnz, hipMemcpyDeviceToHost, p->stream));
     HIP_TRY(hipMemcpyAsync(data, p->val, sizeof(double) * (size_t)p->nnz, hipMemcpyDeviceToHost, p->stream));
@@ -660,7 +687,7 @@
     if (!p || p->csr_only || !f || !dual || !gnorm) return fail(MACHIP_BAD_ARG, "bad argument");
     GroupGuard guard{p};
     HIP_TRY(hipSetDevice(p->device));
-    ST_TRY(assemble(p));
+    ST_TRY(assemble(p, !(p->lgroup && p->lgroup->shard_eig)));
     double lam = 0.0;
     const int grid = std::max(1, (int)std::min<long>(kMaxGrid, (p->m + kBlock - 1) / kBlock));
     const double gamma = 2.0 / ((double)iter + 2.0);
@@ -853,6 +880,7 @@
     if (!p || !v || !y) return fail(MACHIP_BAD_ARG, "NULL argument");
     HIP_TRY(hipSetDevice(p->device));
     if (!p->assembled) ST_TRY(assemble(p));
+    if (p->csr_stale) ST_TRY(fill_csr(p));
     HIP_TRY(hipMemcpyAsync(p->sol.y_raw, v, sizeof(double) * (size_t)p->n, hipMemcpyHostToDevice, p->stream));
     const SpmvPlan pl = plan_spmv(p->sol.opt, p->n, p->nnz, variant);
     OpPlain op{p->sol.w2};
@@ -866,6 +894,7 @@
     if (!p || !u_out || sweeps < 0 || sweeps > 16) return fail(MACHIP_BAD_ARG, "bad argument (0 <= sweeps <= 16)");
     HIP_TRY(hipSetDevice(p->device));
     if (!p->assembled) ST_TRY(assemble(p));
+    if (p->csr_stale) ST_TRY(fill_csr(p));
     const SpmvPlan pl = p->sol.landscape_plan(p->nnz);
     const double* f = p->sol.landscape_field(p->csr(), pl, sweeps);
     HIP_TRY(hipGetLastError());
@@ -878,6 +907,7 @@
     if (!p || !avg_us || reps < 1) return fail(MACHIP_BAD_ARG, "bad argument");
     HIP_TRY(hipSetDevice(p->device));
     if (!p->assembled) ST_TRY(assemble(p));
+    if (p->csr_stale) ST_TRY(fill_csr(p));
     Solver& S = p->sol;
     const SpmvPlan pl = plan_pipe(p->sol.opt, p->n, p->nnz, p->maxlen);
     k_fill_start<<<S.vgrid(), kBlock, 0, p->stream>>>(S.u, p->n, 77ull);
@@ -1217,7 +1247,7 @@
                 st = fail(MACHIP_HIP_ERROR, "machip_eval_batch: copy of x failed");
             } else {
                 q->assembled = false; q->xb_valid = false;
-                st = assemble(q);
+                st = assemble(q, true);
                 q->sol.have_prev = false; q->sol.warm_skip = 0; q->sol.warm_fails = 0; q->sol.last_pr = 0.0; q->sol.hist_lan_steps = -1; q->sol.hist_lob_iters = -1; q->sol.hist_exact_iters = -1; q->sol.last_steps = 0; q->sol.last_steps_lowp = 0;
                 if (st == MACHIP_OK) st = run_fiedler(q, tol, max_steps, nullptr, 0, &lam, nullptr);
             }
@@ -1319,6 +1349,13 @@
     HIP_TRY(hipEventElapsedTime(&a, p->ev_g0, p->ev_g1));
     HIP_TRY(hipEventElapsedTime(&b, p->ev_g1, p->ev_g2));
     *grad_us = 1e3 * (double)a; *exchange_us = 1e3 * (double)b;
+    return MACHIP_OK;
+}
+
+int machip_panel_static_counts(machip_problem* p, int64_t* solves, int64_t* csr_fills) {
+    if (!p) return fail(MACHIP_BAD_ARG, "NULL handle");
+    if (solves) *solves = p->sol.pst_solves;
+    if (csr_fills) *csr_fills = p->sol.pst_fills;
     return MACHIP_OK;
 }
 
diff --git a/mac_amd/csrc/options.h b/mac_amd/csrc/options.h
--- a/mac_amd/csrc/options.h
+++ b/mac_amd/csrc/options.h
@@ -15,7 +15,7 @@
     X(spmv) X(g) X(unroll) X(block) X(maxgrid) X(defer) X(tpr) X(ell)                                                              \
                                                                                                             \
     X(panel) X(panel_min_n) X(panel_min_mean10) X(panel_multi_min_mean10) X(panel_np) X(panel_nb) X(panel_b2) X(panel_g2)         \
-    X(panel_cells) X(panel_maxcells) X(panel_band) X(panel_u) X(panel_u_amp) X(pan32) X(pan32_switch_e9) X(panel_ops) X(panel_rev)                                                                               \
+    X(panel_cells) X(panel_maxcells) X(panel_band) X(panel_u) X(panel_u_amp) X(pan32) X(pan32_switch_e9) X(panel_ops) X(panel_rev) X(panel_static)                                                                             \
                                                                                                  \
     X(woodbury) X(wb_max) X(wb_hard) X(wb_lane_max) X(exact_big) X(exact_switch) X(gj_look_min) X(lob_density_pct) X(lob_chunk)   \
     X(lob_patience) X(lob_small_s) X(lob_fuse)                                                                                     \
diff --git a/mac_amd/csrc/panel_static.h b/mac_amd/csrc/panel_static.h
--- /dev/null
+++ b/mac_amd/csrc/panel_static.h
@@ -0,0 +1,67 @@
+#pragma once
+#include "panel.h"
+
+namespace machip {
+
+struct PanStatic {
+    int* src = nullptr;
+    double* sw = nullptr;
+};
+
+__global__ __launch_bounds__(kBlock) void k_pst_union_csr(PatternView Pt, int* __restrict__ rowptr, int* __restrict__ col, double* __restrict__ val) {
+    const int r = blockIdx.x * kBlock + threadIdx.x;
+    if (r > Pt.n) return;
+    if (r == Pt.n) { rowptr[r] = Pt.prow[r] + r; return; }
+    const int b = Pt.prow[r], e = Pt.prow[r + 1], out = b + r;
+    rowptr[r] = out;
+    col[out] = r; val[out] = 0.0;
+    for (int p = b; p < e; ++p) { col[p + r + 1] = Pt.pcol[p]; val[p + r + 1] = (double)(p + 1); }
+}
+
+__global__ __launch_bounds__(kBlock) void k_pst_src(PatternView Pt, long nslots, const double* __restrict__ bval, long cap, PanStatic S) {
+    for (long e = (long)blockIdx.x * kBlock + threadIdx.x; e < cap; e += (long)gridDim.x * kBlock) {
+        const double d = bval[e];
+        int s = -2;
+        double w = 0.0;
+        if (d >= 1.0 && d <= (double)nslots) {
+            const long p = (long)d - 1;
+            const int k = Pt.pk[p];
+            s = k >= 0 ? k : -1;
+            w = Pt.pw[p];
+        }
+        S.src[e] = s; S.sw[e] = w;
+    }
+}
+
+constexpr int kPstSplit = 8;
+__global__ __launch_bounds__(kBlock) void k_pst_refresh(PanStatic S, const int* __restrict__ tptr, int NTP, int cells,
+                                                        const double* __restrict__ x, const unsigned int* __restrict__ xbits, double* __restrict__ bval) {
+    const int cell = blockIdx.x / kPstSplit, part = blockIdx.x - cell * kPstSplit;
+    if (cell >= cells) return;
+    const int t0 = tptr[(size_t)cell * (NTP + 1)], t1 = tptr[(size_t)cell * (NTP + 1) + NTP];
+    const int per = (((t1 - t0 + kPstSplit - 1) / kPstSplit) + 63) & ~63;
+    const int lo = t0 + part * per, hi = min(t1, lo + per);
+    for (int e0 = lo + threadIdx.x; e0 < hi; e0 += 4 * kBlock) {
+        int s[4];
+        double w[4], xk[4];
+        bool act[4];
+#pragma unroll
+        for (int i = 0; i < 4; ++i) {
+            const int e = min(e0 + i * kBlock, hi - 1);
+            s[i] = S.src[e]; w[i] = S.sw[e];
+        }
+#pragma unroll
+        for (int i = 0; i < 4; ++i) {
+            xk[i] = s[i] >= 0 ? x[s[i]] : 1.0;
+            act[i] = s[i] >= 0 ? x_bit(xbits, s[i]) : s[i] == -1;
+        }
+#pragma unroll
+        for (int i = 0; i < 4; ++i) {
+            const int e = e0 + i * kBlock;
+            const double v = xk[i] * w[i];
+            if (e < hi) bval[e] = act[i] ? -v : 0.0;
+        }
+    }
+}
+
+}
diff --git a/mac_amd/csrc/solver.h b/mac_amd/csrc/solver.h
--- a/mac_amd/csrc/solver.h
+++ b/mac_amd/csrc/solver.h
@@ -15,6 +15,7 @@
 #include "precond.h"
 #include "woodbury.h"
 #include "panel.h"
+#include "panel_static.h"
 #include "plan.h"
 #include "tridiag.h"
 #include "follow.h"
@@ -153,6 +154,22 @@
     PatternView pat{};
     bool pan_rows_ready = false;
     int pan_rows_NP = 0, pan_rows_C = 0; bool pan_rows_band = false;
+    int* dyn_tptr = nullptr; unsigned short *dyn_thead = nullptr, *dyn_bcol = nullptr;
+    int* pst_tptr = nullptr; unsigned short *pst_thead = nullptr, *pst_bcol = nullptr;
+    PanStatic pst{};
+    int pst_state = 0;
+    std::array<int, 5> pst_key{0, 0, 0, 0, 0};
+    bool pst_live = false;
+    bool csr_stale = false;
+    long pst_solves = 0, pst_fills = 0;
+    std::function<int()> csr_fill;
+    const double* pst_x = nullptr;
+    const unsigned int* pst_xb = nullptr;
+    int need_csr() {
+        if (!csr_stale) return MACHIP_OK;
+        csr_stale = false;
+        return csr_fill ? csr_fill() : fail(MACHIP_BAD_ARG, "no CSR of the current iterate and nobody to assemble it");
+    }
 
     int init(int n_, hipStream_t s, int budget_mb = 0) {
         n = n_;
@@ -199,7 +216,7 @@
                         lx_ys, lx_pas, lx_as, lx_bs, lx_maps, lx_ba, lx_bd, lx_bu, wb_ui, wb_uj, wb_counts, wb_uc, wb_g, wb_h, wb_Zt, wb_Cm, wb_Cm2, wb_piv, wb_pas, wb_maps,
                         lx_colT, lx_bad, lx_st, valf};
         {
-            void* pb[] = {panv.tptr, panv.thead, panv.bval, panv.bcol, panv.ypart, panv.coef, panv.cbase, panv.ps, panv.tick, panv.claim, panv.ovf, panv.bd, panv.bpk};
+            void* pb[] = {dyn_tptr, dyn_thead, dyn_bcol, pst_tptr, pst_thead, pst_bcol, pst.src, pst.sw, panv.bval, panv.ypart, panv.coef, panv.cbase, panv.ps, panv.tick, panv.claim, panv.ovf, panv.bd, panv.bpk};
             for (void* q : pb) if (q) (void)hipFree(q);
             void* pu_[] = {pu_U0, pu_U1, pu.W, pu_sig, pan_bv32, d_ps};
             for (void* q : pu_) if (q) (void)hipFree(q);
@@ -224,9 +241,10 @@
     double last_pr = 0.0;
     SpmvPlan landscape_plan(long nnz) const { return plan_spmv(opt, n, nnz, kAuto, 3 * kMaxGrid); }
     const double* landscape_field(const CsrView& A, const SpmvPlan& pl, int sweeps, int* grid_out = nullptr) {
-        k_land_init<<<vgrid(), kBlock, 0, stream>>>(A, wc, y_raw);
+        const bool via_panel = pan_live && OPT(panel_ops, 1) != 0;
+        if (pst_live && via_panel) k_land_init_diag<<<vgrid(), kBlock, 0, stream>>>(panv.bd, n, wc, y_raw);
+        else k_land_init<<<vgrid(), kBlock, 0, stream>>>(A, wc, y_raw);
         double *src = y_raw, *dst = w2;
-        const bool via_panel = pan_live && OPT(panel_ops, 1) != 0;
         for (int s = 0; s < sweeps; ++s) {
             OpLand op{src, dst, wc, part_c, 0.0};
             if (via_panel) panel_spmv(src, op, vgrid());
@@ -360,12 +378,12 @@
         }
         return MACHIP_OK;
     }
-    int ensure_panel(const CsrView& A, long nnz, const PanPlan& pn, bool band, bool rows_ready) {
+    int pan_sizes(const PanPlan& pn, bool band) {
         const size_t cells = (size_t)pn.NB * pn.NP, NTP = (size_t)kPanWork * pn.TWW;
         const size_t NT = cells * NTP;
         bool dropped = false;
         if (NT > pan_nt_cap) {
-            ST_TRY(pan_regrow(&panv.tptr, cells * (NTP + 1) + 1, &dropped)); ST_TRY(pan_regrow(&panv.thead, NT * 64, &dropped));
+            ST_TRY(pan_regrow(&dyn_tptr, cells * (NTP + 1) + 1, &dropped)); ST_TRY(pan_regrow(&dyn_thead, NT * 64, &dropped));
             pan_nt_cap = NT;
         }
         ST_TRY(pan_row_buffers(pn, band));
@@ -403,32 +421,105 @@
             HIP_TRY(hipMemcpyAsync(panv.cbase, base.data(), sizeof(int) * (cells + 1), hipMemcpyHostToDevice, stream));
             HIP_TRY(hipStreamSynchronize(stream));
             if (run + kPanSlack > pan_cap) {
-                ST_TRY(pan_regrow(&panv.bval, run + kPanSlack, &dropped)); ST_TRY(pan_regrow(&panv.bcol, run + kPanSlack, &dropped));
+                ST_TRY(pan_regrow(&panv.bval, run + kPanSlack, &dropped)); ST_TRY(pan_regrow(&dyn_bcol, run + kPanSlack, &dropped));
                 pan_cap = run + kPanSlack;
             }
             pan_shape_key = key;
         }
+        return MACHIP_OK;
+    }
+    void pan_build_launch(const CsrView& A, const PanPlan& pn) {
+        const int g = pan_build_grid(pn.NB, pn.NP);
+        switch ((64 * pn.NTB + kPanThreads - 1) / kPanThreads) {
+            case 1: k_pan_build<1><<<g, kPanThreads, 0, stream>>>(A, panv); break;
+            case 2: k_pan_build<2><<<g, kPanThreads, 0, stream>>>(A, panv); break;
+            case 3: k_pan_build<3><<<g, kPanThreads, 0, stream>>>(A, panv); break;
+            case 4: k_pan_build<4><<<g, kPanThreads, 0, stream>>>(A, panv); break;
+            case 5: k_pan_build<5><<<g, kPanThreads, 0, stream>>>(A, panv); break;
+            case 6: k_pan_build<6><<<g, kPanThreads, 0, stream>>>(A, panv); break;
+            case 7: k_pan_build<7><<<g, kPanThreads, 0, stream>>>(A, panv); break;
+            default: k_pan_build<8><<<g, kPanThreads, 0, stream>>>(A, panv); break;
+        }
+    }
+    int ensure_panel(const CsrView& A, long nnz, const PanPlan& pn, bool band, bool rows_ready, bool stat = false) {
+        ST_TRY(pan_sizes(pn, band));
+        const size_t cells = (size_t)pn.NB * pn.NP, NTP = (size_t)kPanWork * pn.TWW;
+        pst_live = stat;
+        if (panv.tptr != (stat ? pst_tptr : dyn_tptr)) {
+            HIP_TRY(hipStreamSynchronize(stream));
+            drop_graphs();
+        }
+        if (stat) {
+            ++pst_solves;
+            panv.tptr = pst_tptr; panv.thead = pst_thead; panv.bcol = pst_bcol;
+            k_pst_refresh<<<(int)cells * kPstSplit, kBlock, 0, stream>>>(pst, pst_tptr, (int)NTP, (int)cells, pst_x, pst_xb, panv.bval);
+            HIP_TRY(hipGetLastError());
+            return MACHIP_OK;
+        }
+        panv.tptr = dyn_tptr; panv.thead = dyn_thead; panv.bcol = dyn_bcol;
         if (!rows_ready) {
             HIP_TRY(hipMemsetAsync(panv.ovf, 0, sizeof(int), stream));
             k_pan_rows<<<(n + kBlock - 1) / kBlock, kBlock, 0, stream>>>(A, panv);
             pan_rows_ready = true; pan_rows_NP = pn.NP; pan_rows_C = pn.C; pan_rows_band = band;
         }
-        {
-            const int g = pan_build_grid(pn.NB, pn.NP);
-            switch ((64 * pn.NTB + kPanThreads - 1) / kPanThreads) {
-                case 1: k_pan_build<1><<<g, kPanThreads, 0, stream>>>(A, panv); break;
-                case 2: k_pan_build<2><<<g, kPanThreads, 0, stream>>>(A, panv); break;
-                case 3: k_pan_build<3><<<g, kPanThreads, 0, stream>>>(A, panv); break;
-                case 4: k_pan_build<4><<<g, kPanThreads, 0, stream>>>(A, panv); break;
-                case 5: k_pan_build<5><<<g, kPanThreads, 0, stream>>>(A, panv); break;
-                case 6: k_pan_build<6><<<g, kPanThreads, 0, stream>>>(A, panv); break;
-                case 7: k_pan_build<7><<<g, kPanThreads, 0, stream>>>(A, panv); break;
-                default: k_pan_build<8><<<g, kPanThreads, 0, stream>>>(A, panv); break;
-            }
-        }
+        pan_build_launch(A, pn);
         HIP_TRY(hipGetLastError());
         (void)nnz;
         return MACHIP_OK;
+    }
+    bool pst_shape(PanPlan* sh) const {
+        if (OPT(panel_static, 1) == 0 || OPT(panel_ops, 1) == 0 || !pan_allowed || !pat.prow || ipc || shard) return false;
+        *sh = plan_panel(opt, n, 0, 1, true, (long)csr_cap, true, OPT(stream, 1) != 0);
+        return sh->on && sh->u && sh->cells == 1 && sh->band;
+    }
+    static std::array<int, 5> pan_key(const PanPlan& pn) { return {pn.NP, pn.C, pn.NB, pn.NTB, pn.TWW}; }
+    bool pst_serves(const PanPlan& pn) const { return pst_state == 1 && pn.on && pn.u && pn.cells == 1 && pn.band && !pn.verify && pan_key(pn) == pst_key; }
+    int pst_prepare(bool* ready) {
+        *ready = false;
+        PanPlan sh;
+        if (!pst_shape(&sh)) return MACHIP_OK;
+        if (pst_state != 0 && pan_key(sh) == pst_key) { *ready = pst_state == 1; return MACHIP_OK; }
+        HIP_TRY(hipStreamSynchronize(stream));
+        drop_graphs();
+        for (void* q : {(void*)pst_tptr, (void*)pst_thead, (void*)pst_bcol, (void*)pst.src, (void*)pst.sw}) if (q) (void)hipFree(q);
+        pst_tptr = nullptr; pst_thead = nullptr; pst_bcol = nullptr; pst = PanStatic();
+        pst_state = -1; pst_key = pan_key(sh);
+        pan_rows_ready = false;
+        int slots = 0;
+        HIP_TRY(hipMemcpyAsync(&slots, pat.prow + n, sizeof(int), hipMemcpyDeviceToHost, stream));
+        HIP_TRY(hipStreamSynchronize(stream));
+        ST_TRY(pan_sizes(sh, true));
+        const size_t cells = (size_t)sh.NB * sh.NP, NTP = (size_t)kPanWork * sh.TWW;
+        int *u_row = nullptr, *u_col = nullptr;
+        double* u_val = nullptr;
+        auto body = [&]() -> int {
+            ST_TRY(dev_alloc(&pst_tptr, cells * (NTP + 1) + 1)); ST_TRY(dev_alloc(&pst_thead, cells * NTP * 64)); ST_TRY(dev_alloc(&pst_bcol, pan_cap));
+            ST_TRY(dev_alloc(&pst.src, pan_cap)); ST_TRY(dev_alloc(&pst.sw, pan_cap));
+            ST_TRY(dev_alloc(&u_row, (size_t)n + 1)); ST_TRY(dev_alloc(&u_col, (size_t)slots + n + 1)); ST_TRY(dev_alloc(&u_val, (size_t)slots + n + 1));
+            HIP_TRY(hipMemsetAsync(panv.bval, 0, sizeof(double) * pan_cap, stream));
+            HIP_TRY(hipMemsetAsync(pst_bcol, 0, sizeof(unsigned short) * pan_cap, stream));
+            HIP_TRY(hipMemsetAsync(pst_thead, 0, sizeof(unsigned short) * cells * NTP * 64, stream));
+            HIP_TRY(hipMemsetAsync(panv.ovf, 0, sizeof(int), stream));
+            const CsrView U{n, u_row, u_col, u_val};
+            k_pst_union_csr<<<(n + 1 + kBlock - 1) / kBlock, kBlock, 0, stream>>>(pat, u_row, u_col, u_val);
+            panv.tptr = pst_tptr; panv.thead = pst_thead; panv.bcol = pst_bcol;
+            k_pan_rows<<<(n + kBlock - 1) / kBlock, kBlock, 0, stream>>>(U, panv);
+            pan_build_launch(U, sh);
+            HIP_TRY(hipGetLastError());
+            int over = 0;
+            HIP_TRY(hipMemcpyAsync(&over, panv.ovf, sizeof(int), hipMemcpyDeviceToHost, stream));
+            HIP_TRY(hipStreamSynchronize(stream));
+            if (over) return MACHIP_OK;
+            k_pst_src<<<(int)std::min<long>(kMaxGrid, ((long)pan_cap + kBlock - 1) / kBlock), kBlock, 0, stream>>>(pat, (long)slots, panv.bval, (long)pan_cap, pst);
+            HIP_TRY(hipGetLastError());
+            HIP_TRY(hipStreamSynchronize(stream));
+            pst_state = 1;
+            return MACHIP_OK;
+        };
+        const int st = body();
+        for (void* q : {(void*)u_row, (void*)u_col, (void*)u_val}) if (q) (void)hipFree(q);
+        *ready = st == MACHIP_OK && pst_state == 1;
+        return st;
     }
 #ifdef PAN_CLOCKS
 #define MACHIP_FINU_CLK , (const PeerSet*)nullptr, 0, 0, panv.clk
@@ -1153,6 +1244,7 @@
         }
         if ((eligible && want) || after_switch) {
             if (!after_switch) HIP_TRY(hipEventRecord(ev0, stream));
+            ST_TRY(need_csr());
             double lam = 0.0, res = 0.0;
             long iters = 0, spmvs = 0, rst = 0;
             wb_limit_now = throughput_lane ? std::min(wb_soft(), OPT(wb_lane_max, 256)) : wb_soft();
@@ -1244,6 +1336,9 @@
         pan_u = false; last_amp = 0.0; pan32 = false; pan32_from = INT_MAX;
         if (ipc && !(pan.on && pan.u && precision == 0 && (long)pan.grid2 * pan.block2 >= (long)n && pan.grid2 >= ipc->nranks && OPT(ipc_panel, 1) != 0)) pan.on = false;
         if (precision == 1 && !(pan.on && pan.u && pan.TWT == 3 && OPT(pan32, 1) != 0)) pan.on = false;
+        const bool pst_route = csr_stale && pst_serves(pan);
+        pst_live = false;
+        if (!pst_route) ST_TRY(need_csr());
         if (!pan.on && !pmode && !classic && !shard && !ipc && precision == 0 && pp.variant == kVec && pp.width == 4 && pp.defer < 3 &&
             maxlen_hint >= 1 && maxlen_hint <= 16 && OPT(ell, 1) != 0) {
             const int W = maxlen_hint <= 8 ? 8 : 16;
@@ -1255,7 +1350,7 @@
         }
         if (pan.on) {
             const bool rows_ready = pan_rows_ready && !pan.verify && pan_rows_NP == pan.NP && pan_rows_C == pan.C && pan_rows_band == pan.band;
-            ST_TRY(ensure_panel(A, nnz, pan, pan.band, rows_ready));
+            ST_TRY(ensure_panel(A, nnz, pan, pan.band, rows_ready, pst_route));
             if (pan.verify) {
                 int over = 0;
                 HIP_TRY(hipMemcpyAsync(&over, panv.ovf, sizeof(int), hipMemcpyDeviceToHost, stream));
@@ -1692,6 +1787,7 @@
             if (converged) { done = true; break; }
             if (steps_total >= max_steps) break;
             HIP_TRY(hipMemcpyAsync(u, yvec, sizeof(double) * (size_t)n, hipMemcpyDeviceToDevice, stream));
+            ST_TRY(need_csr());
             if (f32_seq) {
                 f32_seq = false;
                 if (res * tiny_l < 1e-4 * std::fabs(lam)) classic = true;
```

Measured after the change: 130.1 iter/s. Within noise of the previous version (-0.2%).
